# unibas-gravis/GiNGR

Measured on AMD Instinct MI355X. Metric: GiNGR update iters/sec, 50k<->50k CPD, higher is better.
Workload: dtype f64; 1 GPU; CPD update, synthetic Gaussian clouds 50000<->50000, GPMM rank 100, w=0.1, rigid global transform, sigma2_0=5032.781; points=50000, targets=50000, rank=100, parallelism=row-shard x1, exchange=single shard

## Files before the change

gingr_amd/_native.py:

```python
from __future__ import annotations

import ctypes
import os
from ctypes import POINTER, c_char_p, c_double, c_int, c_int32, c_int64, c_void_p

import numpy as np

_HERE = os.path.dirname(os.path.abspath(__file__))
LIB_PATH = os.environ.get("GINGR_HIP_LIB") or os.path.join(_HERE, "libgingr_hip.so")

GINGR_OK = 0
ERR_BAD_ARGUMENT, ERR_HIP, ERR_NONFINITE, ERR_NOT_SPD, ERR_NO_DEVICE, ERR_STATE, ERR_NOT_CONVERGED = 1, 2, 3, 4, 5, 6, 7
NUM_PHASES = 3
NUM_SEGMENTS = 2
SEGMENT_FULLFIT = 2
SEGMENT_REVSUM = 3
FLAVOUR_CPD, FLAVOUR_ICP, FLAVOUR_ICP_SURFACE, FLAVOUR_PAIRS = 0, 1, 2, 3
OP_UPDATE, OP_UPDATE_SAMPLE, OP_LOGPDF, OP_POSTERIOR_COVARIANCE, OP_POSTERIOR_MODEL = range(5)
FITTER_OPS = {
    flavour: tuple("gingr_fitter_" + op.format(name) for op in
                   ("update_{}_async", "update_{}_sample_async", "posterior_logpdf_{}", "posterior_covariance_{}", "posterior_model_{}"))
    for flavour, name in ((FLAVOUR_CPD, "cpd"), (FLAVOUR_ICP, "icp"), (FLAVOUR_ICP_SURFACE, "icp_surface"), (FLAVOUR_PAIRS, "pairs"))
}
RCCL_UNIQUE_ID_BYTES = 128

_STATUS_NAMES = {
    1: "GINGR_ERR_BAD_ARGUMENT", 2: "GINGR_ERR_HIP", 3: "GINGR_ERR_NONFINITE", 4: "GINGR_ERR_NOT_SPD",
    5: "GINGR_ERR_NO_DEVICE", 6: "GINGR_ERR_STATE", 7: "GINGR_ERR_NOT_CONVERGED",
}


class GingrNativeError(RuntimeError):
    def __init__(self, code: int, where: str, text: str = ""):
        self.code = code
        super().__init__(f"{where}: {_STATUS_NAMES.get(code, code)} {text}".strip())


class StateScalars(ctypes.Structure):
    _fields_ = [
        ("euler", c_double * 3), ("center", c_double * 3), ("translation", c_double * 3),
        ("scale", c_double), ("sigma2", c_double), ("iteration", c_int32), ("status", c_int32),
    ]


class CpdParams(ctypes.Structure):
    _fields_ = [("w", c_double), ("lambda_", c_double)]


class IcpParams(ctypes.Structure):
    _fields_ = [("initial_sigma", c_double), ("end_sigma", c_double), ("max_iterations", c_int32)]


class MhRequest(ctypes.Structure):
    _fields_ = [
        ("flavour", c_int32), ("kind", c_int32), ("cpd", POINTER(CpdParams)), ("icp", POINTER(IcpParams)),
        ("z", POINTER(c_double)), ("alpha", POINTER(c_double)), ("scalars", POINTER(StateScalars)),
        ("eval_sdev", c_double), ("eval_points", c_int64), ("need_forward", c_int32),
    ]


class MhResult(ctypes.Structure):
    _fields_ = [
        ("scalars", StateScalars), ("log_value", c_double), ("dist_sum", c_double), ("dist_max", c_double), ("count", c_int64),
        ("log_q_forward", c_double), ("log_q_backward", c_double), ("forward_status", c_int32), ("backward_status", c_int32),
    ]


ALLREDUCE_FN = ctypes.CFUNCTYPE(c_int, c_void_p, c_int32, c_void_p, c_int64)
_dp = POINTER(c_double)
_ip = POINTER(c_int32)

KERNEL_GAUSSIAN_MIXTURE, KERNEL_DOT, KERNEL_LOOKUP = 0, 1, 2
OPT_CULL, OPT_FINE_CULL, OPT_NN_GRID, OPT_TRI_GRID, OPT_SPLIT_EXCHANGE, OPT_GRAM_DOWNDATE, OPT_DECIMATE_BATCH = 0, 1, 2, 3, 4, 5, 6


class ScalarKernel(ctypes.Structure):
    _fields_ = [("kind", c_int32), ("n_kernels", c_int32), ("sigmas", _dp), ("scalings", _dp), ("mirror", c_double),
                ("scaling", c_double), ("lookup", _dp)]


GPMM_MAX_COLUMNS = 1536


class GpmmInfo(ctypes.Structure):
    _fields_ = [("columns", c_int32), ("rank", c_int32), ("tolerance_reached", c_int32), ("residual_fraction", c_double),
                ("kept_variance_fraction", c_double)]


CLASSIC_CPD_MAX_COLUMNS = 512


class ClassicCpdLowRankInfo(ctypes.Structure):
    _fields_ = [("columns", c_int32), ("tolerance_reached", c_int32), ("residual_fraction", c_double), ("factor_bytes", c_int64)]


class PcaInfo(ctypes.Structure):
    _fields_ = [("rank", c_int32), ("gpa_sweeps", c_int32), ("gpa_last_change", c_double), ("total_variance", c_double),
                ("kept_variance", c_double)]


class AugmentInfo(ctypes.Structure):
    _fields_ = [("columns", c_int32), ("rank", c_int32), ("total_variance", c_double), ("kept_variance", c_double)]


class LaplacianInfo(ctypes.Structure):
    _fields_ = [("n_components", c_int32), ("n_dropped", c_int32), ("block_columns", c_int32), ("outer_iterations", c_int32),
                ("total_degree", c_int32), ("converged", c_int32), ("max_residual", c_double), ("cut_gap", c_double)]


class NicpInfo(ctypes.Structure):
    _fields_ = [("iterations", c_int32), ("converged", c_int32), ("residual", c_double * 3), ("rhs_norm", c_double * 3)]


SIGNATURES = {
    "gingr_device_count": (c_int, []),
    "gingr_ctx_create": (c_int, [c_int, POINTER(c_void_p)]),
    "gingr_ctx_destroy": (None, [c_void_p]),
    "gingr_last_error": (c_char_p, [c_void_p]),
    "gingr_ctx_set_stream": (c_int, [c_void_p, c_void_p]),
    "gingr_ctx_get_stream": (c_void_p, [c_void_p]),
    "gingr_ctx_synchronize": (c_int, [c_void_p]),
    "gingr_build_info": (c_char_p, []),
    "gingr_ctx_set_option": (c_int, [c_void_p, c_int32, c_int32]),
    "gingr_ctx_get_option": (c_int, [c_void_p, c_int32, POINTER(c_int32)]),
    "gingr_cpd_stats": (c_int, [c_void_p, c_int64, _dp, c_int64, _dp, c_double, c_double, _dp, _dp, _dp, _dp, _dp]),
    "gingr_cpd_initial_sigma2": (c_int, [c_void_p, c_int64, _dp, c_int64, _dp, _dp]),
# ... 13 lines not shown
    "gingr_fitter_icp_surface_phase_async": (c_int, [c_void_p, POINTER(IcpParams), c_int32]),
    "gingr_fitter_get_surface_correspondence": (c_int, [c_void_p, _dp, _dp]),
    "gingr_fitter_surface_distance_stats": (c_int, [c_void_p, c_int32, c_int64, _dp, c_int32, c_double, _dp]),
    "gingr_fitter_mh_step": (c_int, [c_void_p, POINTER(MhRequest), _dp, _dp, POINTER(MhResult)]),
    "gingr_fitter_mh_restore": (c_int, [c_void_p]),
    "gingr_classic_cpd_create": (c_int, [c_void_p, c_int32, c_int64, _dp, c_int64, _dp, c_double, c_double, c_double, POINTER(c_void_p)]),
    "gingr_classic_cpd_destroy": (None, [c_void_p]),
    "gingr_classic_cpd_iterate": (c_int, [c_void_p, c_int32]),
    "gingr_classic_cpd_get": (c_int, [c_void_p, _dp, POINTER(c_double), _dp, _dp]),
    "gingr_classic_cpd_set": (c_int, [c_void_p, _dp, c_double]),
    "gingr_classic_cpd_create_lowrank": (c_int, [c_void_p, c_int64, _dp, c_int64, _dp, c_double, c_double, c_double, c_double, c_int32,
                                                 POINTER(ClassicCpdLowRankInfo), POINTER(c_void_p)]),
    "gingr_classic_cpd_get_factor": (c_int, [c_void_p, _ip, _dp]),
    "gingr_bcpd_create": (c_int, [c_void_p, c_int64, _dp, c_int64, _dp, c_double, c_double, c_double, c_double, c_double, POINTER(c_void_p)]),
    "gingr_bcpd_destroy": (None, [c_void_p]),
    "gingr_bcpd_iterate": (c_int, [c_void_p, c_int32]),
    "gingr_bcpd_get": (c_int, [c_void_p, _dp, _dp, _dp, _dp, _dp, _dp, _dp, _dp]),
    "gingr_bcpd_set": (c_int, [c_void_p, _dp, _dp, _dp, _dp, c_double]),
    "gingr_bcpd_create_lowrank": (c_int, [c_void_p, c_int64, _dp, c_int64, _dp, c_double, c_double, c_double, c_double, c_double, c_double,
                                          c_int32, POINTER(ClassicCpdLowRankInfo), POINTER(c_void_p)]),
    "gingr_bcpd_get_factor": (c_int, [c_void_p, _ip, _dp]),
    "gingr_classic_cpd_transform_points": (c_int, [c_void_p, c_int64, _dp, _dp]),
    "gingr_bcpd_transform_points": (c_int, [c_void_p, c_int64, _dp, _dp]),
    "gingr_bcpd_get_coefficients": (c_int, [c_void_p, _dp]),
    "gingr_mesh_distance_stats": (c_int, [c_void_p, c_int64, _dp, c_int64, _dp, c_int64, POINTER(c_int32), c_int32, c_double, _dp]),
    "gingr_fitter_update_icp_surface_sample_async": (c_int, [c_void_p, POINTER(IcpParams), _dp]),
    "gingr_fitter_posterior_logpdf_icp_surface": (c_int, [c_void_p, POINTER(IcpParams), _dp, POINTER(c_double)]),
    "gingr_rigid_icp_create": (c_int, [c_void_p, c_int32, c_int64, _dp, c_int64, _dp, POINTER(c_void_p)]),
    "gingr_rigid_icp_destroy": (None, [c_void_p]),
    "gingr_rigid_icp_iterate": (c_int, [c_void_p, c_int32, _dp]),
    "gingr_rigid_icp_get": (c_int, [c_void_p, _dp, _dp]),
    "gingr_rigid_icp_set": (c_int, [c_void_p, _dp]),
    "gingr_fitter_set_fit_points": (c_int, [c_void_p, _dp]),
    "gingr_nicp_solve": (c_int, [c_void_p, c_int32, c_int64, _dp, c_int64, _ip, _dp, _dp, c_int32, _ip, _dp, c_double, c_double, c_double,
                                 _dp, _dp]),
    "gingr_nicp_create": (c_int, [c_void_p, c_int32, c_int64, c_int64, _ip, c_int32, _ip, POINTER(c_void_p)]),
    "gingr_nicp_destroy": (None, [c_void_p]),
    "gingr_nicp_step": (c_int, [c_void_p, _dp, _dp, _dp, _dp, c_double, c_double, c_double, c_double, c_int32, _dp, _dp, POINTER(NicpInfo)]),
    "gingr_nicp_get_solution": (c_int, [c_void_p, _dp]),
    "gingr_mesh_closest_points": (c_int, [c_void_p, c_int64, _dp, c_int64, _dp, c_int64, _ip, _dp, _dp, _ip, _dp]),
    "gingr_mesh_decimate": (c_int, [c_void_p, c_int64, _dp, c_int64, _ip, c_int64, POINTER(c_int64), _ip, POINTER(c_int64), _ip, _dp]),
    "gingr_model_new_reference": (c_int, [c_void_p, c_void_p, c_int64, _dp, _ip, _dp, c_int64, c_int64, POINTER(c_void_p)]),
    "gingr_gpmm_build_diagonal": (c_int, [c_void_p, c_int64, _dp, POINTER(ScalarKernel), POINTER(ScalarKernel), POINTER(ScalarKernel),
                                          c_double, c_int32, c_int64, c_int64, POINTER(c_void_p)]),
    "gingr_gpmm_build_diagonal_ex": (c_int, [c_void_p, c_int64, _dp, POINTER(ScalarKernel), POINTER(ScalarKernel), POINTER(ScalarKernel),
                                             c_double, c_int32, c_int32, c_int64, c_int64, POINTER(GpmmInfo), POINTER(c_void_p)]),
    "gingr_model_truncate": (c_int, [c_void_p, c_void_p, c_int32, POINTER(c_void_p)]),
    "gingr_gpmm_build_gaussian": (c_int, [c_void_p, c_int64, _dp, c_int32, _dp, _dp, c_double, c_int32, c_int64, c_int64,
                                          POINTER(c_void_p)]),
    "gingr_pointset_distance_extrema": (c_int, [c_void_p, _dp, c_int64, _dp, _dp]),
    "gingr_model_download": (c_int, [c_void_p, c_void_p, _dp, _dp, _dp, _dp]),
    "gingr_model_num_points": (c_int64, [c_void_p]),
    "gingr_model_rank": (c_int32, [c_void_p]),
    "gingr_model_instance": (c_int, [c_void_p, c_void_p, _dp, _dp, _dp, _dp, c_double, _dp]),
    "gingr_model_coefficients": (c_int, [c_void_p, c_void_p, _dp, _dp, _dp, _dp, _dp]),
    "gingr_model_posterior_mean": (c_int, [c_void_p, c_void_p, _dp, _dp, _dp, _dp, _dp, c_int32, _ip, _dp, _dp, _dp, _dp]),
    "gingr_fitter_create": (c_int, [c_void_p, c_void_p, POINTER(c_void_p)]),
    "gingr_fitter_destroy": (None, [c_void_p]),
    "gingr_fitter_set_target": (c_int, [c_void_p, c_int64, _dp]),
    "gingr_fitter_set_landmarks": (c_int, [c_void_p, c_int32, _ip, _dp, _dp]),
    "gingr_fitter_set_options": (c_int, [c_void_p, c_int32, c_double]),
    "gingr_fitter_set_state": (c_int, [c_void_p, _dp, POINTER(StateScalars)]),
    "gingr_fitter_get_state": (c_int, [c_void_p, _dp, POINTER(StateScalars), _dp]),
    "gingr_fitter_get_cpd_stats": (c_int, [c_void_p, _dp, _dp, _dp, _dp]),
    "gingr_fitter_get_icp_idx": (c_int, [c_void_p, _ip, _dp]),
    "gingr_fitter_update_cpd_async": (c_int, [c_void_p, POINTER(CpdParams), c_int32]),
    "gingr_fitter_update_icp_async": (c_int, [c_void_p, POINTER(IcpParams), c_int32]),
    "gingr_fitter_update_cpd_sample_async": (c_int, [c_void_p, POINTER(CpdParams), _dp]),
    "gingr_fitter_update_icp_sample_async": (c_int, [c_void_p, POINTER(IcpParams), _dp]),
    "gingr_fitter_posterior_logpdf_cpd": (c_int, [c_void_p, POINTER(CpdParams), _dp, _dp]),
    "gingr_fitter_posterior_logpdf_icp": (c_int, [c_void_p, POINTER(IcpParams), _dp, _dp]),
    "gingr_model_marginal_covariance": (c_int, [c_void_p, c_void_p, _dp, _dp, _dp]),
    "gingr_model_cross_covariance": (c_int, [c_void_p, c_void_p, _dp, _dp, c_int64, _dp]),
    "gingr_fitter_posterior_covariance_cpd": (c_int, [c_void_p, POINTER(CpdParams), _dp]),
    "gingr_fitter_posterior_covariance_icp": (c_int, [c_void_p, POINTER(IcpParams), _dp]),
    "gingr_fitter_posterior_covariance_icp_surface": (c_int, [c_void_p, POINTER(IcpParams), _dp]),
    "gingr_model_posterior": (c_int, [c_void_p, c_void_p, _dp, _dp, _dp, _dp, _dp, c_int32, _ip, _dp, _dp, POINTER(c_void_p)]),
    "gingr_fitter_posterior_model_cpd": (c_int, [c_void_p, POINTER(CpdParams), POINTER(c_void_p)]),
    "gingr_fitter_posterior_model_icp": (c_int, [c_void_p, POINTER(IcpParams), POINTER(c_void_p)]),
    "gingr_fitter_posterior_model_icp_surface": (c_int, [c_void_p, POINTER(IcpParams), POINTER(c_void_p)]),
    "gingr_fitter_set_pairs": (c_int, [c_void_p, c_int64, _ip, _dp, _dp]),
    "gingr_fitter_set_pairs_cov": (c_int, [c_void_p, c_int64, _ip, _dp, _dp]),
    "gingr_fitter_get_pair_observations": (c_int, [c_void_p, _dp, _dp]),
    "gingr_fitter_set_sigma2": (c_int, [c_void_p, c_double]),
    "gingr_fitter_last_update_error": (c_int, [c_void_p, POINTER(c_int32)]),
    "gingr_fitter_update_pairs_async": (c_int, [c_void_p, c_int32]),
    "gingr_fitter_pairs_phase_async": (c_int, [c_void_p, c_int32]),
    "gingr_fitter_update_pairs_sample_async": (c_int, [c_void_p, _dp]),
    "gingr_fitter_posterior_logpdf_pairs": (c_int, [c_void_p, _dp, _dp]),
    "gingr_fitter_posterior_covariance_pairs": (c_int, [c_void_p, _dp]),
    "gingr_fitter_posterior_model_pairs": (c_int, [c_void_p, POINTER(c_void_p)]),
    "gingr_model_from_shapes": (c_int, [c_void_p, c_int64, c_int32, _dp, _dp, c_int32, c_int32, c_double, c_double, c_int32,
                                        POINTER(c_void_p), POINTER(PcaInfo)]),
    "gingr_model_augment": (c_int, [c_void_p, c_void_p, c_void_p, c_double, c_int32, POINTER(c_void_p), POINTER(AugmentInfo)]),
    "gingr_model_from_laplacian": (c_int, [c_void_p, c_int64, _dp, c_int64, _ip, c_double, c_int32, c_double, c_int32,
                                           POINTER(LaplacianInfo), POINTER(c_void_p)]),
    "gingr_fitter_retry_counter": (c_int, [c_void_p, c_int32, POINTER(c_int32)]),
    "gingr_fitter_exchange": (c_int, [c_void_p, POINTER(c_void_p), POINTER(c_int64), POINTER(c_int64)]),
    "gingr_fitter_cpd_phase_async": (c_int, [c_void_p, POINTER(CpdParams), c_int32]),
    "gingr_fitter_update_cpd_sharded_async": (c_int, [c_void_p, POINTER(CpdParams), c_int32, ALLREDUCE_FN, c_void_p]),
    "gingr_fitter_update_icp_sharded_async": (c_int, [c_void_p, POINTER(IcpParams), c_int32, ALLREDUCE_FN, c_void_p]),
    "gingr_fitter_icp_phase_async": (c_int, [c_void_p, POINTER(IcpParams), c_int32]),
    "gingr_fitter_update_sharded_async": (c_int, [c_void_p, c_int32, POINTER(CpdParams), POINTER(IcpParams), c_int32, _dp, ALLREDUCE_FN, c_void_p]),
    "gingr_fitter_posterior_logpdf_sharded": (c_int, [c_void_p, c_int32, POINTER(CpdParams), POINTER(IcpParams), _dp, ALLREDUCE_FN, c_void_p, _dp]),
    "gingr_fitter_fullfit_exchange": (c_int, [c_void_p, POINTER(c_void_p), POINTER(c_int64)]),
    "gingr_fitter_reversal_exchange": (c_int, [c_void_p, POINTER(c_void_p), POINTER(c_int64)]),
# ... 83 lines not shown
```

gingr_amd/csrc/common.h:

```cpp
#pragma once
#include <cstdlib>

#include <hip/hip_runtime.h>

#include <cstdarg>
#include <cstdint>
#include <cstdio>
#include <cstring>
#include <string>
#include <vector>

#include "../../include/gingr_hip.h"
#include "host_device.h"

#define GINGR_TIMERS 18

struct gingr_ctx {
    int device = 0;
    hipStream_t own_stream = nullptr;
    hipStream_t stream = nullptr;
    char err[512] = {0};
    bool timing = false;
    struct Span {
        hipEvent_t a, b;
        int which;
    };
    std::vector<Span> spans;
    std::vector<hipEvent_t> pool;
    double t_ms[GINGR_TIMERS] = {0};
    int64_t t_n[GINGR_TIMERS] = {0};
    int cull = 1;
    int tri_grid = 1;
    int nn_grid = 1;
    int32_t *regime_host = nullptr, *regime_dev = nullptr;
    int fine_override = -1;
    unsigned long long *nn_tests = nullptr;
    void *rccl_comm = nullptr;
    int32_t rccl_world = 0, rccl_rank = 0;
    int split_exchange = 0;
    int gram_downdate = -1;
    int decimate_batch = 16;
    hipStream_t side_stream = nullptr, exchange_stream = nullptr;
    hipEvent_t split_ev[2] = {nullptr, nullptr};
    void *scratch = nullptr;
    size_t scratch_bytes = 0;
};

int gingr_set_error(gingr_ctx *ctx, int code, const char *fmt, ...);
void gingr_ctx_rccl_release(gingr_ctx *ctx);

#define HIP_TRY(ctx, expr)                                                                                   \
    do {                                                                                                     \
        hipError_t e__ = (expr);                                                                             \
        if (e__ != hipSuccess)                                                                               \
            return gingr_set_error((ctx), GINGR_ERR_HIP, "%s failed: %s (%s:%d)", #expr, hipGetErrorString(e__), \
                                   __FILE__, __LINE__);                                                      \
    } while (0)

#define GINGR_TRY(expr)          \
    do {                         \
        int s__ = (expr);        \
        if (s__ != GINGR_OK) return s__; \
    } while (0)

#define HANDLE_TRY(ctx, fail, expr)                                                              \
    do {                                                                                         \
        if ((expr) != hipSuccess) {                                                              \
            (void)hipGetLastError();                                                             \
            return fail(gingr_set_error((ctx), GINGR_ERR_HIP, "%s: %s", __func__, #expr));       \
        }                                                                                        \
    } while (0)

inline int check_launch(gingr_ctx *ctx) {
    HIP_TRY(ctx, hipGetLastError());
    return GINGR_OK;
}

struct DevBuf {
    void *p = nullptr;
    size_t bytes = 0;
    DevBuf() = default;
    DevBuf(const DevBuf &) = delete;
    DevBuf &operator=(const DevBuf &) = delete;
    ~DevBuf() {
        if (p) (void)hipFree(p);
    }
    void release() {
        if (p) (void)hipFree(p);
        p = nullptr;
        bytes = 0;
    }
    hipError_t alloc(size_t n) {
        release();
// ... 108 lines not shown
```

gingr_amd/csrc/context.hip:

```cpp
#include "common.h"

#include <map>
#include <mutex>
void set_dynamic_lds(const void *func, int bytes) {
    static std::mutex mu;
    static std::map<std::pair<int, const void *>, int> limit;
    int dev = 0;
    (void)hipGetDevice(&dev);
    std::lock_guard<std::mutex> lock(mu);
    int &have = limit[std::make_pair(dev, func)];
    if (have >= bytes) return;
    if (hipFuncSetAttribute(func, hipFuncAttributeMaxDynamicSharedMemorySize, bytes) == hipSuccess)
        have = bytes;
    else
        (void)hipGetLastError();
}


int gingr_set_error(gingr_ctx *ctx, int code, const char *fmt, ...) {
    if (ctx) {
        va_list ap;
        va_start(ap, fmt);
        vsnprintf(ctx->err, sizeof(ctx->err), fmt, ap);
        va_end(ap);
// ... 78 lines not shown
    (void)hipGetLastError();
    *out = ctx;
    return GINGR_OK;
}

void gingr_ctx_destroy(gingr_ctx *ctx) {
    if (!ctx) return;
    (void)hipSetDevice(ctx->device);
    (void)hipStreamSynchronize(ctx->stream);
    timing_resolve(ctx);
    gingr_ctx_rccl_release(ctx);
    for (auto e : ctx->pool) (void)hipEventDestroy(e);
    if (ctx->scratch) (void)hipFree(ctx->scratch);
    if (ctx->nn_tests) (void)hipFree(ctx->nn_tests);
    if (ctx->regime_host) (void)hipHostFree(ctx->regime_host);
    if (ctx->side_stream) {
        (void)hipStreamSynchronize(ctx->side_stream);
        (void)hipStreamDestroy(ctx->side_stream);
    }
    for (hipEvent_t e : ctx->split_ev)
        if (e) (void)hipEventDestroy(e);
    if (ctx->own_stream) (void)hipStreamDestroy(ctx->own_stream);
    delete ctx;
}

const char *gingr_last_error(const gingr_ctx *ctx) { return ctx ? ctx->err : "null context"; }

int gingr_ctx_set_stream(gingr_ctx *ctx, void *hip_stream) {
    if (!ctx) return GINGR_ERR_BAD_ARGUMENT;
    HIP_TRY(ctx, hipStreamSynchronize(ctx->stream));
    ctx->stream = hip_stream ? reinterpret_cast<hipStream_t>(hip_stream) : ctx->own_stream;
    return GINGR_OK;
}

void *gingr_ctx_get_stream(gingr_ctx *ctx) { return ctx ? reinterpret_cast<void *>(ctx->stream) : nullptr; }

int gingr_ctx_synchronize(gingr_ctx *ctx) {
    if (!ctx) return GINGR_ERR_BAD_ARGUMENT;
    HIP_TRY(ctx, hipSetDevice(ctx->device));
    HIP_TRY(ctx, hipStreamSynchronize(ctx->stream));
    return GINGR_OK;
}

int gingr_ctx_set_option(gingr_ctx *ctx, int32_t option, int32_t value) {
    if (!ctx) return GINGR_ERR_BAD_ARGUMENT;
    switch (option) {
        case GINGR_OPT_CULL: ctx->cull = value != 0; return GINGR_OK;
        case GINGR_OPT_FINE_CULL: ctx->fine_override = value < 0 ? -1 : (value != 0); return GINGR_OK;
        case GINGR_OPT_NN_GRID: ctx->nn_grid = value < 0 ? 0 : (value > 2 ? 2 : value); return GINGR_OK;
        case GINGR_OPT_TRI_GRID: ctx->tri_grid = value < 0 ? 0 : (value > 2 ? 2 : value); return GINGR_OK;
        case GINGR_OPT_SPLIT_EXCHANGE: ctx->split_exchange = value != 0; return GINGR_OK;
        case GINGR_OPT_GRAM_DOWNDATE: ctx->gram_downdate = value < 0 ? -1 : (value != 0); return GINGR_OK;
        case GINGR_OPT_DECIMATE_BATCH: ctx->decimate_batch = value < 1 ? 1 : (value > 60 ? 60 : value); return GINGR_OK;
        default: return gingr_set_error(ctx, GINGR_ERR_BAD_ARGUMENT, "ctx_set_option: unknown option %d", option);
    }
}

int gingr_ctx_get_option(gingr_ctx *ctx, int32_t option, int32_t *value) {
    if (!ctx || !value) return GINGR_ERR_BAD_ARGUMENT;
    switch (option) {
        case GINGR_OPT_CULL: *value = ctx->cull; return GINGR_OK;
        case GINGR_OPT_FINE_CULL: *value = ctx->fine_override; return GINGR_OK;
        case GINGR_OPT_NN_GRID: *value = ctx->nn_grid; return GINGR_OK;
        case GINGR_OPT_TRI_GRID: *value = ctx->tri_grid; return GINGR_OK;
        case GINGR_OPT_SPLIT_EXCHANGE: *value = ctx->split_exchange; return GINGR_OK;
        case GINGR_OPT_GRAM_DOWNDATE: *value = ctx->gram_downdate; return GINGR_OK;
        case GINGR_OPT_DECIMATE_BATCH: *value = ctx->decimate_batch; return GINGR_OK;
        default: return gingr_set_error(ctx, GINGR_ERR_BAD_ARGUMENT, "ctx_get_option: unknown option %d", option);
    }
}

int gingr_ctx_timing_enable(gingr_ctx *ctx, int32_t enable) {
    if (!ctx) return GINGR_ERR_BAD_ARGUMENT;
    ctx->timing = enable != 0;
    return GINGR_OK;
}

int gingr_ctx_timing_read(gingr_ctx *ctx, int32_t which, double *total_ms, int64_t *launches) {
    if (!ctx || which < 0 || which >= GINGR_TIMERS) return GINGR_ERR_BAD_ARGUMENT;
    timing_resolve(ctx);
    if (total_ms) *total_ms = ctx->t_ms[which];
    if (launches) *launches = ctx->t_n[which];
    return GINGR_OK;
}

int gingr_ctx_nn_counting(gingr_ctx *ctx, int32_t enable) {
    if (!ctx) return GINGR_ERR_BAD_ARGUMENT;
    HIP_TRY(ctx, hipSetDevice(ctx->device));
    HIP_TRY(ctx, hipStreamSynchronize(ctx->stream));
    if (enable && !ctx->nn_tests) {
        void *p = nullptr;
        HIP_TRY(ctx, hipMalloc(&p, sizeof(unsigned long long)));
        ctx->nn_tests = static_cast<unsigned long long *>(p);
    }
    if (ctx->nn_tests) {
        HIP_TRY(ctx, hipMemsetAsync(ctx->nn_tests, 0, sizeof(unsigned long long), ctx->stream));
        HIP_TRY(ctx, hipStreamSynchronize(ctx->stream));
    }
    if (!enable && ctx->nn_tests) {
        (void)hipFree(ctx->nn_tests);
        ctx->nn_tests = nullptr;
    }
    return GINGR_OK;
}

int gingr_ctx_nn_tests(gingr_ctx *ctx, int64_t *tests) {
    if (!ctx || !tests) return GINGR_ERR_BAD_ARGUMENT;
    *tests = 0;
    if (!ctx->nn_tests) return gingr_set_error(ctx, GINGR_ERR_STATE, "nn_tests: counting is off (gingr_ctx_nn_counting)");
    HIP_TRY(ctx, hipSetDevice(ctx->device));
    HIP_TRY(ctx, hipStreamSynchronize(ctx->stream));
    unsigned long long v = 0;
    HIP_TRY(ctx, hipMemcpy(&v, ctx->nn_tests, sizeof(v), hipMemcpyDeviceToHost));
    *tests = (int64_t)v;
    return GINGR_OK;
}

int gingr_ctx_timing_reset(gingr_ctx *ctx) {
    if (!ctx) return GINGR_ERR_BAD_ARGUMENT;
    timing_resolve(ctx);
// ... 210 lines not shown
```

gingr_amd/csrc/fitter.h:

```cpp
#pragma once

#include "gp.h"
#include "surface.h"

#include <cstdlib>
#include <vector>

struct StatScratch {
    DevBuf cp, d2, nn, nnd2, ws, part, out;
    DevBuf pos;
    int64_t pos_K = -1, pos_T = -1;
    const int32_t *pos_tri = nullptr;
};

struct gingr_fitter {
    gingr_ctx *ctx = nullptr;
    const gingr_model *m = nullptr;
    int64_t N = 0;
    double *target = nullptr;
    double *inv_den = nullptr, *Pt1 = nullptr;
    double *fit = nullptr;
    double *P1 = nullptr, *PX = nullptr;
    int32_t *nn_idx = nullptr;
    double *nn_d2 = nullptr;
// ... 18 lines not shown
    int32_t *tperm = nullptr;
    std::vector<int32_t> h_tperm;
    double *tboxes = nullptr, *fboxes = nullptr;
    int32_t *tile_bad = nullptr;
    double *xch = nullptr;
    int64_t off[GINGR_NUM_SEGMENTS] = {0, 0}, cnt[GINGR_NUM_SEGMENTS] = {0, 0};
    double *ws = nullptr;
    int64_t ws_doubles = 0;
    int colsum_chunks = 0;
    double *work = nullptr;
    void *aos = nullptr;
    int32_t n_lm = 0;
    int32_t *lm_pid = nullptr;
    double *lm_xyz = nullptr, *lm_cov = nullptr;
    int32_t *lm_mask = nullptr;
    int32_t global_transform = GINGR_RIGID_TRANSFORMS;
    double step_length = 1.0;
    double stop_threshold = -1.0;
    int32_t stop_hit = 0;
    int32_t last_err = 0;
    bool has_state = false;
    int32_t surface_method = 0;
    bool reversed = false;
    int32_t *radj_ptr = nullptr, *radj_tri = nullptr, *rmbnd = nullptr;
    double *rmvn = nullptr, *rfboxes = nullptr;
    void *rws = nullptr;
    int64_t rq0 = 0, rqn = 0;
    double *rtvn_loc = nullptr;
    double *revsum = nullptr, *partial_revsum = nullptr;
    int32_t *gperm = nullptr;
    double *gsorted = nullptr;
    int32_t *rnn_pos = nullptr;
    bool rnn_warm = false;
    int32_t *rtri_pos = nullptr;
    bool rtri_warm = false;
    int32_t *mtri_orig = nullptr, *mboundary = nullptr;
    double *rcp = nullptr, *rd2 = nullptr, *rnnd2 = nullptr, *rw01 = nullptr, *robs = nullptr, *rwin = nullptr;
    int32_t *rnn = nullptr, *rpre = nullptr, *rhit = nullptr, *rkeys = nullptr, *rvals = nullptr, *rskeys = nullptr, *rsvals = nullptr;
    void *rsort = nullptr;
    size_t rsort_bytes = 0;
    int64_t Tm = 0, Tt = 0;
    int32_t *mtri = nullptr, *ttri = nullptr, *ttri_orig = nullptr;
    int32_t *madj_ptr = nullptr, *madj_tri = nullptr, *tadj_ptr = nullptr, *tadj_tri = nullptr;
    double *mcn = nullptr, *tcn = nullptr, *mvn = nullptr, *tvn = nullptr;
    double *mtboxes = nullptr, *ttboxes = nullptr;
    double *mtribox = nullptr, *ttribox = nullptr;
    int32_t *tboundary = nullptr;
    double *surf_cp = nullptr, *surf_d2 = nullptr, *surf_w01 = nullptr, *surf_win = nullptr, *surf_nnd2 = nullptr;
    int32_t *surf_nn = nullptr, *surf_pre = nullptr, *surf_hit = nullptr;
    struct Key {
        std::vector<double> v;
        int flavour = -1;
        double p0 = 0, p1 = 0;
        bool same(const Key &o) const { return flavour == o.flavour && p0 == o.p0 && p1 == o.p1 && v == o.v; }
    };
    Key state_key, post_key;
    bool state_key_valid = false;
    int post_stage = 0;
    bool skip_phase1 = false;
    double *small = nullptr;
    StatScratch *stat_scratch = nullptr;
    double *alt_seg = nullptr;
    bool seg_swapped = false;
    double *seg1_live() const { return seg_swapped ? alt_seg : xch + off[1]; }
    double *seg1_parked() const { return seg_swapped ? xch + off[1] : alt_seg; }
    Key alt_key;
    int alt_stage = 0;
    bool allow_alt = false, corr_stale = false;
    double *fxbuf[2] = {nullptr, nullptr};
    unsigned *lp_sync = nullptr;
    double *lp_scratch = nullptr;
    unsigned lp_epoch = 0;
    bool fx_valid[2] = {false, false};
    double *nfac[2] = {nullptr, nullptr};
    bool nf_valid[2] = {false, false};
    int live = 0;
    int32_t *surf_tri_pos = nullptr;
    bool surf_tri_warm = false;
    bool nn_warm = false, surf_nn_warm = false;
    NNGrid tgrid;
    TriGrid ttgrid;
    MovGrid mgrid;
    void forget_posteriors() {
        post_stage = 0;
        alt_stage = 0;
        fx_valid[0] = fx_valid[1] = false;
        nf_valid[0] = nf_valid[1] = false;
    }
    double *partial_out = nullptr;
    double *fullfit = nullptr, *partial_fullfit = nullptr;
    int32_t *zero_counts = nullptr;
    double *gstage = nullptr;
    int gstage_world = 0;
    int gather_agreed = -1, gather_agreed_world = 0;
    bool sharded() const { return m->M != m->M_total; }
    int32_t *retry = nullptr;
    double *fit_alt = nullptr, *mh_save = nullptr;
    double *mh_rb = nullptr;
    Key mh_key;
    bool mh_saved = false;
    uint64_t mh_serial = 0;
    bool cpd_seen = false, fit_boxes_valid = false;
    int split_half = 0;
    DevBuf cov_work, cov_out;
    int64_t n_pairs = 0, pairs_cap = -1;
    int32_t *ppid = nullptr, *pkeys = nullptr, *pvals = nullptr, *pskeys = nullptr, *psvals = nullptr;
    double *pxyz = nullptr, *pvar = nullptr, *pobs = nullptr, *pwin = nullptr;
    void *psort = nullptr;
    size_t psort_bytes = 0;
    int32_t n_pc = 0, n_cat = 0;
    std::vector<int32_t> h_pc_row, h_lm_row, h_lm_mask;
    std::vector<double> h_pc_xyz, h_pc_cov, h_lm_xyz, h_lm_cov;
    DevBuf cat_pid, cat_xyz, cat_cov;
};

constexpr int64_t kGramDowndateMinRows = 16384;
constexpr int64_t kTriGridMinTriangles = 16384;
constexpr size_t kScalarsDoubles = (sizeof(gingr_state_scalars) + 7) / 8, kDevStateDoubles = (sizeof(DevState) + 7) / 8;

template <typename T>
int dev_alloc(gingr_ctx *ctx, T **p, size_t count) {
    HIP_TRY(ctx, hipMalloc(reinterpret_cast<void **>(p), (count ? count : 1) * sizeof(T)));
    static const bool poison = getenv("GINGR_DEBUG_POISON") != nullptr;
    if (poison) {
        HIP_TRY(ctx, hipMemset(*p, 0xFF, (count ? count : 1) * sizeof(T)));
        HIP_TRY(ctx, hipDeviceSynchronize());
    }
    return GINGR_OK;
}

inline void dev_free(void *p) { if (p) (void)hipFree(p); }

inline Cloud cloud_of(const double *soa, int64_t n) { return Cloud{soa, soa + n, soa + 2 * n, n}; }

inline hipError_t ensure(DevBuf &b, size_t bytes) { return b.p && b.bytes >= bytes ? hipSuccess : b.alloc(bytes); }

int check_ready(gingr_fitter *f);
int check_parameters(gingr_fitter *f, const Correspondence &c);
SweepArgs base_args(const gingr_fitter *f);
void refresh_fit(gingr_fitter *f);
void fit_boxes_now(gingr_fitter *f);
std::vector<double> state_key_values(int32_t r, const double *alpha, const double euler[3], const double center[3], const double t[3],
                                     double scale, double sigma2);
void scalars_of_state(const DevState &hst, gingr_state_scalars *s);
int fitter_upload_zrand(gingr_fitter *f, const double *z);
void launch_mh_readback(gingr_ctx *ctx, int64_t n, const double *block, int nblock, const double *fit, int64_t M, const int32_t *perm,
                        double *out, double *flag, int32_t *done, double epoch);
bool wait_pinned_flag(gingr_fitter *f, double epoch);
int pull_small(gingr_fitter *f, const double *src, int n, double *dst);
struct PinnedWords {
    double *pin = nullptr;
    size_t pin_doubles = 0;
    double *pin_dev = nullptr;
    int32_t *done = nullptr;
    uint64_t epoch = 0;
};
bool wait_pinned_flag(const PinnedWords &w, double epoch);
int pull_small(gingr_ctx *ctx, PinnedWords &w, const double *src, int n, double *dst);
int model_observation_system(gingr_ctx *ctx, const gingr_model *model, const double euler[3], const double center[3],
                             const double translation[3], const double *obs_xyz, const double *weight, int32_t n_lm, const int32_t *lm_pid,
                             const double *lm_xyz, const double *lm_cov, gingr_fitter **f_out, DevBuf &sys);
struct Rot3 {
    double R[9];
};
void launch_basis_rotate(gingr_ctx *ctx, const gingr_model *src, const double *T, const Rot3 &rot, gingr_model *dst);
int gather_fit(gingr_fitter *f, const Correspondence &c, gingr_allreduce_fn reduce, void *user, fitter_gather_fn gather, const char *who);
int fitter_posterior_inputs(gingr_fitter *f, const Correspondence &c);
void free_meshes(gingr_fitter *f);
int pairs_ensure_planes(gingr_fitter *f);
int pairs_rebuild_cov_list(gingr_fitter *f);
void free_pairs(gingr_fitter *f);
```

gingr_amd/csrc/fitter.hip:

```cpp
#include "fitter.h"

#include <algorithm>
#include <atomic>
#include <chrono>
#include <thread>

namespace {

__global__ __launch_bounds__(256) void mh_readback_kernel(const double *__restrict__ block, int nblock, const double *__restrict__ fit, int64_t M,
                                                         const int32_t *__restrict__ perm, double *__restrict__ out, double *flag,
                                                         int32_t *__restrict__ done, double epoch) {
    const int64_t i = (int64_t)blockIdx.x * 256 + threadIdx.x;
    if (i < nblock) out[i] = block[i];
    if (fit && i < M) {
        const int64_t o = perm ? perm[i] : i;
        double *dst = out + nblock + 3 * o;
        dst[0] = fit[i];
        dst[1] = fit[M + i];
        dst[2] = fit[2 * M + i];
    }
    if (!flag) return;
    __threadfence_system();
    __syncthreads();
    if (threadIdx.x == 0) {
        if (atomicAdd(done, 1) == (int)gridDim.x - 1) {
            *done = 0;
            __threadfence_system();
            *reinterpret_cast<volatile double *>(flag) = epoch;
        }
    }
}

}

void launch_mh_readback(gingr_ctx *ctx, int64_t n, const double *block, int nblock, const double *fit, int64_t M, const int32_t *perm,
                        double *out, double *flag, int32_t *done, double epoch) {
    hipLaunchKernelGGL(mh_readback_kernel, dim3((unsigned)ceil_div(n, 256)), dim3(256), 0, ctx->stream, block, nblock, fit, M, perm, out, flag,
                       done, epoch);
}

SweepArgs base_args(const gingr_fitter *f) {
    SweepArgs a;
    memset(&a, 0, sizeof(a));
    a.Q0 = f->m->Q0;
    a.ref = f->m->ref;
    a.mean = f->m->mean;
    a.M = f->m->M;
    a.rp = f->m->rp;
    a.state = f->st;
    a.pose = f->pose;
    a.c0[0] = f->m->c0[0];
    a.c0[1] = f->m->c0[1];
    a.c0[2] = f->m->c0[2];
    a.partial = f->ws;
    return a;
}

void fit_boxes_now(gingr_fitter *f) {
    if (!f->fboxes) return;
    (void)hipMemsetAsync(f->absmax + 1, 0, sizeof(double), f->ctx->stream);
    launch_tile_bbox(f->ctx, cloud_of(f->fit, f->m->M), f->fboxes, f->absmax + 2, f->absmax + 1);
    f->fit_boxes_valid = true;
}

void refresh_fit(gingr_fitter *f) {
    SweepArgs a = base_args(f);
    a.coef0 = f->alpha;
    a.shape_out = f->fit;
    if (f->fboxes && f->m->rp <= 512 && f->cpd_seen) {
        a.qboxes = f->fboxes + 6 * ceil_div(f->m->M, 256);
        a.box_centre = f->absmax + 2;
        a.absmax_slot = f->absmax + 1;
        launch_sweep(f->ctx, SWEEP_FIT, a);
        f->fit_boxes_valid = true;
    } else {
        launch_sweep(f->ctx, SWEEP_FIT, a);
        f->fit_boxes_valid = false;
        if (f->cpd_seen) fit_boxes_now(f);
    }
}

int check_ready(gingr_fitter *f) {
    if (!f) return GINGR_ERR_BAD_ARGUMENT;
    if (!f->target) return gingr_set_error(f->ctx, GINGR_ERR_STATE, "update: no target set (gingr_fitter_set_target)");
    if (!f->has_state) return gingr_set_error(f->ctx, GINGR_ERR_STATE, "update: no state set (gingr_fitter_set_state)");
    if (hipSetDevice(f->ctx->device) != hipSuccess) return gingr_set_error(f->ctx, GINGR_ERR_HIP, "hipSetDevice failed");
    return GINGR_OK;
}

int check_parameters(gingr_fitter *f, const Correspondence &c) {
    GINGR_TRY(check_ready(f));
    switch (correspondence_error(c)) {
        case CorrespondenceError::None: return GINGR_OK;
        case CorrespondenceError::CpdParams: return gingr_set_error(f->ctx, GINGR_ERR_BAD_ARGUMENT, "cpd params: need 0 <= w < 1 and lambda > 0");
        case CorrespondenceError::IcpParams: return gingr_set_error(f->ctx, GINGR_ERR_BAD_ARGUMENT, "icp params: max_iterations < 1");
        case CorrespondenceError::BadFlavour: break;
    }
    return gingr_set_error(f->ctx, GINGR_ERR_BAD_ARGUMENT, "correspondence flavour %d out of range", (int)c.kind);
}

int check_correspondence(gingr_fitter *f, const Correspondence &c) {
    GINGR_TRY(check_parameters(f, c));
    if (needs_meshes(c) && (!f->Tm || !f->Tt)) return gingr_set_error(f->ctx, GINGR_ERR_STATE, "icp surface: no meshes set (gingr_fitter_set_meshes)");
    if (c.kind == Flavour::Pairs) GINGR_TRY(pairs_ensure_planes(f));
    return GINGR_OK;
}

std::vector<double> state_key_values(int32_t r, const double *alpha, const double euler[3], const double center[3], const double t[3],
                                     double scale, double sigma2) {
    std::vector<double> v(alpha, alpha + r);
    for (int q = 0; q < 3; ++q) v.push_back(euler[q]);
    for (int q = 0; q < 3; ++q) v.push_back(center[q]);
    for (int q = 0; q < 3; ++q) v.push_back(t[q]);
    v.push_back(scale);
    v.push_back(sigma2);
    return v;
}

void scalars_of_state(const DevState &hst, gingr_state_scalars *s) {
    for (int q = 0; q < 3; ++q) {
        s->euler[q] = hst.euler[q];
        s->center[q] = hst.center[q];
// ... 126 lines not shown
                    f->zrand, f->pose, f->scalars, f->fxbuf[0], f->fxbuf[1], f->alt_seg, f->nfac[0], f->nfac[1],
                    f->lp_sync, f->lp_scratch, f->retry, f->part, f->absmax, f->tperm, f->tboxes, f->fboxes,
                    f->tile_bad, f->xch, f->fullfit, f->gstage, f->zero_counts, f->ws, f->work, f->aos, f->lm_pid,
                    f->lm_xyz, f->lm_cov, f->lm_mask};
    for (void *q : ptrs) dev_free(q);
    if (f->pin) (void)hipHostFree(f->pin);
    if (f->zpin) (void)hipHostFree(f->zpin);
    if (f->zpin_done) (void)hipEventDestroy(f->zpin_done);
    nn_grid_free(&f->tgrid);
    tri_grid_free(&f->ttgrid);
    free_meshes(f);
    free_pairs(f);
    delete f;
}

int gingr_fitter_set_target(gingr_fitter *f, int64_t N, const double *target_xyz) {
    if (!f) return GINGR_ERR_BAD_ARGUMENT;
    f->nn_warm = f->surf_nn_warm = f->surf_tri_warm = false;
    f->forget_posteriors();
    gingr_ctx *ctx = f->ctx;
    if (N < 1 || N > INT32_MAX || !target_xyz) return gingr_set_error(ctx, GINGR_ERR_BAD_ARGUMENT, "set_target: bad N");
    HIP_TRY(ctx, hipSetDevice(ctx->device));
    HIP_TRY(ctx, hipStreamSynchronize(ctx->stream));
    const int64_t M = f->m->M;
    const int32_t rp = f->m->rp;
    void *old[] = {f->target, f->inv_den, f->Pt1, f->xch, f->ws, f->aos, f->tperm, f->tboxes, f->fboxes, f->tile_bad};
    for (void *q : old) dev_free(q);
    free_meshes(f);
    f->target = f->inv_den = f->Pt1 = f->xch = f->ws = f->tboxes = f->fboxes = nullptr;
    f->aos = nullptr;
    f->tperm = f->tile_bad = nullptr;
    f->N = N;
    GINGR_TRY(dev_alloc(ctx, &f->target, (size_t)3 * N));
    GINGR_TRY(dev_alloc(ctx, &f->inv_den, (size_t)N));
    GINGR_TRY(dev_alloc(ctx, &f->Pt1, (size_t)N));
    f->cnt[0] = N;
    f->cnt[1] = (int64_t)rp * rp + rp + 8 + rp;
    int64_t o = 0;
    for (int s = 0; s < GINGR_NUM_SEGMENTS; ++s) {
        f->off[s] = o;
        o += round_up(f->cnt[s], 32);
    }
    GINGR_TRY(dev_alloc(ctx, &f->xch, (size_t)o));
    f->seg_swapped = false;
    HIP_TRY(ctx, hipMemsetAsync(f->xch, 0, (size_t)o * sizeof(double), ctx->stream));
    int64_t w = cpd_colsum_ws_doubles(M, N);
    auto mx = [&](int64_t v) {
        if (v > w) w = v;
    };
    mx(cpd_rowstats_ws_doubles(M, N));
    mx(ceil_div(nn_ws_bytes(M, N), 8));
    mx(ceil_div(nn_ws_bytes(N, M), 8));
    mx(gram_ws_doubles(M, rp) + sweep_ws_doubles(M, rp));
    f->ws_doubles = w;
    GINGR_TRY(dev_alloc(ctx, &f->ws, (size_t)w));
    const int64_t big = M > N ? M : N;
    double *aos = nullptr;
    GINGR_TRY(dev_alloc(ctx, &aos, (size_t)3 * big));
    f->aos = aos;
    HIP_TRY(ctx, hipMemcpyAsync(aos, target_xyz, (size_t)3 * N * sizeof(double), hipMemcpyHostToDevice, ctx->stream));
    kd_leaf_order(target_xyz, N, f->h_tperm);
    GINGR_TRY(nn_grid_build(ctx, target_xyz, N, f->h_tperm.data(), M, &f->tgrid));
    GINGR_TRY(dev_alloc(ctx, &f->tperm, (size_t)N));
    HIP_TRY(ctx, hipMemcpyAsync(f->tperm, f->h_tperm.data(), (size_t)N * sizeof(int32_t), hipMemcpyHostToDevice, ctx->stream));
    GINGR_TRY(dev_alloc(ctx, &f->tboxes, (size_t)ceil_div(N, 256) * 30));
    GINGR_TRY(dev_alloc(ctx, &f->fboxes, (size_t)ceil_div(M, 256) * 30));
    f->fit_boxes_valid = false;
    GINGR_TRY(dev_alloc(ctx, &f->tile_bad, (size_t)ceil_div(N, 256)));
    launch_aos_to_soa(ctx, aos, N, f->target, f->tperm);
    launch_tile_bbox(ctx, cloud_of(f->target, N), f->tboxes);
    launch_cloud_centroid(ctx, cloud_of(f->target, N), f->absmax + 2);
    launch_cloud_absmax(ctx, cloud_of(f->target, N), f->absmax + 2, f->absmax);
    if (f->has_state) fit_boxes_now(f);
    GINGR_TRY(check_launch(ctx));
    HIP_TRY(ctx, hipStreamSynchronize(ctx->stream));
    return GINGR_OK;
}

int gingr_fitter_set_landmarks(gingr_fitter *f, int32_t n_lm, const int32_t *lm_pid, const double *lm_xyz,
                               const double *lm_cov) {
    if (!f) return GINGR_ERR_BAD_ARGUMENT;
    f->forget_posteriors();
    gingr_ctx *ctx = f->ctx;
    if (n_lm < 0 || (n_lm > 0 && (!lm_pid || !lm_xyz || !lm_cov)))
        return gingr_set_error(ctx, GINGR_ERR_BAD_ARGUMENT, "set_landmarks: bad argument");
    HIP_TRY(ctx, hipSetDevice(ctx->device));
    HIP_TRY(ctx, hipStreamSynchronize(ctx->stream));
    dev_free(f->lm_pid);
    dev_free(f->lm_xyz);
    dev_free(f->lm_cov);
    f->lm_pid = nullptr;
    f->lm_xyz = f->lm_cov = nullptr;
    f->n_lm = n_lm;
    const int64_t M = f->m->M;
    std::vector<int32_t> mask((size_t)M, 0), local((size_t)(n_lm > 0 ? n_lm : 1), -1);
    for (int32_t l = 0; l < n_lm; ++l) {
        if (lm_pid[l] < 0 || lm_pid[l] >= f->m->M_total)
            return gingr_set_error(ctx, GINGR_ERR_BAD_ARGUMENT, "set_landmarks: point id %d out of range", lm_pid[l]);
        const int64_t lp = (int64_t)lm_pid[l] - f->m->row_begin;
        if (lp >= 0 && lp < M) {
            const int32_t pos = f->m->hiperm[(size_t)lp];
            local[(size_t)l] = pos;
            mask[(size_t)pos] = 1;
        }
    }
    HIP_TRY(ctx, hipMemcpy(f->lm_mask, mask.data(), (size_t)M * sizeof(int32_t), hipMemcpyHostToDevice));
// ... 171 lines not shown
        scalars6[5] = loc[5];
    }
    return GINGR_OK;
}

int gingr_fitter_get_icp_idx(gingr_fitter *f, int32_t *idx, double *d2) {
    if (!f) return GINGR_ERR_BAD_ARGUMENT;
    gingr_ctx *ctx = f->ctx;
    if (f->corr_stale)
        return gingr_set_error(ctx, GINGR_ERR_STATE, "get_icp_idx: a probabilistic query brought another state's posterior back; the correspondences on the device are not this state's -- run an update or a phase first");
    HIP_TRY(ctx, hipSetDevice(ctx->device));
    const int64_t M = f->m->M;
    std::vector<int32_t> hidx((size_t)M);
    std::vector<double> hd2((size_t)M);
    HIP_TRY(ctx, hipMemcpyAsync(hidx.data(), f->nn_idx, (size_t)M * sizeof(int32_t), hipMemcpyDeviceToHost, ctx->stream));
    HIP_TRY(ctx, hipMemcpyAsync(hd2.data(), f->nn_d2, (size_t)M * sizeof(double), hipMemcpyDeviceToHost, ctx->stream));
    HIP_TRY(ctx, hipStreamSynchronize(ctx->stream));
    for (int64_t sidx = 0; sidx < M; ++sidx) {
        const int32_t row = f->m->hperm[(size_t)sidx];
        const int32_t pos = hidx[(size_t)sidx];
        if (idx) idx[row] = (pos >= 0 && (size_t)pos < f->h_tperm.size()) ? f->h_tperm[(size_t)pos] : -1;
        if (d2) d2[row] = hd2[(size_t)sidx];
    }
    return GINGR_OK;
}

int gingr_fitter_retry_counter(gingr_fitter *f, int32_t set_to, int32_t *value_out) {
    if (!f) return GINGR_ERR_BAD_ARGUMENT;
    gingr_ctx *ctx = f->ctx;
    HIP_TRY(ctx, hipSetDevice(ctx->device));
    if (set_to >= 0) HIP_TRY(ctx, hipMemcpyAsync(f->retry, &set_to, sizeof(set_to), hipMemcpyHostToDevice, ctx->stream));
    int32_t v = set_to;
    if (value_out && set_to < 0) HIP_TRY(ctx, hipMemcpyAsync(&v, f->retry, sizeof(v), hipMemcpyDeviceToHost, ctx->stream));
    HIP_TRY(ctx, hipStreamSynchronize(ctx->stream));
    if (value_out) *value_out = v;
    return GINGR_OK;
}

int gingr_fitter_exchange(gingr_fitter *f, void **dev_ptr, int64_t offsets[GINGR_NUM_SEGMENTS],
                          int64_t counts[GINGR_NUM_SEGMENTS]) {
    if (!f || !dev_ptr) return GINGR_ERR_BAD_ARGUMENT;
    if (!f->xch) return gingr_set_error(f->ctx, GINGR_ERR_STATE, "exchange: no target set");
    *dev_ptr = f->xch;
    for (int s = 0; s < GINGR_NUM_SEGMENTS; ++s) {
        if (offsets) offsets[s] = f->off[s];
        if (counts) counts[s] = f->cnt[s];
    }
    return GINGR_OK;
}

}

void fitter_set_partial_output(gingr_fitter *f, double *base) { f->partial_out = base; }
void fitter_set_partial_fullfit(gingr_fitter *f, double *base) { f->partial_fullfit = base; }
double *fitter_fullfit(gingr_fitter *f) { return f->fullfit; }
void fitter_set_partial_revsum(gingr_fitter *f, double *base) { f->partial_revsum = base; }
double *fitter_revsum(gingr_fitter *f) { return f->revsum; }
int fitter_upload_zrand(gingr_fitter *f, const double *z) {
    gingr_ctx *ctx = f->ctx;
    const size_t bytes = (size_t)f->m->rp * sizeof(double);
    if (!f->zpin) {
        HIP_TRY(ctx, hipHostMalloc(reinterpret_cast<void **>(&f->zpin), bytes, hipHostMallocDefault));
        if (hipEventCreateWithFlags(&f->zpin_done, hipEventDisableTiming) != hipSuccess) {
            (void)hipHostFree(f->zpin);
            f->zpin = nullptr, f->zpin_done = nullptr;
            return gingr_set_error(ctx, GINGR_ERR_HIP, "upload of the posterior draws: hipEventCreate failed");
        }
    } else {
        HIP_TRY(ctx, hipEventSynchronize(f->zpin_done));
    }
    memset(f->zpin, 0, bytes);
    memcpy(f->zpin, z, (size_t)f->m->r * sizeof(double));
    HIP_TRY(ctx, hipMemcpyAsync(f->zrand, f->zpin, bytes, hipMemcpyHostToDevice, ctx->stream));
    HIP_TRY(ctx, hipEventRecord(f->zpin_done, ctx->stream));
    return GINGR_OK;
}
int fitter_set_zrand(gingr_fitter *f, const double *z) {
    f->zrand_active = false;
    if (!z) return GINGR_OK;
    GINGR_TRY(fitter_upload_zrand(f, z));
    f->zrand_active = true;
    return GINGR_OK;
}
gingr_ctx *fitter_ctx(gingr_fitter *f) { return f->ctx; }
bool fitter_gather_possible(gingr_fitter *f, int32_t world, int32_t rank) {
    if (!f || !f->fullfit || world < 1 || rank < 0 || rank >= world) return false;
    const gingr_model *m = f->m;
    const int64_t Mt = m->M_total, base = Mt / world, extra = Mt % world;
    const int64_t b = rank * base + (rank < extra ? rank : extra), e = b + base + (rank < extra ? 1 : 0);
    return b == m->row_begin && e - b == m->M;
}
int fitter_gather_agreed(gingr_fitter *f, int32_t world) { return f->gather_agreed_world == world ? f->gather_agreed : -1; }
void fitter_set_gather_agreed(gingr_fitter *f, int32_t world, int agreed) {
    f->gather_agreed = agreed;
    f->gather_agreed_world = world;
}
bool fitter_reversed(gingr_fitter *f) { return f->reversed; }
const gingr_model *fitter_model(gingr_fitter *f) { return f->m; }
```

gingr_amd/csrc/fitter_phases.hip:

```cpp
#include "fitter.h"

#include <algorithm>
#include <utility>

namespace {

__global__ __launch_bounds__(256) void swap_segments_kernel(double *__restrict__ a, double *__restrict__ b, int64_t n, int exchange) {
    const int64_t i = (int64_t)blockIdx.x * 256 + threadIdx.x;
    if (i >= n) return;
    const double va = a[i], vb = b[i];
    a[i] = vb;
    if (exchange) b[i] = va;
}

__global__ __launch_bounds__(256) void fit_contribution_kernel(const double *__restrict__ fit, const int32_t *__restrict__ iperm, int64_t M,
                                                               int64_t row_begin, int64_t M_total, double *__restrict__ full) {
    const int64_t g = (int64_t)blockIdx.x * 256 + threadIdx.x;
    if (g >= M_total) return;
    const int64_t l = g - row_begin;
    const bool mine = l >= 0 && l < M;
    const int64_t pos = mine ? iperm[l] : 0;
#pragma unroll
    for (int d = 0; d < 3; ++d) full[d * M_total + g] = mine ? fit[d * M + pos] : 0.0;
}
// ... 15 lines not shown
    const int64_t q = g < cut ? g / (base + 1) : extra + (g - cut) / (base > 0 ? base : 1);
    const int64_t b = q * base + (q < extra ? q : extra);
    const double *p = stage + q * 3 * chunk + (g - b);
#pragma unroll
    for (int d = 0; d < 3; ++d) full[d * M_total + g] = p[d * chunk];
}

__global__ __launch_bounds__(256) void reversal_local_kernel(int64_t M, int64_t row_begin, const int32_t *__restrict__ perm, int64_t M_total,
                                                             const double *__restrict__ sums, const double *__restrict__ sigma2,
                                                             double *__restrict__ obs, double *__restrict__ win) {
    const int64_t p = (int64_t)blockIdx.x * 256 + threadIdx.x;
    if (p >= M) return;
    const int64_t g = row_begin + perm[p];
    const double k = sums[3 * M_total + g];
    const double kk = k > 0.0 ? k : 1.0;
#pragma unroll
    for (int d = 0; d < 3; ++d) obs[d * M + p] = sums[d * M_total + g] / kk;
    win[p] = k / sigma2[0];
}

__global__ __launch_bounds__(256) void soa_permute_kernel(const double *__restrict__ src, const int32_t *__restrict__ perm, int64_t n,
                                                          double *__restrict__ dst) {
    const int64_t p = (int64_t)blockIdx.x * 256 + threadIdx.x;
    if (p >= n) return;
    const int64_t g = perm[p];
#pragma unroll
    for (int d = 0; d < 3; ++d) dst[d * n + p] = src[d * n + g];
}
__global__ __launch_bounds__(256) void index_map_kernel(const int32_t *__restrict__ pos, int64_t n, const int32_t *__restrict__ map,
                                                        int32_t *__restrict__ idx) {
    const int64_t j = (int64_t)blockIdx.x * 256 + threadIdx.x;
    if (j >= n) return;
    const int32_t v = pos[j];
    idx[j] = v >= 0 ? map[v] : v;
}

int64_t split_cut(int64_t N) { return (N / 512) * 256; }

void nearest_target_vertex(gingr_ctx *ctx, gingr_fitter *f, Cloud query, Cloud tgt, int32_t *idx, double *d2, bool warm) {
    const int32_t *w = warm ? idx : nullptr;
    if (ctx->nn_grid && f->tgrid.ready && ctx->cull && query.n <= f->tgrid.max_queries) {
        if (!launch_nn_grid(ctx, query, tgt, f->tperm, f->tgrid, w, idx, d2))
            launch_nn(ctx, query, tgt, f->tperm, f->tboxes, f->ws, idx, d2, idx, f->tgrid.flag, f->tgrid.cur_nflag());
    } else {
        launch_nn(ctx, query, tgt, f->tperm, f->tboxes, f->ws, idx, d2, w);
    }
}

struct Segments {
    double *seg0, *G, *rhs, *sc8;
    double *seg0w, *Gw, *rhsw, *sc8w;
};

bool memo_enter(gingr_fitter *f, const Correspondence &c, int phase) {
    const gingr_model *m = f->m;
    if (phase == 0) {
        f->skip_phase1 = false;
        gingr_fitter::Key k;
        k.flavour = memo_flavour_key(c, f->surface_method, f->reversed);
        k.p0 = c.cpd.w;
        k.p1 = c.cpd.lambda;
        const bool single = m->M == m->M_total;
        if (single && f->state_key_valid) {
            k.v = f->state_key.v;
            if (f->post_stage == 2 && f->post_key.same(k)) {
                f->skip_phase1 = true;
                return true;
            }
            if (f->allow_alt && !f->partial_out && f->alt_stage == 2 && f->alt_key.same(k)) {
                const bool both = f->post_stage == 2;
                f->seg_swapped = !f->seg_swapped;
                if (both) {
                    std::swap(f->post_key, f->alt_key);
                } else {
                    f->post_key = f->alt_key;
                    f->alt_stage = 0;
                    f->fx_valid[f->live] = f->nf_valid[f->live] = false;
                }
                f->live ^= 1;
                f->post_stage = 2;
                f->corr_stale = true;
                f->skip_phase1 = true;
                return true;
            }
            if (f->allow_alt && !f->partial_out && f->post_stage == 2) {
                f->seg_swapped = !f->seg_swapped;
                f->alt_key = f->post_key;
                f->alt_stage = 2;
                f->live ^= 1;
            }
            f->fx_valid[f->live] = f->nf_valid[f->live] = false;
            f->post_key = k;
            f->post_stage = 1;
        } else {
            f->post_stage = 0;
            f->fx_valid[f->live] = f->nf_valid[f->live] = false;
        }
        f->corr_stale = false;
    } else if (phase == 1) {
        if (f->skip_phase1) {
            f->skip_phase1 = false;
            return true;
        }
        if (f->post_stage == 1) f->post_stage = 2;
    } else {
        f->state_key_valid = false;
        f->mh_saved = false;
    }
    return false;
}

void phase0_cpd_colsums(gingr_fitter *f, const Segments &s, Cloud fit, Cloud tgt) {
    gingr_ctx *ctx = f->ctx;
    const gingr_model *m = f->m;
// ... 181 lines not shown
        CpdObsArgs ob;
        memset(&ob, 0, sizeof(ob));
        ob.ref = m->ref;
        ob.mean = m->mean;
        ob.sigma2 = &f->st->sigma2;
        ob.R = f->st->R;
        ob.center = f->st->center;
        ob.t = f->st->t;
        ob.lambda = c.cpd.lambda;
        ob.lm_mask = f->lm_mask;
        ob.weight = f->weight;
        ob.evec = f->evec;
        launch_cpd_rowstats(ctx, fit, tgt, &f->st->sigma2, f->absmax, f->inv_den, f->tboxes, f->tile_bad, f->ws, f->P1,
                            f->PX, f->part, f->scalars, nullptr, 0, &ob, false);
        fa.scalar_mode = 1;
        fa.part = f->part;
        fa.scalars_local = f->scalars;
        fa.contribute_xpx = m->row_begin == 0 ? 1 : 0;
    }
}

struct GramOutcome {
    bool rhs_done;
    ZeroGate rhs_gate;
};

GramOutcome phase1_gram(gingr_fitter *f, const Correspondence &c, double *gram_ws, double *sweep_ws, Phase1FinalizeArgs &fa) {
    gingr_ctx *ctx = f->ctx;
    const gingr_model *m = f->m;
    const int64_t M = m->M;
    const int32_t rp = m->rp;
    GramOutcome out{false, ZeroGate{}};
    if (uniform_weights(c, f->reversed, f->n_lm)) {
        fa.nslabs = 0;
        fa.scaled_src = m->mom + MomentLayout{rp}.stot();
        fa.sigma2 = &f->st->sigma2;
        fa.scaled_contribute = m->row_begin == 0 ? 1 : 0;
    } else if (zero_one_weights(c, f->reversed) &&
               (ctx->gram_downdate == 1 || (ctx->gram_downdate < 0 && M >= kGramDowndateMinRows))) {
        const bool gated = ctx->gram_downdate != 1;
        ZeroGate few{f->zero_counts, (int32_t)ceil_div(M, 256), 0, M}, many = few;
        many.run_if_many = 1;
        fa.gram_partial = gram_ws;
        fa.nslabs = launch_gram_downdate(ctx, m->Q0, M, rp, f->weight, gram_ws, gated ? &few : nullptr);
        fa.scaled_src = m->mom + MomentLayout{rp}.stot();
        fa.sigma2 = &f->st->sigma2;
        fa.scaled_contribute = m->row_begin == 0 ? 1 : 0;
        if (gated) {
            bool alt_rhs = false;
            fa.alt_nslabs = launch_gram(ctx, m->Q0, M, rp, f->weight, gram_ws, nullptr, f->evec, sweep_ws, &alt_rhs, &many);
            fa.gate = many;
            out.rhs_gate = few;
        }
    } else {
        fa.gram_partial = gram_ws;
        fa.nslabs = launch_gram(ctx, m->Q0, M, rp, f->weight, gram_ws, nullptr, f->evec, sweep_ws, &out.rhs_done);
    }
    return out;
}

void phase2_solve_and_commit(gingr_fitter *f, const Correspondence &c, const Segments &s) {
    gingr_ctx *ctx = f->ctx;
    const gingr_model *m = f->m;
    const int32_t r = m->r, rp = m->rp;
    const bool eig = uniform_weights(c, f->reversed, f->n_lm) && !f->zrand_active && m->eig_ready;
    if (eig)
        launch_posterior_solve_eig(ctx, r, rp, m->eigV, m->eigL, &f->st->sigma2, s.rhs, f->acoef, f->st);
    else if (f->zrand_active && f->allow_alt && f->post_stage == 2 && f->nf_valid[f->live] && m->M == m->M_total && !f->partial_out)
        launch_posterior_sample_cached(ctx, r, rp, f->nfac[f->live], f->fxbuf[f->live] + (int64_t)rp * rp, f->zrand, f->acoef, f->st);
    else
        launch_posterior_solve(ctx, r, rp, s.G, s.rhs, f->zrand_active ? f->zrand : nullptr, f->work, f->acoef, f->st);
    launch_post_matvecs(ctx, m, f->alpha, f->acoef, f->zbuf);
    PostSolveArgs a;
    memset(&a, 0, sizeof(a));
    a.r = r;
    a.rp = rp;
    a.pvec = m->pvec;
    a.zbuf = f->zbuf;
    a.alpha = f->alpha;
    a.scalars = s.sc8;
    a.is_icp = post_solve_sigma2_rule(c);
    if (is_icp_schedule(c)) {
        a.icp_step = (c.icp.initial_sigma - c.icp.end_sigma) / (double)c.icp.max_iterations;
        a.icp_end = c.icp.end_sigma;
    }
    a.step = f->step_length;
    a.global_transform = f->global_transform;
    a.state = f->st;
    a.retry = f->retry;
    a.zero_slot = f->absmax + 1;
    a.probabilistic = f->zrand_active ? 1 : 0;
    a.stop_threshold = f->stop_threshold;
    launch_post_solve(ctx, a);
    refresh_fit(f);
}

int run_phase(gingr_fitter *f, const Correspondence &c, int phase) {
    gingr_ctx *ctx = f->ctx;
    const gingr_model *m = f->m;
    const int64_t M = m->M;
    const int32_t rp = m->rp;
    if (f->seg_swapped && !f->allow_alt) {
        const int64_t seg = (int64_t)rp * rp + rp + 8;
        hipLaunchKernelGGL(swap_segments_kernel, dim3((unsigned)ceil_div(seg, 256)), dim3(256), 0, ctx->stream, f->xch + f->off[1], f->alt_seg,
                           seg, 0);
        f->seg_swapped = false;
        f->alt_stage = 0;
        f->fx_valid[f->live ^ 1] = f->nf_valid[f->live ^ 1] = false;
    }
    Segments s;
    s.seg0 = f->xch + f->off[0];
    s.G = f->seg1_live();
    s.rhs = s.G + (int64_t)rp * rp;
    s.sc8 = s.rhs + rp;
    double *wbase = f->partial_out ? f->partial_out : f->xch;
    s.seg0w = wbase + f->off[0];
    s.Gw = f->partial_out ? wbase + f->off[1] : s.G;
    s.rhsw = s.Gw + (int64_t)rp * rp;
    s.sc8w = s.rhsw + rp;
    const Cloud fit = cloud_of(f->fit, M);
    const Cloud tgt = cloud_of(f->target, f->N);
    if (phase == GINGR_PHASE_GATHER) {
        if (!f->sharded()) return GINGR_OK;
        if (!f->fullfit) return gingr_set_error(ctx, GINGR_ERR_STATE, "gather phase: no meshes set (gingr_fitter_set_meshes)");
        hipLaunchKernelGGL(fit_contribution_kernel, dim3((unsigned)ceil_div(m->M_total, 256)), dim3(256), 0, ctx->stream, f->fit, m->iperm, M,
                           m->row_begin, m->M_total, f->partial_fullfit ? f->partial_fullfit : f->fullfit);
        return check_launch(ctx);
    }
    const Cloud meshc = f->sharded() && f->fullfit ? cloud_of(f->fullfit, m->M_total) : fit;
    if (memo_enter(f, c, phase)) return GINGR_OK;
    switch (phase) {
        case 0:
            if (c.kind == Flavour::Pairs)
                break;
            if (reversed_icp(c, f->reversed))
                GINGR_TRY(phase0_reversed(f, c, fit, tgt, meshc));
            else if (c.kind == Flavour::IcpSurface)
                phase0_surface(f, fit, tgt, meshc);
            else if (c.kind == Flavour::IcpCloud)
                phase0_nearest_vertex(f, fit, tgt);
            else
                phase0_cpd_colsums(f, s, fit, tgt);
            break;
        case 1: {
            Phase1FinalizeArgs fa;
            memset(&fa, 0, sizeof(fa));
            fa.rp = rp;
// ... 266 lines not shown
```

gingr_amd/csrc/gp.h:

```cpp
#pragma once

#include "common.h"
#include "correspondence.h"
#include "svd3.h"

#include <functional>

#define GINGR_COEFF_NOISE 1e-5

struct DevState {
    double R[9];
    double euler[3];
    double center[3];
    double t[3];
    double scale;
    double sigma2;
    int32_t iteration;
    int32_t status;
    int32_t err;
    int32_t pad;
    int32_t stopped;
    int32_t pad2;
};

// ... 23 lines not shown
    double scale;
};

struct MomentLayout {
    int32_t rp;
    __host__ __device__ int64_t stot() const { return 0; }
    __host__ __device__ int64_t S(int d, int e) const { return (int64_t)rp * rp * (1 + d * 3 + e); }
    __host__ __device__ int64_t V(int d, int e) const { return (int64_t)rp * rp * 10 + (int64_t)rp * (d * 3 + e); }
    __host__ __device__ int64_t W(int d) const { return (int64_t)rp * rp * 10 + (int64_t)rp * (9 + d); }
    __host__ __device__ int64_t total() const { return (int64_t)rp * rp * 10 + (int64_t)rp * 12; }
};

struct PostVec {
    int32_t rp;
    static constexpr int kV = 0;
    static constexpr int kW = 9;
    static constexpr int kBV = 12;
    static constexpr int kBW = 21;
    static constexpr int kRows = 24;
    __host__ __device__ int64_t consts() const { return (int64_t)kRows * rp; }
    __host__ __device__ int64_t total() const { return consts() + 16; }
    static constexpr int kZa = 0;
    static constexpr int kBSa = 9;
    static constexpr int kBTa = 18;
    static constexpr int kA1 = 27;
    static constexpr int kZRows = 28;
};

constexpr int kBasisRowSlack = 144;

struct gingr_model {
    gingr_ctx *ctx = nullptr;
    int64_t M_total = 0, row_begin = 0, row_end = 0, M = 0;
    int32_t r = 0, rp = 0;
    double *Q0 = nullptr;
    double *ref = nullptr;
    double *mean = nullptr;
    double *mom = nullptr;
    int32_t *perm = nullptr;
    std::vector<int32_t> hperm, hiperm;
    int32_t *iperm = nullptr;
    std::vector<double> h_full_pts;
    double *Binv = nullptr;
    double *eigV = nullptr;
    double *eigL = nullptr;
    bool eig_ready = false;
    double *cmat = nullptr;
    double *pvec = nullptr;
    double c0[3] = {0, 0, 0};
    double Pp[9] = {0};
    double Ps[3] = {0};
    std::vector<double> variance;
    bool finalized = false;
};

void launch_interp_pack(gingr_ctx *ctx, const double *Qs, int32_t rp, const int32_t *inv_src, const int32_t *ids, const double *w,
                        const int32_t *perm_new, int64_t row_begin, int64_t M, double *Q0);

int model_create_impl(gingr_ctx *ctx, int64_t M_total, int32_t rank, const double *ref, const double *mean,
                      const double *variance, int64_t row_begin, int64_t row_end,
                      const std::function<int(gingr_model *)> &fill_basis, gingr_model **out, bool finalize = true);

void fitter_set_partial_output(gingr_fitter *f, double *base);
void fitter_set_partial_fullfit(gingr_fitter *f, double *base);
int check_correspondence(gingr_fitter *f, const Correspondence &c);
typedef int (*fitter_gather_fn)(void *user, gingr_fitter *f);
int fitter_sharded_update(gingr_fitter *f, const Correspondence &c, int32_t n_iterations, const double *z, gingr_allreduce_fn reduce,
                          void *user, fitter_gather_fn gather = nullptr, bool split_native = false);
int fitter_sharded_logpdf(gingr_fitter *f, const Correspondence &c, const double *mesh_xyz_full, gingr_allreduce_fn reduce, void *user,
                          double *logpdf, fitter_gather_fn gather = nullptr);
int fitter_run_phase(gingr_fitter *f, const Correspondence &c, int phase);
int fitter_update(gingr_fitter *f, const Correspondence &c, int32_t n_iterations);
int fitter_sample_update(gingr_fitter *f, const Correspondence &c, const double *z);
int fitter_posterior_logpdf(gingr_fitter *f, const Correspondence &c, const double *mesh_xyz, double *logpdf);
int fitter_logpdf_prepare(gingr_fitter *f, const double *mesh_xyz_full);
int fitter_logpdf_finish(gingr_fitter *f, double *logpdf);
int fitter_set_zrand(gingr_fitter *f, const double *z);
double *fitter_fullfit(gingr_fitter *f);
void fitter_set_partial_revsum(gingr_fitter *f, double *base);
double *fitter_revsum(gingr_fitter *f);
gingr_ctx *fitter_ctx(gingr_fitter *f);
bool fitter_gather_possible(gingr_fitter *f, int32_t world, int32_t rank);
int fitter_gather_agreed(gingr_fitter *f, int32_t world);
void fitter_set_gather_agreed(gingr_fitter *f, int32_t world, int agreed);
const gingr_model *fitter_model(gingr_fitter *f);

struct ZeroGate {
    const int32_t *counts;
    int32_t nblocks;
    int32_t run_if_many;
    int64_t M;
};

__device__ __forceinline__ bool gate_open(const ZeroGate &g) {
    if (!g.counts) return true;
    __shared__ int gate_sum;
    if (threadIdx.x == 0) gate_sum = 0;
    __syncthreads();
    int s = 0;
    for (int b = threadIdx.x; b < g.nblocks; b += blockDim.x) s += g.counts[b];
#pragma unroll
    for (int off = 32; off > 0; off >>= 1) s += __shfl_xor(s, off);
    if ((threadIdx.x & 63) == 0 && s != 0) atomicAdd(&gate_sum, s);
    __syncthreads();
    const bool many = (int64_t)gate_sum * 8 > g.M;
    return many == (g.run_if_many != 0);
}

enum SweepMode {
    SWEEP_RHS = 0,
    SWEEP_PROJ1 = 1,
    SWEEP_SHAPES = 2,
    SWEEP_PROJ2 = 3,
    SWEEP_FIT = 4,
    SWEEP_POSED = 5,
    SWEEP_RHS_ICP = 6
};

struct SweepArgs {
    const double *Q0;
    const double *ref;
    const double *mean;
    int64_t M;
    int32_t rp;
    const double *coef0;
    const double *coef1;
    const double *evec;
    const double *shape_in;
    double *shape_out;
    const DevState *state;
    const DevPose *pose;
    double c0[3];
    double *partial;
    double *out;
    double *zero_slot;
    double *qboxes;
    const double *box_centre;
    double *absmax_slot;
    int32_t no_reduce;
    const int32_t *icp_idx;
    const double *tx, *ty, *tz;
    int64_t n_targets;
    const int32_t *lm_mask;
    double *weight_out, *evec_out;
    const DevState *frame;
    ZeroGate gate;
};

int sweep_num_blocks(int64_t M);
int64_t sweep_ws_doubles(int64_t M, int32_t rp);
void launch_sweep(gingr_ctx *ctx, SweepMode mode, const SweepArgs &a);

int64_t gram_ws_doubles(int64_t M, int32_t rp);
int launch_gram(gingr_ctx *ctx, const double *Q0, int64_t M, int32_t rp, const double *weight, double *ws, double *G,
                const double *evec = nullptr, double *rhs_partial = nullptr, bool *rhs_done = nullptr, const ZeroGate *gate = nullptr);

int64_t gram_wide_ws_doubles(int64_t M, int32_t rp);
int launch_gram_wide(gingr_ctx *ctx, const double *Q0, int64_t M, int32_t rp, const double *weight, double *ws, const double *evec,
                     double *rhs_partial, const ZeroGate *gate = nullptr);

int64_t gram_rows_ws_doubles(int64_t rows, int32_t rp);
int launch_gram_rows(gingr_ctx *ctx, const double *Z, int64_t rows, int32_t rp, double *ws);

struct Phase1FinalizeArgs {
    int32_t rp;
    const double *gram_partial;
    int32_t nslabs;
    const double *scaled_src;
    const double *sigma2;
    int32_t scaled_contribute;
    double *G;
    const double *sweep_partial;
    int32_t sweep_blocks;
    double *rhs;
    int32_t scalar_mode;
    const double *part;
    double *scalars_local;
    double *sc8;
    int32_t contribute_xpx;
    ZeroGate gate;
    int32_t alt_nslabs;
};
void launch_phase1_finalize(gingr_ctx *ctx, const Phase1FinalizeArgs &a);
int launch_gram_downdate(gingr_ctx *ctx, const double *Q0, int64_t M, int32_t rp, const double *weight, double *ws,
                         const ZeroGate *gate = nullptr);

void launch_obs_cpd(gingr_ctx *ctx, const gingr_model *m, const DevState *st, Cloud fit, const double *P1,
                    const double *PX, double lambda, const int32_t *lm_mask, double *weight, double *evec);
void launch_obs_icp(gingr_ctx *ctx, const gingr_model *m, const DevState *st, Cloud target, const int32_t *idx,
                    const int32_t *lm_mask, double *weight, double *evec);
void launch_obs_points(gingr_ctx *ctx, const gingr_model *m, const DevState *st, const double *obs_soa,
                       const double *weight_in, double *weight, double *evec, const int32_t *lm_mask = nullptr,
                       int32_t *zero_counts = nullptr);
void launch_landmarks(gingr_ctx *ctx, const gingr_model *m, const DevState *st, int32_t n_lm, const int32_t *lm_pid_local,
                      const double *lm_xyz, const double *lm_cov, double *G, double *rhs);

void launch_posterior_solve(gingr_ctx *ctx, int32_t r, int32_t rp, const double *G, const double *rhs, const double *zrand,
                            double *work, double *a, DevState *st);
int launch_posterior_logpdf(gingr_ctx *ctx, int32_t r, int32_t rp, const double *G, const double *rhs, const double *Stot,
                            const double *qte, double *fx, bool cached, double *work, double *out2, unsigned *sync = nullptr,
                            unsigned epoch = 0, bool keep_factor = true, double *nfac = nullptr);
void launch_posterior_sample_cached(gingr_ctx *ctx, int32_t r, int32_t rp, const double *nfac, const double *a_mean, const double *zrand,
                                    double *a, DevState *st);
void launch_posterior_solve_eig(gingr_ctx *ctx, int32_t r, int32_t rp, const double *eigV, const double *eigL, const double *sigma2,
                                const double *rhs, double *a, DevState *st);
constexpr int kJacMaxN = 512;
int sym_eig(gingr_ctx *ctx, int count, const double *const *G, const int32_t *ldg, const int32_t *n, double *const *evals,
            double *const *Vs, bool blocks = false);
int launch_jacobi_eig(gingr_ctx *ctx, const double *G, int32_t ldg, int32_t n, double *evals, double *Vs, bool blocks = false);
constexpr int kSymEigColsMaxN = 192;
int64_t sym_eig_cols_work_doubles(int32_t n);
int64_t sym_eig_blocks_work_doubles(int32_t n);
int sym_eig_blocks(gingr_ctx *ctx, int count, const double *const *G, const int32_t *ldg, const int32_t *n, double *const *work,
                   double *const *evals, double *const *Vs, int32_t *const *info);
void launch_sym_eig_cols(gingr_ctx *ctx, int count, const double *const *G, const int32_t *ldg, const int32_t *n, double *const *work,
                         double *const *evals, double *const *Vs, int32_t *const *info);
int64_t posterior_work_doubles(int32_t rp);
int64_t binv_work_doubles(int32_t rp);
void launch_binv(gingr_ctx *ctx, int32_t r, int32_t rp, const double *S, double *work, double *Binv, int32_t *err_flag);
void launch_coeff_solve(gingr_ctx *ctx, int32_t r, int32_t rp, const double *Binv, const double *p, double *out);
void launch_state_init(gingr_ctx *ctx, DevState *st, const gingr_state_scalars *host_scalars_dev, double *zero_slot = nullptr);

int64_t moment_grams_ws_doubles(int64_t M, int32_t rp);
void launch_moment_grams(gingr_ctx *ctx, const double *Q0, int64_t M, int32_t rp, double *ws, double *mom);
void launch_centered_mean(gingr_ctx *ctx, const gingr_model *m, double *ptil);

struct PostSolveArgs {
    int32_t r, rp;
    const double *pvec;
    const double *zbuf;
    double *alpha;
    const double *scalars;
    int32_t is_icp;
    double icp_step, icp_end;
    double step;
    int32_t global_transform;
    DevState *state;
    double *zero_slot;
    int32_t *retry;
    int32_t probabilistic;
    double stop_threshold;
};
#define GINGR_RETRY_INIT 10
void launch_post_solve(gingr_ctx *ctx, const PostSolveArgs &a);
void launch_post_matvecs(gingr_ctx *ctx, const gingr_model *m, const double *alpha, const double *a, double *zbuf);
void launch_small_gemm(gingr_ctx *ctx, int32_t r, int32_t rp, const double *A, const double *B, double scale, double *out);
void launch_postvec(gingr_ctx *ctx, int32_t r, int32_t rp, const double *Binv, const double *moment_vectors, double *pvec);

void launch_marginal_covariance(gingr_ctx *ctx, const gingr_model *m, const double *W, int64_t ldw, bool upper, const double R[9],
                                const DevState *state, double *cov6);
void launch_cross_covariance(gingr_ctx *ctx, const gingr_model *m, const double *W, int64_t ldw, const double R[9], int64_t device_row,
// ... 7 lines not shown
```

gingr_amd/csrc/gp.hip:

```cpp
#include "dense_spd.h"
#include "gp.h"
#include "solve_blocks.h"

#include <algorithm>

namespace {


template <bool FAST, typename PtrD>
__device__ __forceinline__ void posterior_solve_body(PtrD sm, int r, int rp, const double *__restrict__ G, const double *__restrict__ rhs,
                                                     const double *__restrict__ zrand, double *__restrict__ a, DevState *__restrict__ st,
                                                     int *bad_spd, int *bad) {
    const int n = rp, ld = solve_ld(n);
    constexpr int XR = FAST ? 2 * kNB : kNB;
    auto A = sm;
    auto y = sm + (size_t)n * ld;
    auto rd = sm + (size_t)(n + XR) * ld;
    auto y2 = rd + n;
    const int tid = threadIdx.x;
    if (tid == 0) {
        *bad_spd = 0;
        *bad = 0;
    }
    for (int k = tid; k < kNB * ld; k += kSolveThreads) y[k] = k < r ? rhs[k] : 0.0;
    for (int k = tid; k < n; k += kSolveThreads) y2[k] = (zrand && k < r) ? zrand[k] : 0.0;
    if (FAST)
        for (int k = tid; k < kNB * ld; k += kSolveThreads) {
            const int c = k / ld, j = k - c * ld;
            y[kNB * ld + k] = (j < n && (j & 15) == c) ? 1.0 : 0.0;
        }
    GINGR_STAGE_CLOCK(7)
    lds_load_spd<kSolveThreads>(A, ld, r, n, G, 1.0, nullptr, 0.0, 1.0);
    GINGR_STAGE_CLOCK(0)
    lds_cholesky<kSolveThreads>(A, ld, n, rd, bad_spd, kNB, FAST ? kNB : 0);
    GINGR_STAGE_CLOCK(4)
    if constexpr (FAST) {
        if (zrand) {
            lds_backward_w<kSolveThreads>(A, ld, n, y + kNB * ld, y2, rd);
            for (int k = tid; k < n; k += kSolveThreads) y2[k] = rd[k];
            __syncthreads();
        }
        lds_backward_w<kSolveThreads>(A, ld, n, y + kNB * ld, y, rd);
        for (int k = tid; k < n; k += kSolveThreads) y[k] = rd[k];
        __syncthreads();
    } else {
        lds_backward<kSolveThreads>(A, ld, n, rd, y);
        if (zrand) lds_backward<kSolveThreads>(A, ld, n, rd, y2);
    }
    GINGR_STAGE_CLOCK(5)
    GINGR_STAGE_CLOCK(6)
    for (int k = tid; k < rp; k += kSolveThreads) {
        const double v = k < r ? y[k] + y2[k] : 0.0;
        a[k] = v;
        if (!finite_d(v)) *bad = 1;
    }
    __syncthreads();
    if (tid == 0) {
        if (*bad_spd)
            st->err = GINGR_ERR_NOT_SPD;
        else if (*bad)
            st->err = GINGR_ERR_NONFINITE;
    }
}

template <int MODE>
__global__ __launch_bounds__(kSolveThreads) void posterior_solve_lds_kernel(int r, int rp, const double *__restrict__ G,
                                                                  const double *__restrict__ rhs,
                                                                  const double *__restrict__ zrand, double *__restrict__ a,
                                                                  DevState *__restrict__ st) {
    extern __shared__ double lds_sm[];
    __shared__ int bad_spd, bad;
#ifdef GINGR_SOLVE_TWICE
    for (int pass = 0; pass < 2; ++pass) {
        __syncthreads();
#endif
    posterior_solve_body<MODE == 0>(lds_sm, r, rp, G, rhs, zrand, a, st, &bad_spd, &bad);
#ifdef GINGR_SOLVE_TWICE
    }
#endif
}

constexpr int kWideSolveThreads = 512;

template <int SW>
struct WideSolveLds {
    double rdl[SW];
    double red[2][kWideSolveThreads / 64][SW];
    double xs[2][512];
    double yv[2][SW];
    int bad_spd;
};

template <int SW, bool HAS_S>
__device__ __forceinline__ void wide_solve_body(double *P, WideSolveLds<SW> &Ls, int r, int n, const double *__restrict__ G, double ca,
                                                const double *__restrict__ S, double cs, double ci, const double *__restrict__ b1,
                                                const double *__restrict__ b2, double cb, const double *__restrict__ zrand, double *gw) {
    constexpr int ldp = SW + 1, NW = kWideSolveThreads / 64;
    double *rdl = Ls.rdl;
    auto &red = Ls.red;
    auto &xs = Ls.xs;
    auto &yv = Ls.yv;
    int &bad_spd = Ls.bad_spd;
    const int tid = threadIdx.x, lane = tid & 63, wave = tid >> 6, l15 = lane & 15, l4 = lane >> 4;
    double *Lg = gw;
    double *rdg = gw + (size_t)(n + kNB) * n;
    const int nvec = zrand ? 2 : 1;
    if (tid == 0) bad_spd = 0;
    GINGR_STAGE_CLOCK(7)
    typedef double d2 __attribute__((ext_vector_type(2)));
    constexpr int NTJ = SW / 16;
    constexpr int TSTEP = NW / NTJ;
    constexpr int TACC = SW == 64 ? 9 : 9;
    constexpr int HALF = SW / 2;
    constexpr int RSTEP = kWideSolveThreads / HALF;
    constexpr int PRE = 17;
    const int wv = __builtin_amdgcn_readfirstlane(wave);
    const int my_tj = wv % NTJ, ti0 = wv / NTJ;
    for (int e = tid; e < kNB * n; e += kWideSolveThreads) Lg[(size_t)n * n + e] = e < r ? (b2 ? __builtin_fma(cb, b2[e], b1[e]) : b1[e]) : 0.0;
    __syncthreads();
    const int srow = tid / HALF, scp = tid % HALF;
    for (int kb = 0; kb < n; kb += SW) {
        const int sw = min(SW, n - kb), rows = n - kb + kNB;
        const int nti = rows >> 4, ntj = sw >> 4;
        v4f64 acc[TACC];
// ... 737 lines not shown
        return (brow == 0 && c < r) ? __builtin_fma(GINGR_COEFF_NOISE, rhs[c], qte[c]) : 0.0;
    }
};
__global__ __launch_bounds__(512) void logpdf_finish_kernel(int r, int n, int64_t Mp, const double *__restrict__ G, const double *__restrict__ rhs,
                                                            const double *__restrict__ Wn, const double *__restrict__ Wk, const double *__restrict__ Lk,
                                                            const int32_t *__restrict__ flag_n, const int32_t *__restrict__ flag_k,
                                                            double *__restrict__ fx, double *__restrict__ out2) {
    __shared__ double w[512], hv[2][512], red[512];
    const int tid = threadIdx.x;
    for (int k = tid; k < n; k += 512) w[k] = k < r ? Wk[k] : 0.0;
    __syncthreads();
    for (int kk = tid & 255; kk < r; kk += 256) {
        const int half = tid >> 8;
        const int j0 = half ? (r + 1) / 2 : 0, j1 = half ? r : (r + 1) / 2;
        double s0 = 0.0, s1 = 0.0, s2 = 0.0, s3 = 0.0;
        int j = j0;
        for (; j + 3 < j1; j += 4) {
            s0 = __builtin_fma(G[(int64_t)j * n + kk], w[j], s0);
            s1 = __builtin_fma(G[(int64_t)(j + 1) * n + kk], w[j + 1], s1);
            s2 = __builtin_fma(G[(int64_t)(j + 2) * n + kk], w[j + 2], s2);
            s3 = __builtin_fma(G[(int64_t)(j + 3) * n + kk], w[j + 3], s3);
        }
        for (; j < j1; ++j) s0 = __builtin_fma(G[(int64_t)j * n + kk], w[j], s0);
        hv[half][kk] = (s0 + s1) + (s2 + s3);
    }
    for (int64_t e = tid; e < (int64_t)n * n; e += 512) {
        const int64_t i = e / n, j = e - i * n;
        fx[e] = j <= i ? Lk[i * Mp + j] : 0.0;
    }
    for (int k = tid; k < n; k += 512) {
        fx[(int64_t)n * n + k] = k < r ? Wn[k] : 0.0;
        fx[(int64_t)n * n + n + k] = 1.0 / Lk[(int64_t)k * Mp + k];
    }
    __syncthreads();
    double part = 0.0;
    for (int k = tid; k < r; k += 512) {
        const double nw = (hv[0][k] + hv[1][k]) + w[k];
        part = __builtin_fma(w[k] - Wn[k], nw - rhs[k], part);
    }
    red[tid] = part;
    __syncthreads();
    for (int st2 = 256; st2 > 0; st2 >>= 1) {
        if (tid < st2) red[tid] += red[tid + st2];
        __syncthreads();
    }
    if (tid == 0) {
        const bool bad = *flag_n != 0 || *flag_k != 0;
        out2[0] = bad ? __builtin_nan("") : -0.5 * red[0] - 0.5 * (double)r * 1.8378770664093454836;
        out2[1] = bad ? 1.0 : 0.0;
    }
}
}

void launch_posterior_solve(gingr_ctx *ctx, int32_t r, int32_t rp, const double *G, const double *rhs, const double *zrand,
                            double *work, double *a, DevState *st) {
    TimerScope ts(ctx, 5);
    if (rp > 240 && !zrand) {
        const DenseSpdWork ws(rp, DenseSpdWork::kRhsRows);
        double *Aw = work + ws.aw(), *Linv = work + ws.linv(), *W = work + ws.w();
        int32_t *flag = reinterpret_cast<int32_t *>(work + ws.flag());
        launch_spd_system(ctx->stream, (int)r, ws, SpdIdentityPlus{G, (int)rp}, SpdRhsRow{rhs}, Aw, flag);
        dense_spd_solve3(ctx, Aw, ws.Mp, Linv, W, flag);
        hipLaunchKernelGGL(solve_finish_kernel, dim3(1), dim3(256), 0, ctx->stream, (int)r, (int)rp, W, flag, a, st);
        return;
    }
    if (r <= 128) {
        const bool fast = rp <= 112;
        const size_t lds = lds_solve_doubles(rp, fast ? 2 * kNB : kNB) * sizeof(double);
        auto go = [&](auto kern) {
            if (lds > 48 * 1024)
                set_dynamic_lds(kern, (size_t)(lds));
            hipLaunchKernelGGL(kern, dim3(1), dim3(kSolveThreads), lds, ctx->stream, (int)r, (int)rp, G, rhs, zrand, a, st);
        };
        if (fast)
            go(posterior_solve_lds_kernel<0>);
        else
            go(posterior_solve_lds_kernel<1>);
        return;
    }
    auto gow = [&](auto kern, int sw) {
        const size_t lds = (size_t)(rp + kNB) * (sw + 1) * sizeof(double);
        set_dynamic_lds(kern, (size_t)(lds));
        hipLaunchKernelGGL(kern, dim3(1), dim3(kWideSolveThreads), lds, ctx->stream, (int)r, (int)rp, G, rhs, zrand, a, st, work);
    };
    if (rp <= 256)
        gow(posterior_solve_wide_kernel<64>, 64);
    else
        gow(posterior_solve_wide_kernel<32>, 32);
}

namespace {
__global__ __launch_bounds__(1024) void posterior_solve_eig_kernel(int r, int rp, const double *__restrict__ V,
                                                                   const double *__restrict__ lam, const double *__restrict__ sigma2,
                                                                   const double *__restrict__ rhs, double *__restrict__ a, DevState *st) {
    __shared__ double x[512], t[512];
    __shared__ int bad;
    const int tid = threadIdx.x, lane16 = tid & 15, grp = tid >> 4;
    if (tid == 0) bad = 0;
    for (int k = tid; k < r; k += 1024) x[k] = rhs[k];
    __syncthreads();
    const double inv_s2 = 1.0 / sigma2[0];
    for (int k = grp; k < r; k += 64) {
        double s = 0.0;
        for (int i = lane16; i < r; i += 16) s = __builtin_fma(V[(int64_t)i * r + k], x[i], s);
        s = group16_sum(s);
        if (lane16 == 0) t[k] = s / (1.0 + lam[k] * inv_s2);
    }
    __syncthreads();
    for (int i = grp; i < rp; i += 64) {
        double s = 0.0;
        if (i < r)
            for (int k = lane16; k < r; k += 16) s = __builtin_fma(V[(int64_t)i * r + k], t[k], s);
        s = group16_sum(s);
        if (lane16 == 0) {
            a[i] = i < r ? s : 0.0;
            if (!finite_d(s)) bad = 1;
        }
    }
    __syncthreads();
    if (tid == 0 && bad) st->err = GINGR_ERR_NONFINITE;
}
}

void launch_posterior_solve_eig(gingr_ctx *ctx, int32_t r, int32_t rp, const double *eigV, const double *eigL, const double *sigma2,
                                const double *rhs, double *a, DevState *st) {
// ... 109 lines not shown
```

gingr_amd/csrc/gp_gram.hip:

```cpp
#include "gp.h"
#include "gp_device.h"

#include <algorithm>

namespace {

__global__ __launch_bounds__(256) void gram_kernel(const double *__restrict__ Q0, int64_t rows, int rp,
                                                   const double *__restrict__ weight, int64_t rows_per_slab, int nbp,
                                                   int row_stride, int offA, int offB, int full,
                                                   double *__restrict__ partial) {
    __shared__ double red[16 * 4 * 64];
    int pa = 0, pb = 0;
    if (full) {
        pa = blockIdx.y / nbp;
        pb = blockIdx.y - pa * nbp;
    } else {
        int t = blockIdx.y;
        for (pa = 0; pa < nbp; ++pa) {
            const int cnt = nbp - pa;
            if (t < cnt) {
                pb = pa + t;
                break;
            }
            t -= cnt;
// ... 43 lines not shown
        for (int t = 0; t < 4; ++t) {
            ca[t] = na[t];
            cb[t] = nb[t];
        }
    }
    for (int w = 1; w < 4; ++w) {
        __syncthreads();
        if (wave == w) {
#pragma unroll
            for (int i = 0; i < 4; ++i)
#pragma unroll
                for (int j = 0; j < 4; ++j)
#pragma unroll
                    for (int reg = 0; reg < 4; ++reg) red[((i * 4 + j) * 4 + reg) * 64 + lane] = acc[i][j][reg];
        }
        __syncthreads();
        if (wave == 0) {
#pragma unroll
            for (int i = 0; i < 4; ++i)
#pragma unroll
                for (int j = 0; j < 4; ++j)
#pragma unroll
                    for (int reg = 0; reg < 4; ++reg) acc[i][j][reg] += red[((i * 4 + j) * 4 + reg) * 64 + lane];
        }
    }
    if (wave != 0) return;
    double *out = partial + (int64_t)blockIdx.x * rp * rp;
#pragma unroll
    for (int i = 0; i < 4; ++i)
#pragma unroll
        for (int j = 0; j < 4; ++j) {
#pragma unroll
            for (int reg = 0; reg < 4; ++reg) {
                const int gi = pa * 64 + 4 * (kq + 4 * reg) + i;
                const int gj = pb * 64 + 4 * cl + j;
                if (gi < rp && gj < rp) out[(int64_t)gi * rp + gj] = acc[i][j][reg];
            }
        }
}

template <int NT>
__host__ __device__ constexpr int tri_row(int q) {
    int t = 0;
    while (q >= NT - t) q -= NT - t, ++t;
    return t;
}
template <int NT>
__host__ __device__ constexpr int tri_col(int q) {
    int t = 0;
    while (q >= NT - t) q -= NT - t, ++t;
    return t + q;
}

template <int NT, int HALF, bool FULL>
__device__ __forceinline__ void gram_tri_half(const double *__restrict__ Q0, int rp, const double *__restrict__ weight, int64_t r0,
                                              int64_t r1, int kgroup, int kq, int cl, int lane, double *red, double *xchg,
                                              double *__restrict__ out, const double *__restrict__ evec, int64_t npts,
                                              double *__restrict__ rhs_out, double *rsh) {
    constexpr int kTiles = NT * (NT + 1) / 2;
    constexpr int kMine = HALF == 0 ? (kTiles + 1) / 2 : kTiles / 2;
    constexpr int kM = kMine > 0 ? kMine : 1;
    v4f64 acc[kM];
#pragma unroll
    for (int q = 0; q < kMine; ++q) acc[q] = v4f64{0, 0, 0, 0};
    constexpr int kOwn = HALF == 0 ? (NT + 1) / 2 : NT / 2;
    constexpr int kO = kOwn > 0 ? kOwn : 1;
    const bool with_rhs = evec != nullptr;
    const bool with_w = weight != nullptr;
    const int kgu = __builtin_amdgcn_readfirstlane(kgroup);
    const int64_t ubase = r0 + 4 * kgu;
    const int64_t first = ubase + kq;
    const double *pclamp = Q0 + r0 * rp + cl;
    const double *pnext = Q0 + first * rp + cl;
    const int64_t pstep = 16 * (int64_t)rp;
    int64_t left_u = r1 - ubase;
    const int64_t pt_first = first / 3;
    const int rem_first = (int)(first - 3 * pt_first);
    constexpr unsigned kThird = 0x55555556u;
    unsigned third = (unsigned)rem_first * kThird;
    const double *wclamp = with_w ? weight + r0 / 3 : pclamp;
    const double *eclamp = with_rhs ? evec + r0 / 3 : pclamp;
    const double *wp = with_w ? weight + pt_first : pclamp;
    const double *ep = with_rhs ? evec + rem_first * npts + pt_first : pclamp;
    const int64_t estep = with_rhs ? 5 + npts : 0, ewrap = with_rhs ? 6 - 2 * npts : 0;
    double fn[2][kO], wn[2], en[2];
    int vrows[2];
    auto load_next = [&](auto slot) __attribute__((always_inline)) {
        constexpr int L = decltype(slot)::value;
        if (left_u >= 4) {
            vrows[L] = 4;
#pragma unroll
            for (int k = 0; k < kOwn; ++k) fn[L][k] = pnext[16 * (2 * k + HALF)];
            wn[L] = *wp;
            en[L] = *ep;
        } else {
            vrows[L] = (int)max((int64_t)0, left_u);
            const bool valid = left_u > kq;
            const double *p = valid ? pnext : pclamp;
#pragma unroll
            for (int k = 0; k < kOwn; ++k) fn[L][k] = p[16 * (2 * k + HALF)];
            wn[L] = *(valid ? wp : wclamp);
            en[L] = *(valid ? ep : eclamp);
        }
        left_u -= 16;
        pnext += pstep;
        const unsigned t2 = third + kThird;
        const bool wrap = t2 < third;
        third = t2;
        wp += wrap ? 6 : 5;
        ep += wrap ? ewrap : estep;
    };
    double racc[kO];
#pragma unroll
    for (int k = 0; k < kOwn; ++k) racc[k] = 0.0;
    const int64_t nsteps = (r1 - r0 + 15) / 16;
    constexpr int kBufStride = 4 * 2 * NT * 64;
    double *xbuf = xchg + (size_t)kgu * 2 * NT * 64 + lane;
    double cur[2][NT], a[2][NT];
    auto hand_over_write = [&](auto slot) __attribute__((always_inline)) {
        constexpr int L = decltype(slot)::value;
        double w = wn[L], e = en[L];
        if constexpr (!FULL) {
            w = with_w ? w : 1.0;
            e = with_rhs ? e : 0.0;
        }
        if (vrows[L] < 4) {
            asm volatile("; rows past the slab");
            const bool valid = vrows[L] > kq;
            w = valid ? w : 0.0;
            e = valid ? e : 0.0;
        }
#pragma unroll
        for (int k = 0; k < kOwn; ++k) {
            xbuf[L * kBufStride + (2 * k + HALF) * 64] = fn[L][k];
            xbuf[L * kBufStride + (NT + 2 * k + HALF) * 64] = fn[L][k] * w;
            racc[k] = __builtin_fma(fn[L][k], e, racc[k]);
        }
    };
    auto hand_over_read = [&](auto set) __attribute__((always_inline)) {
        constexpr int S = decltype(set)::value;
#pragma unroll
        for (int t = 0; t < NT; ++t) {
            cur[S][t] = xbuf[S * kBufStride + t * 64];
            a[S][t] = xbuf[S * kBufStride + (NT + t) * 64];
        }
    };
    auto mfmas = [&](auto set, auto begin, auto endq) __attribute__((always_inline)) {
        constexpr int S = decltype(set)::value;
        static_for<decltype(begin)::value, decltype(endq)::value>([&](auto m) {
            constexpr int mi = decltype(m)::value, q = 2 * mi + HALF, tr = tri_row<NT>(q), tc = tri_col<NT>(q);
            acc[mi] = __builtin_amdgcn_mfma_f64_16x16x4f64(a[S][tr], cur[S][tc], acc[mi], 0, 0, 0);
        });
    };
    using std::integral_constant;
    constexpr integral_constant<int, 0> c0{};
    constexpr integral_constant<int, 1> c1{};
    constexpr int kQ1 = kMine / 4, kQ2 = kMine / 2, kQ3 = (3 * kMine) / 4;
    load_next(c0);
    load_next(c1);
    hand_over_write(c0);
    __syncthreads();
    load_next(c0);
    hand_over_read(c0);
// ... 22 lines not shown
        step(c1);
    }
    if (st < nsteps) step(c0);
    __syncthreads();
    if (evec) {
#pragma unroll
        for (int k = 0; k < kOwn; ++k) {
            racc[k] += __shfl_xor(racc[k], 16);
            racc[k] += __shfl_xor(racc[k], 32);
        }
        if (kq == 0)
#pragma unroll
            for (int k = 0; k < kOwn; ++k) rsh[kgroup * (NT * 16) + (2 * k + HALF) * 16 + cl] = racc[k];
        __syncthreads();
        if (HALF == 0 && kgroup == 0 && kq == 0)
#pragma unroll
            for (int t = 0; t < NT; ++t) {
                const int c = t * 16 + cl;
                rhs_out[c] = ((rsh[c] + rsh[NT * 16 + c]) + rsh[2 * NT * 16 + c]) + rsh[3 * NT * 16 + c];
            }
    }
    static_assert(((kTiles + 1) / 2) * 2 * 256 <= 2 * kBufStride, "the exchange area must hold one slot of the K-group reduction");
    double *slot0 = red + HALF * ((kTiles + 1) / 2) * 256, *slot1 = xchg + HALF * ((kTiles + 1) / 2) * 256;
    auto put = [&](double *slot) {
#pragma unroll
        for (int q = 0; q < kMine; ++q)
#pragma unroll
            for (int reg = 0; reg < 4; ++reg) slot[(q * 4 + reg) * 64 + lane] = acc[q][reg];
    };
    auto add = [&](const double *slot) {
#pragma unroll
        for (int q = 0; q < kMine; ++q)
#pragma unroll
            for (int reg = 0; reg < 4; ++reg) acc[q][reg] += slot[(q * 4 + reg) * 64 + lane];
    };
    if (kgroup >= 2) put(kgroup == 2 ? slot0 : slot1);
    __syncthreads();
    if (kgroup < 2) add(kgroup == 0 ? slot0 : slot1);
    __syncthreads();
    if (kgroup == 1) put(slot0);
    __syncthreads();
    if (kgroup == 0) add(slot0);
    if (kgroup != 0) return;
    int q = 0;
#pragma unroll
    for (int t = 0; t < NT; ++t)
#pragma unroll
        for (int u = t; u < NT; ++u, ++q)
            if ((q & 1) == HALF)
#pragma unroll
                for (int reg = 0; reg < 4; ++reg) out[(int64_t)(16 * t + kq + 4 * reg) * rp + 16 * u + cl] = acc[q >> 1][reg];
}

template <int NT, bool FULL>
__global__ __launch_bounds__(512) void gram_tri_kernel(const double *__restrict__ Q0, int64_t rows, int rp,
                                                       const double *__restrict__ weight, int64_t rows_per_slab,
                                                       double *__restrict__ partial, const double *__restrict__ evec, int64_t npts,
                                                       double *__restrict__ rhs_partial, ZeroGate gate) {
    constexpr int kTiles = NT * (NT + 1) / 2;
    if (!gate_open(gate)) return;
    __shared__ double red[(kTiles + 1) * 256];
    __shared__ double xchg[2 * 4 * 2 * NT * 64];
    __shared__ double rsh[4 * NT * 16];
    const int wave = threadIdx.x >> 6, lane = threadIdx.x & 63, kq = lane >> 4, cl = lane & 15;
    const int64_t r0 = (int64_t)blockIdx.x * rows_per_slab;
    const int64_t r1 = min(rows, r0 + rows_per_slab);
    double *out = partial + (int64_t)blockIdx.x * rp * rp;
    double *rhs_out = rhs_partial ? rhs_partial + (int64_t)blockIdx.x * rp : nullptr;
    if ((wave >> 2) == 0)
        gram_tri_half<NT, 0, FULL>(Q0, rp, weight, r0, r1, wave & 3, kq, cl, lane, red, xchg, out, evec, npts, rhs_out, rsh);
    else
        gram_tri_half<NT, 1, FULL>(Q0, rp, weight, r0, r1, wave & 3, kq, cl, lane, red, xchg, out, evec, npts, rhs_out, rsh);
}

__global__ __launch_bounds__(256) void gram_reduce_kernel(const double *__restrict__ partial, int nslabs, int rp, int symmetric,
                                                          double *__restrict__ G) {
    __shared__ double sh[8][33];
    const int el = threadIdx.x & 31, g = threadIdx.x >> 5;
    const int idx = blockIdx.x * 32 + el;
    const int rr = rp * rp;
    const int i = idx / rp, j = idx - i * rp;
    const bool need = idx < rr && !(symmetric && i > j);
    double s = 0.0;
    if (need) {
        const double *p = partial + idx;
#pragma unroll 8
        for (int b = g; b < nslabs; b += 8) s += p[(int64_t)b * rr];
    }
    sh[g][el] = s;
    __syncthreads();
    if (g == 0 && need) {
        const double t = ((sh[0][el] + sh[1][el]) + (sh[2][el] + sh[3][el])) + ((sh[4][el] + sh[5][el]) + (sh[6][el] + sh[7][el]));
        G[i * rp + j] = t;
        if (symmetric) G[j * rp + i] = t;
    }
}

__global__ __launch_bounds__(256) void phase1_finalize_kernel(Phase1FinalizeArgs A) {
    __shared__ double sh[8][33];
    __shared__ double sv[256];
    const int rp = A.rp, rr = rp * rp;
    const int nG = (A.nslabs > 0 || A.scaled_src) ? (rr + 31) / 32 : 0;
    const int b = blockIdx.x;
    if (A.gate.counts && gate_open(A.gate)) {
        A.nslabs = A.alt_nslabs;
        A.scaled_src = nullptr;
        A.sweep_blocks = A.alt_nslabs;
    }
    if (b < nG) {
        const int el = threadIdx.x & 31, g = threadIdx.x >> 5;
        const int idx = b * 32 + el;
        if (A.nslabs <= 0) {
            if (g == 0 && idx < rr) A.G[idx] = A.scaled_contribute ? A.scaled_src[idx] * (1.0 / A.sigma2[0]) : 0.0;
            return;
        }
        const int i = idx / rp, j = idx - i * rp;
        const bool need = idx < rr && !(i > j);
        double s = 0.0;
        if (need) {
            const double *p = A.gram_partial + idx;
#pragma unroll 8
            for (int q = g; q < A.nslabs; q += 8) s += p[(int64_t)q * rr];
        }
        sh[g][el] = s;
        __syncthreads();
        if (g == 0 && need) {
            double t = ((sh[0][el] + sh[1][el]) + (sh[2][el] + sh[3][el])) + ((sh[4][el] + sh[5][el]) + (sh[6][el] + sh[7][el]));
            if (A.scaled_src)
                t = ((A.scaled_contribute ? A.scaled_src[idx] : 0.0) - t) * (1.0 / A.sigma2[0]);
            A.G[i * rp + j] = t;
            A.G[j * rp + i] = t;
        }
        return;
    }
    if (b < nG + rp) {
        const int k = b - nG;
        double s = 0.0;
        for (int q = threadIdx.x; q < A.sweep_blocks; q += 256) s += A.sweep_partial[(int64_t)q * rp + k];
        sv[threadIdx.x] = s;
        __syncthreads();
#pragma unroll
        for (int st = 128; st > 0; st >>= 1) {
            if ((int)threadIdx.x < st) sv[threadIdx.x] += sv[threadIdx.x + st];
            __syncthreads();
        }
        if (threadIdx.x == 0) A.rhs[k] = sv[0];
        return;
    }
    if (A.scalar_mode == 1) {
        const int map[4] = {1, 0, 2, 3};
        for (int q = 0; q < 4; ++q) {
            sv[threadIdx.x] = A.part[q * GINGR_SCALAR_BLOCKS + threadIdx.x];
            __syncthreads();
#pragma unroll
            for (int st = 128; st > 0; st >>= 1) {
                if ((int)threadIdx.x < st) sv[threadIdx.x] += sv[threadIdx.x + st];
                __syncthreads();
            }
            if (threadIdx.x == 0) {
                const double tot = sv[0];
                if (A.scalars_local) A.scalars_local[map[q]] = tot;
                A.sc8[map[q]] = (map[q] == 1 && !A.contribute_xpx) ? 0.0 : tot;
            }
            __syncthreads();
        }
        if (threadIdx.x >= 4 && threadIdx.x < 8) A.sc8[threadIdx.x] = 0.0;
    } else if (threadIdx.x < 8) {
        A.sc8[threadIdx.x] = 0.0;
    }
}

__global__ __launch_bounds__(256) void gram_downdate_kernel(const double *__restrict__ Q0, int64_t M, int rp, const double *__restrict__ weight,
                                                            int64_t verts_per_slab, double *__restrict__ partial, ZeroGate gate) {
    if (!gate_open(gate)) return;
    constexpr int kBatch = 4;
    int pa = 0, pb = 0;
    {
        const int np = (rp + 111) / 112;
        int t = blockIdx.y;
        for (pa = 0; pa < np; ++pa) {
            if (t < np - pa) {
                pb = pa + t;
                break;
            }
            t -= np - pa;
        }
    }
    const int ca0 = 112 * pa, cb0 = 112 * pb;
    __shared__ double q[kBatch][3][112], qb[kBatch][3][112];
    __shared__ unsigned long long zmask[16];
    const int tid = threadIdx.x, ti = tid >> 4, tj = tid & 15;
// ... 102 lines not shown
    gram_tri_plan(M, &nslabs_tri, &rps);
    const int64_t n = (int64_t)std::max(nslabs, nslabs_tri) * rp * rp;
    return rp >= 128 ? std::max(n, gram_wide_ws_doubles(M, rp)) : n;
}

int launch_gram(gingr_ctx *ctx, const double *Q0, int64_t M, int32_t rp, const double *weight, double *ws, double *G, const double *evec,
                double *rhs_partial, bool *rhs_done, const ZeroGate *gate) {
    if (rhs_done) *rhs_done = false;
    int nbp, npatch, nslabs;
    int64_t rps;
    gram_plan(M, rp, &nbp, &npatch, &nslabs, &rps);
    {
        const int nt = rp / 16;
        if (nt <= 7) {
            TimerScope ts(ctx, 2);
            gram_tri_plan(M, &nslabs, &rps);
            const bool fuse = evec && rhs_partial && rhs_done;
            if (fuse) *rhs_done = true;
            auto go = [&](auto kern) {
                hipLaunchKernelGGL(kern, dim3(nslabs), dim3(512), 0, ctx->stream, Q0, 3 * M, (int)rp, weight, rps, ws,
                                   fuse ? evec : (const double *)nullptr, M, fuse ? rhs_partial : (double *)nullptr, gate ? *gate : ZeroGate{});
            };
            const bool full = fuse && weight;
#define GINGR_GRAM_TRI(n) \
    case n: \
        if (full) go(gram_tri_kernel<n, true>); \
        else go(gram_tri_kernel<n, false>); \
        break;
            switch (nt) {
                GINGR_GRAM_TRI(1)
                GINGR_GRAM_TRI(2)
                GINGR_GRAM_TRI(3)
                GINGR_GRAM_TRI(4)
                GINGR_GRAM_TRI(5)
                GINGR_GRAM_TRI(6)
                default:
                    if (full) go(gram_tri_kernel<7, true>);
                    else go(gram_tri_kernel<7, false>);
                    break;
            }
#undef GINGR_GRAM_TRI
        } else {
            const bool fuse = evec && rhs_partial && rhs_done;
            if (fuse) *rhs_done = true;
            nslabs = launch_gram_wide(ctx, Q0, M, rp, weight, ws, fuse ? evec : nullptr, fuse ? rhs_partial : nullptr, gate);
        }
    }
    if (G)
        hipLaunchKernelGGL(gram_reduce_kernel, dim3((unsigned)ceil_div((int64_t)rp * rp, 32)), dim3(256), 0, ctx->stream, ws,
                           nslabs, (int)rp, 1, G);
    return nslabs;
}

int launch_gram_downdate(gingr_ctx *ctx, const double *Q0, int64_t M, int32_t rp, const double *weight, double *ws, const ZeroGate *gate) {
    int nslabs_tri;
    int64_t rows_per_slab;
    gram_tri_plan(M, &nslabs_tri, &rows_per_slab);
    const int64_t want = std::max<int64_t>(1, std::min<int64_t>(std::min(nslabs_tri, 128), ceil_div(M, 64)));
    const int64_t vps = ceil_div(M, want);
    const int nslabs = (int)ceil_div(M, vps);
    const int np = (rp + 111) / 112;
    hipLaunchKernelGGL(gram_downdate_kernel, dim3((unsigned)nslabs, (unsigned)(np * (np + 1) / 2)), dim3(256), 0, ctx->stream, Q0, M, (int)rp, weight,
                       vps, ws, gate ? *gate : ZeroGate{});
    return nslabs;
}

void launch_phase1_finalize(gingr_ctx *ctx, const Phase1FinalizeArgs &a) {
    const int nG = (a.nslabs > 0 || a.scaled_src) ? (a.rp * a.rp + 31) / 32 : 0;
    hipLaunchKernelGGL(phase1_finalize_kernel, dim3((unsigned)(nG + a.rp + 1)), dim3(256), 0, ctx->stream, a);
}

namespace {
__global__ __launch_bounds__(256) void moment_scatter_kernel(const double *__restrict__ T, int rp, MomentLayout ml, double *__restrict__ mom) {
    const int64_t idx = (int64_t)blockIdx.x * 256 + threadIdx.x;
    const int64_t w = 3 * (int64_t)rp;
    if (idx >= w * w) return;
    const int I = (int)(idx / w), J = (int)(idx - (int64_t)I * w);
    const int d = I / rp, a = I - d * rp, e = J / rp, b = J - e * rp;
    mom[ml.S(d, e) + (int64_t)a * rp + b] = T[idx];
}
__global__ __launch_bounds__(256) void transpose_kernel(const double *__restrict__ in, int rp, double *__restrict__ out) {
    const int idx = blockIdx.x * 256 + threadIdx.x;
    if (idx >= rp * rp) return;
    const int i = idx / rp, j = idx - i * rp;
    out[idx] = in[j * rp + i];
}
bool moments_as_rows(int32_t rp) { return 3 * rp >= 128 && 3 * rp <= 512; }
}

int64_t moment_grams_ws_doubles(int64_t M, int32_t rp) {
    if (moments_as_rows(rp)) return gram_rows_ws_doubles(M, 3 * rp) + 9 * (int64_t)rp * rp;
    return gram_ws_doubles(M, rp);
}

void launch_moment_grams(gingr_ctx *ctx, const double *Q0, int64_t M, int32_t rp, double *ws, double *mom) {
    const MomentLayout ml{rp};
    if (moments_as_rows(rp)) {
        const int32_t w = 3 * rp;
        double *T = ws + gram_rows_ws_doubles(M, w);
        const int nslabs = launch_gram_rows(ctx, Q0, M, w, ws);
        hipLaunchKernelGGL(gram_reduce_kernel, dim3((unsigned)ceil_div((int64_t)w * w, 32)), dim3(256), 0, ctx->stream, ws, nslabs, (int)w, 1, T);
        hipLaunchKernelGGL(moment_scatter_kernel, dim3((unsigned)ceil_div((int64_t)w * w, 256)), dim3(256), 0, ctx->stream, T, (int)rp, ml, mom);
        return;
    }
    int nbp, npatch, nslabs;
    int64_t rps;
// ... 15 lines not shown
```

gingr_amd/csrc/gp_sweep.hip:

```cpp
#include "gp.h"
#include "gp_device.h"

#include <algorithm>

namespace {

__global__ __launch_bounds__(256) void interp_pack_kernel(const double *__restrict__ Qs, int32_t rp, const int32_t *__restrict__ inv_src,
                                                          const int32_t *__restrict__ ids, const double *__restrict__ w,
                                                          const int32_t *__restrict__ perm_new, int64_t row_begin, int64_t M,
                                                          double *__restrict__ Q0) {
    const int64_t idx = (int64_t)blockIdx.x * 256 + threadIdx.x;
    if (idx >= 3 * M * rp) return;
    const int64_t row = idx / rp;
    const int32_t q = (int32_t)(idx - row * rp);
    const int64_t s = row / 3;
    const int d = (int)(row - 3 * s);
    const int64_t o = row_begin + perm_new[s];
    double acc = 0.0;
#pragma unroll
    for (int k = 0; k < 3; ++k) {
        const double wk = w[3 * o + k];
        if (wk != 0.0) acc += wk * Qs[((int64_t)3 * inv_src[ids[3 * o + k]] + d) * rp + q];
    }
    Q0[idx] = acc;
// ... 165 lines not shown
        if (TRANS) {
            if (!valid) e[0] = e[1] = e[2] = 0.0;
#pragma unroll
            for (int m = 0; m < KMAX; ++m) {
                if (m < km) {
                    const int k = m * 16;
                    acc[m] = __builtin_fma(q0[k], e[0], __builtin_fma(q1[k], e[1], __builtin_fma(q2[k], e[2], acc[m])));
                }
            }
        }
    }
    if (TRANS) {
        __syncthreads();
#pragma unroll
        for (int m = 0; m < KMAX; ++m)
            if (m < km) red[grp * rp + m * 16 + lane16] = acc[m];
        __syncthreads();
        for (int k = tid; k < rp; k += kSweepThreads) {
            double s = 0.0;
            for (int g = 0; g < kGroups; ++g) s += red[g * rp + k];
            a.partial[(int64_t)blockIdx.x * rp + k] = s;
        }
    }
    if (MODE == SWEEP_SHAPES) {
        __syncthreads();
        if (lane16 == 0)
            for (int s = 0; s < 16; ++s) red[grp * 16 + s] = us[s];
        __syncthreads();
        if (tid < 24) {
            double s = 0.0;
            if (tid < 16)
                for (int g = 0; g < kGroups; ++g) s += red[g * 16 + tid];
            a.partial[(int64_t)blockIdx.x * 24 + tid] = s;
        }
    }
}

__global__ __launch_bounds__(256) void block_partials_reduce_kernel(const double *__restrict__ partial, int nblocks, int width,
                                                                    double *__restrict__ out) {
    __shared__ double sh[256];
    const int k = blockIdx.x;
    double s = 0.0;
    for (int b = threadIdx.x; b < nblocks; b += 256) s += partial[(int64_t)b * width + k];
    sh[threadIdx.x] = s;
    __syncthreads();
#pragma unroll
    for (int st = 128; st > 0; st >>= 1) {
        if ((int)threadIdx.x < st) sh[threadIdx.x] += sh[threadIdx.x + st];
        __syncthreads();
    }
    if (threadIdx.x == 0) out[k] = sh[0];
}

template <int KM, int S>
__global__ __launch_bounds__(kSweepThreads) void sweep_fit_boxes_kernel(SweepArgs a) {
    constexpr int CH = KM < 8 ? KM : 8;
    static_assert(4 % S == 0, "points per group and round");
    extern __shared__ double lds[];
    const int tid = threadIdx.x, lane16 = tid & 15, grp = tid >> 4;
    const int rp = a.rp, km = rp >> 4;
    const int64_t M = a.M;
    double *coef = lds, *red = lds + rp;
    for (int k = tid; k < rp; k += kSweepThreads) coef[k] = a.coef0[k];
    double R[9], tr[3], cen[3];
    for (int q = 0; q < 9; ++q) R[q] = a.state->R[q];
    for (int q = 0; q < 3; ++q) {
        tr[q] = a.state->t[q];
        cen[q] = a.state->center[q];
    }
    const double scale = a.state->scale;
    double cf[KM];
    __syncthreads();
#pragma unroll
    for (int m = 0; m < KM; ++m) cf[m] = m < km ? coef[m * 16 + lane16] : 0.0;
    double amax = 0.0;
    for (int64_t qd = blockIdx.x; qd * 64 < M; qd += gridDim.x) {
        double lo[3] = {__builtin_huge_val(), __builtin_huge_val(), __builtin_huge_val()};
        double hi[3] = {-__builtin_huge_val(), -__builtin_huge_val(), -__builtin_huge_val()};
#pragma unroll
        for (int s0 = 0; s0 < 4; s0 += S) {
            double facc[S][3], rm[S][3];
#pragma unroll
            for (int s = 0; s < S; ++s)
#pragma unroll
                for (int d = 0; d < 3; ++d) facc[s][d] = 0.0;
#pragma unroll
            for (int mc = 0; mc < KM; mc += CH) {
                double u[S][3][CH];
#pragma unroll
                for (int s = 0; s < S; ++s) {
                    const int64_t p = qd * 64 + (s0 + s) * kGroups + grp;
                    const int64_t pc = p < M ? p : 0;
                    const double *q0 = a.Q0 + (3 * pc) * rp + lane16;
#pragma unroll
                    for (int d = 0; d < 3; ++d) {
#pragma unroll
                        for (int m = 0; m < CH; ++m) u[s][d][m] = (mc + m < KM && mc + m < km) ? q0[d * rp + (mc + m) * 16] : 0.0;
                        if (mc == 0) rm[s][d] = a.ref[d * M + pc] + a.mean[d * M + pc];
                    }
                }
#pragma unroll
                for (int s = 0; s < S; ++s)
#pragma unroll
                    for (int d = 0; d < 3; ++d)
#pragma unroll
                        for (int m = 0; m < CH; ++m)
                            if (mc + m < KM) facc[s][d] = __builtin_fma(u[s][d][m], cf[mc + m], facc[s][d]);
            }
#pragma unroll
            for (int s = 0; s < S; ++s) {
                const int64_t p = qd * 64 + (s0 + s) * kGroups + grp;
                double f[3];
#pragma unroll
                for (int d = 0; d < 3; ++d) f[d] = group16_sum(facc[s][d]);
                const double ix = rm[s][0] + f[0] - cen[0], iy = rm[s][1] + f[1] - cen[1], iz = rm[s][2] + f[2] - cen[2];
                const double nx = scale * (R[0] * ix + R[1] * iy + R[2] * iz + cen[0] + tr[0]);
                const double ny = scale * (R[3] * ix + R[4] * iy + R[5] * iz + cen[1] + tr[1]);
                const double nz = scale * (R[6] * ix + R[7] * iy + R[8] * iz + cen[2] + tr[2]);
                if (p < M) {
                    if (lane16 == 0) {
                        a.shape_out[p] = nx;
                        a.shape_out[M + p] = ny;
                        a.shape_out[2 * M + p] = nz;
                    }
                    lo[0] = fmin(lo[0], nx), lo[1] = fmin(lo[1], ny), lo[2] = fmin(lo[2], nz);
                    hi[0] = fmax(hi[0], nx), hi[1] = fmax(hi[1], ny), hi[2] = fmax(hi[2], nz);
                }
            }
        }
        if (lane16 == 0) {
#pragma unroll
            for (int d = 0; d < 3; ++d) {
                red[grp * 8 + d] = lo[d];
                red[grp * 8 + 3 + d] = hi[d];
            }
        }
        __syncthreads();
        if (tid < 6) {
            double v = red[tid];
            for (int g = 1; g < kGroups; ++g) v = tid < 3 ? fmin(v, red[g * 8 + tid]) : fmax(v, red[g * 8 + tid]);
            a.qboxes[qd * 6 + tid] = v;
            red[kGroups * 8 + tid] = fabs(v - a.box_centre[tid % 3]);
        }
        __syncthreads();
        if (tid == 0)
            for (int q = 0; q < 6; ++q) amax = fmax(amax, red[kGroups * 8 + q]);
        __syncthreads();
    }
    if (tid == 0 && a.absmax_slot) {
        const unsigned long long mb = __builtin_bit_cast(unsigned long long, amax);
        if (mb > __hip_atomic_load(reinterpret_cast<unsigned long long *>(a.absmax_slot), __ATOMIC_RELAXED, __HIP_MEMORY_SCOPE_AGENT))
            atomicMax(reinterpret_cast<unsigned long long *>(a.absmax_slot), mb);
    }
}

}

int sweep_num_blocks(int64_t M) {
    const int64_t nb = ceil_div(M, kGroups);
    return (int)(nb < kSweepMaxBlocks ? (nb > 0 ? nb : 1) : kSweepMaxBlocks);
}

int64_t sweep_ws_doubles(int64_t M, int32_t rp) {
    const int w = rp > 24 ? rp : 24;
    return (int64_t)sweep_num_blocks(M) * w;
}

template <int MODE>
static void launch_sweep_mode(gingr_ctx *ctx, const SweepArgs &a, int width) {
    if (MODE == SWEEP_FIT && a.qboxes && a.rp <= 512) {
        const int nq = (int)std::min<int64_t>(4096, ceil_div(a.M, 64));
        const size_t l2 = (size_t)(a.rp + kGroups * 8 + 8) * sizeof(double);
        TimerScope ts(ctx, 4);
        if (a.rp <= 64)
            hipLaunchKernelGGL((sweep_fit_boxes_kernel<4, 4>), dim3(nq), dim3(kSweepThreads), l2, ctx->stream, a);
        else if (a.rp <= 112)
            hipLaunchKernelGGL((sweep_fit_boxes_kernel<7, 4>), dim3(nq), dim3(kSweepThreads), l2, ctx->stream, a);
        else if (a.rp <= 128)
            hipLaunchKernelGGL((sweep_fit_boxes_kernel<8, 4>), dim3(nq), dim3(kSweepThreads), l2, ctx->stream, a);
        else if (a.rp <= 192)
            hipLaunchKernelGGL((sweep_fit_boxes_kernel<12, 1>), dim3(nq), dim3(kSweepThreads), l2, ctx->stream, a);
        else if (a.rp <= 256)
            hipLaunchKernelGGL((sweep_fit_boxes_kernel<16, 1>), dim3(nq), dim3(kSweepThreads), l2, ctx->stream, a);
        else if (a.rp <= 384)
            hipLaunchKernelGGL((sweep_fit_boxes_kernel<24, 1>), dim3(nq), dim3(kSweepThreads), l2, ctx->stream, a);
        else
            hipLaunchKernelGGL((sweep_fit_boxes_kernel<32, 1>), dim3(nq), dim3(kSweepThreads), l2, ctx->stream, a);
        return;
    }
    const int nb = sweep_num_blocks(a.M);
    const size_t lds = (size_t)(2 * a.rp + kGroups * (a.rp > 16 ? a.rp : 16)) * sizeof(double);
    TimerScope ts(ctx, 4);
    if (a.rp <= 128) {
        hipLaunchKernelGGL((sweep_kernel<MODE, 8>), dim3(nb), dim3(kSweepThreads), lds, ctx->stream, a);
    } else {
        if (lds > 48 * 1024)
            set_dynamic_lds(&sweep_kernel<MODE, 32>, (size_t)(lds));
        hipLaunchKernelGGL((sweep_kernel<MODE, 32>), dim3(nb), dim3(kSweepThreads), lds, ctx->stream, a);
    }
    ts.stop();
    if (width > 0 && !a.no_reduce)
        hipLaunchKernelGGL(block_partials_reduce_kernel, dim3((unsigned)width), dim3(256), 0, ctx->stream, a.partial, nb,
                           width, a.out);
}

void launch_sweep(gingr_ctx *ctx, SweepMode mode, const SweepArgs &a) {
    switch (mode) {
        case SWEEP_RHS: launch_sweep_mode<SWEEP_RHS>(ctx, a, a.rp); break;
        case SWEEP_PROJ1: launch_sweep_mode<SWEEP_PROJ1>(ctx, a, a.rp); break;
        case SWEEP_SHAPES: launch_sweep_mode<SWEEP_SHAPES>(ctx, a, 24); break;
        case SWEEP_PROJ2: launch_sweep_mode<SWEEP_PROJ2>(ctx, a, a.rp); break;
        case SWEEP_FIT: launch_sweep_mode<SWEEP_FIT>(ctx, a, 0); break;
        case SWEEP_POSED: launch_sweep_mode<SWEEP_POSED>(ctx, a, 0); break;
        case SWEEP_RHS_ICP: launch_sweep_mode<SWEEP_RHS_ICP>(ctx, a, a.rp); break;
    }
}

void launch_interp_pack(gingr_ctx *ctx, const double *Qs, int32_t rp, const int32_t *inv_src, const int32_t *ids, const double *w,
                        const int32_t *perm_new, int64_t row_begin, int64_t M, double *Q0) {
    const int64_t total = 3 * M * rp;
    hipLaunchKernelGGL(interp_pack_kernel, dim3((unsigned)ceil_div(total, 256)), dim3(256), 0, ctx->stream, Qs, rp, inv_src, ids, w,
                       perm_new, row_begin, M, Q0);
}
void launch_pack_basis(gingr_ctx *ctx, const double *stage_colmajor, const double *variance_dev, int64_t M, int32_t r,
                       int32_t rp, const int32_t *perm, double *Q0) {
    const int64_t total = 3 * M * rp;
    hipLaunchKernelGGL(pack_basis_kernel, dim3((unsigned)ceil_div(total, 256)), dim3(256), 0, ctx->stream, stage_colmajor,
// ... 3 lines not shown
```

gingr_amd/csrc/group.hip:

```cpp
#include "gp.h"

#include <algorithm>
#include <atomic>
#include <condition_variable>
#include <functional>
#include <mutex>
#include <thread>

namespace {

constexpr int kMaxGroup = 16;

struct PeerPtrs {
    const double *p[kMaxGroup];
};

__global__ __launch_bounds__(256) void peer_sum_kernel(double *__restrict__ out, PeerPtrs src, int n, int64_t count) {
    const int64_t i = ((int64_t)blockIdx.x * 256 + threadIdx.x) * 2;
    if (i + 1 < count) {
        double2 s = *reinterpret_cast<const double2 *>(src.p[0] + i);
        for (int q = 1; q < n; ++q) {
            const double2 v = *reinterpret_cast<const double2 *>(src.p[q] + i);
            s.x += v.x;
            s.y += v.y;
// ... 216 lines not shown
        int64_t count = 0;
        std::vector<double *> mom((size_t)n, nullptr), tmp((size_t)n, nullptr);
        auto release = [&]() {
            for (int r = 0; r < n; ++r)
                if (tmp[(size_t)r]) {
                    (void)hipSetDevice(g->dev[(size_t)r]);
                    (void)hipFree(tmp[(size_t)r]);
                }
        };
        for (int r = 0; r < n; ++r) {
            void *p = nullptr;
            int64_t c = 0;
            GINGR_TRY(gingr_model_gram_exchange(g->model[(size_t)r], &p, &c));
            if (r == 0) count = c;
            if (c != count) return group_fail(g, GINGR_ERR_STATE, "group: shards disagree on the model rank");
            mom[(size_t)r] = static_cast<double *>(p);
        }
        for (int r = 0; r < n; ++r) {
            void *buf = nullptr;
            bool fine = false;
            if (hipSetDevice(g->dev[(size_t)r]) != hipSuccess) {
                release();
                return group_fail(g, GINGR_ERR_HIP, "group: hipSetDevice failed");
            }
            const int rc = alloc_peer_readable(g, (size_t)count * sizeof(double), &buf, &fine);
            if (rc) {
                release();
                return rc;
            }
            tmp[(size_t)r] = static_cast<double *>(buf);
        }
        int rc = g->run([&](int r) {
            gingr_ctx *ctx = g->ctx[(size_t)r];
            if (hipMemcpyAsync(tmp[(size_t)r], mom[(size_t)r], (size_t)count * sizeof(double), hipMemcpyDeviceToDevice, ctx->stream) != hipSuccess)
                return gingr_set_error(ctx, GINGR_ERR_HIP, "group: moment copy failed");
            return gingr_ctx_synchronize(ctx);
        });
        if (!rc)
            rc = g->run([&](int r) {
                gingr_ctx *ctx = g->ctx[(size_t)r];
                PeerPtrs src;
                for (int q = 0; q < n; ++q) src.p[q] = tmp[(size_t)q];
                hipLaunchKernelGGL(peer_sum_kernel, dim3((unsigned)ceil_div(ceil_div(count, 2), 256)), dim3(256), 0, ctx->stream,
                                   mom[(size_t)r], src, n, count);
                if (hipGetLastError() != hipSuccess) return gingr_set_error(ctx, GINGR_ERR_HIP, "group: moment all-reduce launch failed");
                return gingr_ctx_synchronize(ctx);
            });
        release();
        if (rc) return rc;
        GINGR_TRY(g->run([&](int r) { return gingr_model_finalize(g->ctx[(size_t)r], g->model[(size_t)r]); }));
    }
    g->rank = gingr_model_rank(g->model[0]);
    g->fit.assign((size_t)n, nullptr);
    return g->run([&](int r) { return gingr_fitter_create(g->ctx[(size_t)r], g->model[(size_t)r], &g->fit[(size_t)r]); });
}

int exchange_buffers(gingr_group *g, int r, std::vector<hipEvent_t> &ev, const std::vector<double *> &src_base, int64_t src_off, double *dst,
                     int64_t count, bool ok, bool gather_rows = false) {
    gingr_ctx *ctx = g->ctx[(size_t)r];
    int rc = GINGR_OK;
    if (ok && hipEventRecord(ev[(size_t)r], ctx->stream) != hipSuccess) rc = gingr_set_error(ctx, GINGR_ERR_HIP, "group: hipEventRecord failed");
    g->bar.wait();
    if (!ok || rc) return rc;
    PeerPtrs src;
    for (int q = 0; q < g->n; ++q) {
        if (q != r && hipStreamWaitEvent(ctx->stream, ev[(size_t)q], 0) != hipSuccess)
            return gingr_set_error(ctx, GINGR_ERR_HIP, "group: hipStreamWaitEvent failed");
        src.p[q] = src_base[(size_t)q] + src_off;
    }
    if (gather_rows) {
        RowBounds rb;
        for (int q = 0; q < g->n; ++q) rb.b[q] = g->begin[(size_t)q];
        rb.b[g->n] = g->M_total;
        hipLaunchKernelGGL(peer_gather_rows_kernel, dim3((unsigned)ceil_div(g->M_total, 256)), dim3(256), 0, ctx->stream, dst, src, rb, g->n, g->M_total);
    } else {
        hipLaunchKernelGGL(peer_sum_kernel, dim3((unsigned)ceil_div(ceil_div(count, 2), 256)), dim3(256), 0, ctx->stream, dst, src, g->n, count);
    }
    if (hipGetLastError() != hipSuccess) return gingr_set_error(ctx, GINGR_ERR_HIP, "group: all-reduce kernel launch failed");
    return GINGR_OK;
}
int exchange_segment(gingr_group *g, int r, int s, int parity, bool ok) {
    return exchange_buffers(g, r, g->ready[parity][s], g->send[parity], g->off[s], g->xch[(size_t)r] + g->off[s], g->cnt[s], ok);
}
int timed_exchange_segment(gingr_group *g, int r, int s, int parity, bool ok) {
    TimerScope ts(g->ctx[(size_t)r], 6 + s);
    return exchange_segment(g, r, s, parity, ok);
}
int exchange_fullfit(gingr_group *g, int r, int parity, bool ok) {
    return exchange_buffers(g, r, g->readyfit[parity], g->sendfit[parity], 0, fitter_fullfit(g->fit[(size_t)r]), 3 * g->M_total, ok, true);
}
int exchange_revsum(gingr_group *g, int r, int parity, bool ok) {
    return exchange_buffers(g, r, g->readyrev[parity], g->sendrev[parity], 0, fitter_revsum(g->fit[(size_t)r]), 4 * g->M_total, ok);
}

bool group_flavour(const Correspondence &c) { return correspondence_error(c) != CorrespondenceError::BadFlavour && c.kind != Flavour::Pairs; }

int group_update(gingr_group *g, const Correspondence &c, int32_t n_iterations, const double *z) {
    if (!g || n_iterations < 0 || !group_flavour(c)) return GINGR_ERR_BAD_ARGUMENT;
    if (g->fit.empty() || !g->fit[0] || g->xch.empty()) return group_fail(g, GINGR_ERR_STATE, "group update: no model / target set");
    const bool gather = needs_gathered_fit(c, g->reversed);
    if (gather && !g->meshes) return group_fail(g, GINGR_ERR_STATE, "group update: no meshes set (gingr_group_set_meshes)");
    if (z && n_iterations != 1) return group_fail(g, GINGR_ERR_BAD_ARGUMENT, "group update: a sampled proposal is one iteration");
    if (g->n == 1)
        return g->run([&](int) { return z ? fitter_sample_update(g->fit[0], c, z) : fitter_update(g->fit[0], c, n_iterations); });
    const int64_t it0 = g->iteration;
    g->iteration += n_iterations;
    return g->run([&](int r) {
// ... 405 lines not shown
```

gingr_amd/csrc/model.hip:

```cpp
#include "fitter.h"

#include <algorithm>
#include <cmath>
#include <functional>

namespace {

__global__ __launch_bounds__(256) void unpack_basis_kernel(const double *__restrict__ Q0, const double *__restrict__ variance,
                                                           int64_t M, int32_t r, int32_t rp,
                                                           const int32_t *__restrict__ perm, double *__restrict__ stage) {
    const int64_t idx = (int64_t)blockIdx.x * 256 + threadIdx.x;
    if (idx >= 3 * M * r) return;
    const int64_t row = idx / r;
    const int32_t k = (int32_t)(idx - row * r);
    const int64_t s = row / 3, d = row - 3 * s;
    const double sd = sqrt(variance[k]);
    stage[(int64_t)k * 3 * M + 3 * (int64_t)(perm ? perm[s] : s) + d] = sd > 0.0 ? Q0[row * rp + k] / sd : 0.0;
}

__global__ __launch_bounds__(256) void truncate_basis_kernel(const double *__restrict__ Qs, int32_t rps, int64_t rows, int32_t k, int32_t rpn,
                                                             double *__restrict__ Q) {
    const int64_t idx = (int64_t)blockIdx.x * 256 + threadIdx.x;
    if (idx >= rows * rpn) return;
    const int64_t row = idx / rpn;
    const int32_t q = (int32_t)(idx - row * rpn);
    Q[idx] = q < k ? Qs[row * rps + q] : 0.0;
}

int model_finalize_impl(gingr_ctx *ctx, gingr_model *m) {
    DevBuf work, flag;
    HIP_TRY(ctx, work.alloc((size_t)binv_work_doubles(m->rp) * sizeof(double)));
    HIP_TRY(ctx, flag.alloc(sizeof(int32_t)));
    launch_binv(ctx, m->r, m->rp, m->mom, work.as<double>(), m->Binv, flag.as<int32_t>());
    GINGR_TRY(check_launch(ctx));
    int32_t err = 0;
    HIP_TRY(ctx, hipMemcpyAsync(&err, flag.p, sizeof(err), hipMemcpyDeviceToHost, ctx->stream));
    HIP_TRY(ctx, hipStreamSynchronize(ctx->stream));
    if (err) return gingr_set_error(ctx, GINGR_ERR_NOT_SPD, "model finalize: Q^T Q / 1e-5 + I is not positive definite");
    const MomentLayout ml{m->rp};
    const int64_t rr = (int64_t)m->rp * m->rp;
    launch_small_gemm(ctx, m->r, m->rp, m->Binv, m->mom + ml.stot(), 1.0 / GINGR_COEFF_NOISE, m->cmat);
    for (int d = 0; d < 3; ++d)
        for (int e = 0; e < 3; ++e) {
            launch_small_gemm(ctx, m->r, m->rp, m->Binv, m->mom + ml.S(d, e), 1.0, m->cmat + (1 + d * 3 + e) * rr);
            launch_small_gemm(ctx, m->r, m->rp, m->mom + ml.S(d, e), m->cmat, 1.0, work.as<double>());
            launch_small_gemm(ctx, m->r, m->rp, m->Binv, work.as<double>(), 1.0, m->cmat + (10 + d * 3 + e) * rr);
        }
    const PostVec pvl{m->rp};
    launch_postvec(ctx, m->r, m->rp, m->Binv, m->mom + ml.V(0, 0), m->pvec);
    {
        double cst[16];
        for (int q = 0; q < 9; ++q) cst[q] = m->Pp[q];
        for (int q = 0; q < 3; ++q) {
            cst[9 + q] = m->Ps[q];
            cst[12 + q] = m->c0[q];
        }
        cst[15] = (double)m->M_total;
        HIP_TRY(ctx, hipMemcpyAsync(m->pvec + pvl.consts(), cst, sizeof(cst), hipMemcpyHostToDevice, ctx->stream));
        HIP_TRY(ctx, hipStreamSynchronize(ctx->stream));
    }
    GINGR_TRY(check_launch(ctx));
    m->eig_ready = false;
    if (m->r <= kSymEigColsMaxN) {
        if (launch_jacobi_eig(ctx, m->mom + ml.stot(), m->rp, m->r, m->eigL, m->eigV) == GINGR_OK)
            m->eig_ready = true;
        else
            (void)hipGetLastError();
    }
    HIP_TRY(ctx, hipStreamSynchronize(ctx->stream));
    m->finalized = true;
    return GINGR_OK;
}

}


int model_create_impl(gingr_ctx *ctx, int64_t M_total, int32_t rank, const double *ref, const double *mean,
                      const double *variance, int64_t row_begin, int64_t row_end,
                      const std::function<int(gingr_model *)> &fill_basis, gingr_model **out, bool finalize) {
    if (!ctx || !out) return GINGR_ERR_BAD_ARGUMENT;
    *out = nullptr;
    if (M_total < 1 || rank < 1 || rank > 512 || !ref || !mean || !variance)
// ... 90 lines not shown
            }
        if (hipGetLastError() != hipSuccess || hipStreamSynchronize(ctx->stream) != hipSuccess)
            return fail(gingr_set_error(ctx, GINGR_ERR_HIP, "model_upload: kernel launch failed"));
    }
    for (int q = 0; q < 9; ++q) m->Pp[q] = 0.0;
    for (int q = 0; q < 3; ++q) m->Ps[q] = 0.0;
    if (M != M_total) {
        m->h_full_pts.resize((size_t)3 * M_total);
        for (int64_t i = 0; i < 3 * M_total; ++i) m->h_full_pts[(size_t)i] = ref[i] + mean[i];
    }
    for (int64_t i = 0; i < M_total; ++i) {
        double pt[3];
        for (int d = 0; d < 3; ++d) pt[d] = ref[3 * i + d] + mean[3 * i + d] - m->c0[d];
        for (int d = 0; d < 3; ++d) {
            m->Ps[d] += pt[d];
            for (int e = 0; e < 3; ++e) m->Pp[d * 3 + e] += pt[d] * pt[e];
        }
    }
    if (row_begin == 0 && row_end == M_total && finalize) {
        rc = model_finalize_impl(ctx, m);
        if (rc) return fail(rc);
    }
    *out = m;
    return GINGR_OK;
}

extern "C" {

int gingr_model_upload(gingr_ctx *ctx, int64_t M_total, int32_t rank, const double *ref, const double *mean,
                       const double *basis_colmajor, const double *variance, int64_t row_begin, int64_t row_end,
                       gingr_model **out) {
    if (!ctx || !out) return GINGR_ERR_BAD_ARGUMENT;
    *out = nullptr;
    if (!basis_colmajor) return gingr_set_error(ctx, GINGR_ERR_BAD_ARGUMENT, "model_upload: basis is null");
    DevBuf stage, var;
    auto fill = [&](gingr_model *m) -> int {
        const int64_t M = m->M;
        if (stage.alloc((size_t)3 * M * rank * sizeof(double)) != hipSuccess || var.alloc(rank * sizeof(double)) != hipSuccess)
            return gingr_set_error(ctx, GINGR_ERR_HIP, "model_upload: out of device memory");
        if (hipMemcpy2DAsync(stage.p, (size_t)3 * M * sizeof(double), basis_colmajor + 3 * row_begin,
                             (size_t)3 * M_total * sizeof(double), (size_t)3 * M * sizeof(double), (size_t)rank,
                             hipMemcpyHostToDevice, ctx->stream) != hipSuccess)
            return gingr_set_error(ctx, GINGR_ERR_HIP, "model_upload: basis copy failed");
        (void)hipMemcpyAsync(var.p, variance, rank * sizeof(double), hipMemcpyHostToDevice, ctx->stream);
        launch_pack_basis(ctx, stage.as<double>(), var.as<double>(), M, rank, m->rp, m->perm, m->Q0);
        return GINGR_OK;
    };
    return model_create_impl(ctx, M_total, rank, ref, mean, variance, row_begin, row_end, fill, out);
}

void gingr_model_destroy(gingr_model *m) {
    if (!m) return;
    if (m->ctx) (void)hipSetDevice(m->ctx->device);
    void *ptrs[] = {m->Q0, m->ref, m->mean, m->mom, m->Binv, m->eigV, m->eigL, m->cmat, m->pvec, m->perm, m->iperm};
    for (void *p : ptrs) dev_free(p);
    delete m;
}

int64_t gingr_model_num_points(const gingr_model *m) { return m ? m->M : 0; }
int32_t gingr_model_rank(const gingr_model *m) { return m ? m->r : 0; }

int gingr_model_gram_exchange(gingr_model *m, void **dev_ptr, int64_t *count) {
    if (!m || !dev_ptr || !count) return GINGR_ERR_BAD_ARGUMENT;
    *dev_ptr = m->mom;
    *count = MomentLayout{m->rp}.total();
    return GINGR_OK;
}

int gingr_model_finalize(gingr_ctx *ctx, gingr_model *m) {
    if (!ctx || !m) return GINGR_ERR_BAD_ARGUMENT;
    HIP_TRY(ctx, hipSetDevice(ctx->device));
    return model_finalize_impl(ctx, m);
}

static void fill_scalars(gingr_state_scalars *s, const double euler[3], const double center[3], const double translation[3],
                         double scale) {
    memset(s, 0, sizeof(*s));
    for (int q = 0; q < 3; ++q) {
        s->euler[q] = euler[q];
        s->center[q] = center[q];
        s->translation[q] = translation[q];
    }
    s->scale = scale;
    s->sigma2 = 1.0;
}

}

int model_observation_system(gingr_ctx *ctx, const gingr_model *model, const double euler[3], const double center[3],
                             const double translation[3], const double *obs_xyz, const double *weight, int32_t n_lm, const int32_t *lm_pid,
                             const double *lm_xyz, const double *lm_cov, gingr_fitter **f_out, DevBuf &sys) {
    gingr_fitter *f = nullptr;
    GINGR_TRY(gingr_fitter_create(ctx, model, &f));
    const int64_t M = model->M;
    const int32_t r = model->r, rp = model->rp;
    int rc = GINGR_OK;
    std::vector<double> zero((size_t)r, 0.0);
    gingr_state_scalars s;
    fill_scalars(&s, euler, center, translation, 1.0);
    rc = gingr_fitter_set_state(f, zero.data(), &s);
    if (!rc) rc = gingr_fitter_set_landmarks(f, n_lm, lm_pid, lm_xyz, lm_cov);
    DevBuf aos, obs, win, gws;
    if (!rc && (aos.alloc((size_t)3 * M * sizeof(double)) != hipSuccess || obs.alloc((size_t)3 * M * sizeof(double)) != hipSuccess ||
                win.alloc((size_t)M * sizeof(double)) != hipSuccess ||
                sys.alloc(((size_t)rp * rp + rp) * sizeof(double)) != hipSuccess ||
                gws.alloc((size_t)gram_ws_doubles(M, rp) * sizeof(double)) != hipSuccess))
        rc = gingr_set_error(ctx, GINGR_ERR_HIP, "out of memory");
    if (!rc) {
        std::vector<double> wo((size_t)M), wh((size_t)M);
// ... 225 lines not shown
```

gingr_amd/csrc/solve_blocks.h:

```cpp
#pragma once

#include "common.h"
#include "gp_device.h"

constexpr int kNB = 16;

#ifndef GINGR_STAGE_CLOCK
#define GINGR_STAGE_CLOCK(slot)
#endif


template <int J>
__device__ __forceinline__ double row_bcast(double v) {
    double out;
    asm volatile("s_nop 1\n\tv_mov_b64_dpp %0, %1 row_newbcast:%2 row_mask:0xf bank_mask:0xf" : "=v"(out) : "v"(v), "n"(J));
    return out;
}

template <int J, bool FRESH>
__device__ __forceinline__ void fmac_row_bcast(double &acc, double a, double b) {
    if (FRESH)
        asm volatile("s_nop 1\n\tv_fmac_f64_dpp %0, %1, %2 row_newbcast:%3 row_mask:0xf bank_mask:0xf"
                     : "+v"(acc)
                     : "v"(a), "v"(b), "n"(J));
    else
        asm volatile("v_fmac_f64_dpp %0, %1, %2 row_newbcast:%3 row_mask:0xf bank_mask:0xf" : "+v"(acc) : "v"(a), "v"(b), "n"(J));
}

template <int K>
__device__ __forceinline__ void panel_step4(double (&x)[4], double rdl, double nl) {
    double t0, t1, t2, t3;
    asm volatile(
        "v_mul_f64 %4, %0, %8\n\t"
        "v_mul_f64 %5, %1, %8\n\t"
        "v_mul_f64 %6, %2, %8\n\t"
        "v_mul_f64 %7, %3, %8\n\t"
        "v_fmac_f64_dpp %0, %4, %9 row_newbcast:%10 row_mask:0xf bank_mask:0xf\n\t"
        "v_fmac_f64_dpp %1, %5, %9 row_newbcast:%10 row_mask:0xf bank_mask:0xf\n\t"
        "v_fmac_f64_dpp %2, %6, %9 row_newbcast:%10 row_mask:0xf bank_mask:0xf\n\t"
        "v_fmac_f64_dpp %3, %7, %9 row_newbcast:%10 row_mask:0xf bank_mask:0xf"
        : "+v"(x[0]), "+v"(x[1]), "+v"(x[2]), "+v"(x[3]), "=&v"(t0), "=&v"(t1), "=&v"(t2), "=&v"(t3)
        : "v"(rdl), "v"(nl), "n"(K));
}

__device__ __forceinline__ double row16_sum_dpp(double v) {
    auto step = [&](auto ctrl) {
        constexpr int c = decltype(ctrl)::value;
        const unsigned long long b = __builtin_bit_cast(unsigned long long, v);
        const int lo = __builtin_amdgcn_update_dpp(0, (int)(unsigned)b, c, 0xf, 0xf, false);
        const int hi = __builtin_amdgcn_update_dpp(0, (int)(unsigned)(b >> 32), c, 0xf, 0xf, false);
        v += __builtin_bit_cast(double, ((unsigned long long)(unsigned)hi << 32) | (unsigned)lo);
    };
    step(std::integral_constant<int, 0xB1>{});
    step(std::integral_constant<int, 0x4E>{});
    step(std::integral_constant<int, 0x141>{});
    step(std::integral_constant<int, 0x140>{});
    return v;
}


__host__ __device__ inline int solve_ld(int n) { return n | 1; }
__host__ __device__ inline size_t lds_solve_doubles(int rp, int xr) { return (size_t)(rp + xr) * solve_ld(rp) + 2 * (size_t)rp; }

template <int NT, bool HAS_S = false>
__device__ __forceinline__ void lds_load_spd(double *A, int ld, int r, int n, const double *__restrict__ G, double ca,
                                             const double *__restrict__ S, double cs, double ci) {
    const int tid = threadIdx.x, tx = tid & 15, ty = tid >> 4;
    constexpr int RB = NT / 16;
    if (RB == 16 && n <= 128) {
        double v[36], vs[HAS_S ? 36 : 1];
        int idx = 0;
#pragma unroll
        for (int bi = 0; bi < 8; ++bi)
#pragma unroll
            for (int bj = 0; bj <= bi; ++bj, ++idx) {
                const int i = bi * 16 + ty, j = bj * 16 + tx;
                const int g = min(min(i, r - 1), n - 1) * n + min(j, r - 1);
                v[idx] = G[g];
                if (HAS_S) vs[idx] = S[g];
            }
        idx = 0;
#pragma unroll
        for (int bi = 0; bi < 8; ++bi)
#pragma unroll
            for (int bj = 0; bj <= bi; ++bj, ++idx) {
                double t = ca * v[idx];
                if (HAS_S) t = __builtin_fma(cs, vs[idx], t);
                v[idx] = t;
            }
        idx = 0;
#pragma unroll
        for (int bi = 0; bi < 8; ++bi)
#pragma unroll
            for (int bj = 0; bj <= bi; ++bj, ++idx) {
                const int i = bi * 16 + ty, j = bj * 16 + tx;
                if (bi * 16 < n && j <= i) {
                    double t = v[idx];
                    if (i == j) t += ci;
                    A[i * ld + j] = (i < r && j < r) ? t : (i == j ? 1.0 : 0.0);
                }
            }
        __syncthreads();
        return;
    }
    int ib = 0, jb = 0;
    while (ib < n) {
        double v[8];
        int off[8];
#pragma unroll
        for (int u = 0; u < 8; ++u) {
            const int i = ib + ty, j = jb + tx;
            const int g = min(i, r - 1) * n + min(j, r - 1);
            double t = ca * G[g];
            if (HAS_S) t = __builtin_fma(cs, S[g], t);
            if (i == j) t += ci;
            v[u] = (i < r && j < r) ? t : (i == j ? 1.0 : 0.0);
            off[u] = (ib < n && i < n && j <= i) ? i * ld + j : -1;
            jb += 16;
            if (jb > ib + RB - 16 || jb >= n) {
                jb = 0;
                ib += RB;
            }
        }
#pragma unroll
        for (int u = 0; u < 8; ++u)
            if (off[u] >= 0) A[off[u]] = v[u];
    }
    __syncthreads();
}

template <int NT, bool IDENT = false>
__device__ __forceinline__ void lds_cholesky(double *A, int ld, int n, double *rd, int *bad_spd, int xr, int wr = 0) {
    const int tid = threadIdx.x, lane = tid & 63, wave = tid >> 6;
    constexpr int NW = NT / 64;
    constexpr int PU = NT >= 1024 ? 2 : 4;
    constexpr int PR = (NT / 16) * PU;
    const int rows_all = n + xr;
    auto diag_block = [&](int kb) {
        const int l15 = lane & 15;
        double row[kNB];
#pragma unroll
        for (int k = 0; k < kNB; ++k) row[k] = A[(kb + l15) * ld + kb + k];
        static_for<0, kNB>([&](auto cc) {
            constexpr int c = decltype(cc)::value;
            const double d = row_bcast<c>(row[c]);
// ... 201 lines not shown
```

gingr_amd/models.py:

```python
from __future__ import annotations

import ctypes
import dataclasses
from ctypes import c_int64, c_void_p
from typing import Optional, Sequence, Tuple

import numpy as np

from . import _native as nat
from ._native import f64, dptr, iptr
from .context import Context, _check


@dataclasses.dataclass
class PointDistributionModel:
    reference: np.ndarray
    mean: np.ndarray
    basis: np.ndarray
    variance: np.ndarray
    cells: Optional[np.ndarray] = None

    @property
    def rank(self) -> int:
        return int(self.variance.shape[0])
# ... 523 lines not shown
                                                            int(row_end), ctypes.byref(h)), "gingr_model_upload")
            self.handle = h
        self.row_begin, self.row_end = int(row_begin), int(row_end)
        self.M_local = self.row_end - self.row_begin
        self.rank = int(self._lib.gingr_model_rank(self.handle))

    @classmethod
    def _adopt(cls, ctx: Context, handle, model, M: int) -> "DeviceModel":
        self = cls.__new__(cls)
        self.ctx, self._lib, self.host, self.handle, self._owner = ctx, ctx._lib, model, handle, True
        self.row_begin, self.row_end, self.M_local = 0, M, M
        self.rank = int(self._lib.gingr_model_rank(handle))
        return self

    def truncate(self, k: int) -> "DeviceModel":
        if isinstance(self.host, PointDistributionModel):
            host = self.host.truncate(k)
            h = c_void_p()
            _check(self.ctx.handle, self._lib.gingr_model_truncate(self.ctx.handle, self.handle, int(k), ctypes.byref(h)), "gingr_model_truncate")
            return DeviceModel._adopt(self.ctx, h, host, host.numberOfPoints)
        return TruncatedDevicePointDistributionModel(self, k, cells=getattr(self.host, "cells", None)).device()

    def _augment_native(self, other: "DeviceModel", relativeTolerance: float, maxRank: int):
        if not isinstance(other, DeviceModel):
            raise TypeError("augment: the other model must be a DeviceModel")
        h, info = c_void_p(), nat.AugmentInfo()
        _check(self.ctx.handle, self._lib.gingr_model_augment(self.ctx.handle, self.handle, other.handle, float(relativeTolerance), int(maxRank),
                                                              ctypes.byref(h), ctypes.byref(info)), "gingr_model_augment")
        return h, AugmentInfo(int(info.columns), int(info.rank), float(info.total_variance), float(info.kept_variance))

    def augment(self, other: "DeviceModel", relativeTolerance: float = 1e-10, maxRank: int = 0) -> "DeviceModel":
        h, info = self._augment_native(other, relativeTolerance, maxRank)
        cells = _cells_of(self)
        return AugmentedDevicePointDistributionModel(self.ctx, None, None, cells=cells if cells is not None else _cells_of(other), _handle=h,
                                                     _info=info).device()

    def download(self, basis: bool = True) -> "PointDistributionModel":
        M, r = self.M_local, self.rank
        ref, mean, var = np.empty((M, 3)), np.empty((M, 3)), np.empty(r)
        U = np.empty((3 * M, r), order="F") if basis else None
        _check(self.ctx.handle, self._lib.gingr_model_download(self.ctx.handle, self.handle, dptr(ref), dptr(mean),
                                                               U.ctypes.data_as(nat._dp) if basis else None, dptr(var)),
               "gingr_model_download")
        return PointDistributionModel(reference=ref, mean=mean, basis=U, variance=var)

    def gram_exchange(self) -> Tuple[int, int]:
        p, n = c_void_p(), c_int64()
        _check(self.ctx.handle, self._lib.gingr_model_gram_exchange(self.handle, ctypes.byref(p), ctypes.byref(n)), "gram_exchange")
        return p.value, n.value

    def finalize(self):
        _check(self.ctx.handle, self._lib.gingr_model_finalize(self.ctx.handle, self.handle), "gingr_model_finalize")

    def close(self):
        if getattr(self, "handle", None):
            if self._owner and getattr(self.ctx, "handle", None):
                self._lib.gingr_model_destroy(self.handle)
            self.handle = None

    def __del__(self):
        try:
            self.close()
        except Exception:
            pass

    def instance(self, alpha, euler=(0, 0, 0), center=(0, 0, 0), translation=(0, 0, 0), scale: float = 1.0) -> np.ndarray:
        a, e, c, t = f64(alpha), f64(euler), f64(center), f64(translation)
        out = np.empty((self.M_local, 3))
        _check(self.ctx.handle, self._lib.gingr_model_instance(self.ctx.handle, self.handle, dptr(a), dptr(e), dptr(c), dptr(t),
                                                               float(scale), dptr(out)), "gingr_model_instance")
        return out

    def coefficients(self, mesh, euler=(0, 0, 0), center=(0, 0, 0), translation=(0, 0, 0)) -> np.ndarray:
        m, e, c, t = f64(mesh), f64(euler), f64(center), f64(translation)
        out = np.empty(self.rank)
        _check(self.ctx.handle, self._lib.gingr_model_coefficients(self.ctx.handle, self.handle, dptr(e), dptr(c), dptr(t),
                                                                   dptr(m), dptr(out)), "gingr_model_coefficients")
        return out

    def posterior_mean(self, obs_points, weights, euler=(0, 0, 0), center=(0, 0, 0), translation=(0, 0, 0),
                       landmarks: Optional["LandmarkCorrespondences"] = None) -> Tuple[np.ndarray, np.ndarray]:
        o, w, e, c, t = f64(obs_points), f64(weights), f64(euler), f64(center), f64(translation)
        mean = np.empty((self.M_local, 3))
        coeffs = np.empty(self.rank)
        n, lp, lx, lc = _landmarks_native(landmarks)
        _check(self.ctx.handle, self._lib.gingr_model_posterior_mean(
            self.ctx.handle, self.handle, dptr(e), dptr(c), dptr(t), dptr(o), dptr(w), n, iptr(lp), dptr(lx), dptr(lc),
            dptr(mean), dptr(coeffs)), "gingr_model_posterior_mean")
        return mean, coeffs

    def posterior(self, obs_points, weights, euler=(0, 0, 0), center=(0, 0, 0), translation=(0, 0, 0),
                  landmarks: Optional["LandmarkCorrespondences"] = None) -> "DeviceModel":
        o, w, e, c, t = f64(obs_points), f64(weights), f64(euler), f64(center), f64(translation)
        n, lp, lx, lc = _landmarks_native(landmarks)
        h = c_void_p()
        _check(self.ctx.handle, self._lib.gingr_model_posterior(
            self.ctx.handle, self.handle, dptr(e), dptr(c), dptr(t), dptr(o), dptr(w), n, iptr(lp), dptr(lx), dptr(lc),
            ctypes.byref(h)), "gingr_model_posterior")
        return PosteriorDevicePointDistributionModel(self.ctx, h, cells=getattr(self.host, "cells", None)).device()

    def _factor(self, factor):
        if factor is None:
            return None
        W = f64(factor)
        if W.shape != (self.rank, self.rank):
            raise ValueError(f"factor must be ({self.rank}, {self.rank}), row-major")
# ... 17 lines not shown
```

include/gingr_hip.h:

```cpp
#ifndef GINGR_HIP_H
#define GINGR_HIP_H

#include <stddef.h>
#include <stdint.h>

#ifdef __cplusplus
extern "C" {
#endif

typedef struct gingr_ctx gingr_ctx;
typedef struct gingr_model gingr_model;
typedef struct gingr_fitter gingr_fitter;

typedef enum gingr_status {
    GINGR_OK = 0,
    GINGR_ERR_BAD_ARGUMENT = 1,
    GINGR_ERR_HIP = 2,
    GINGR_ERR_NONFINITE = 3,
    GINGR_ERR_NOT_SPD = 4,
    GINGR_ERR_NO_DEVICE = 5,
    GINGR_ERR_STATE = 6,
    GINGR_ERR_NOT_CONVERGED = 7
} gingr_status;

typedef enum gingr_global_transform {
    GINGR_NO_TRANSFORMS = 0,
    GINGR_RIGID_TRANSFORMS = 1,
    GINGR_SIMILARITY_TRANSFORMS = 2
} gingr_global_transform;

typedef enum gingr_fitting_status {
    GINGR_FIT_NONE = 0,
    GINGR_FIT_CONVERGED = 1,
    GINGR_FIT_MAX_ITERATION = 2,
    GINGR_FIT_MODEL_FLEXIBILITY_ERROR = 3
} gingr_fitting_status;


int gingr_device_count(void);
int gingr_ctx_create(int device, gingr_ctx **out);
void gingr_ctx_destroy(gingr_ctx *ctx);
const char *gingr_last_error(const gingr_ctx *ctx);
int gingr_ctx_set_stream(gingr_ctx *ctx, void *hip_stream);
void *gingr_ctx_get_stream(gingr_ctx *ctx);
int gingr_ctx_synchronize(gingr_ctx *ctx);
const char *gingr_build_info(void);
typedef enum gingr_ctx_option {
    GINGR_OPT_CULL = 0,
    GINGR_OPT_FINE_CULL = 1,
    GINGR_OPT_NN_GRID = 2,
    GINGR_OPT_TRI_GRID = 3,
    GINGR_OPT_SPLIT_EXCHANGE = 4,
    GINGR_OPT_GRAM_DOWNDATE = 5,
    GINGR_OPT_DECIMATE_BATCH = 6
} gingr_ctx_option;
int gingr_ctx_set_option(gingr_ctx *ctx, int32_t option, int32_t value);
int gingr_ctx_get_option(gingr_ctx *ctx, int32_t option, int32_t *value);


int gingr_cpd_stats(gingr_ctx *ctx, int64_t M, const double *fit, int64_t N, const double *target, double sigma2,
                    double w, double *den, double *P1, double *PX, double *Pt1, double *scalars);

int gingr_cpd_initial_sigma2(gingr_ctx *ctx, int64_t M, const double *ref, int64_t N, const double *target,
                             double *sigma2_out);

int gingr_nn(gingr_ctx *ctx, int64_t M, const double *query, int64_t N, const double *target, int32_t *idx,
             double *d2, double *mean_distance);

int gingr_gauss_block(gingr_ctx *ctx, int64_t na, const double *A, int64_t nb, const double *B, double sigma,
                      double scaling, double *out);

int gingr_model_upload(gingr_ctx *ctx, int64_t M_total, int32_t rank, const double *ref, const double *mean,
                       const double *basis_colmajor, const double *variance, int64_t row_begin, int64_t row_end,
                       gingr_model **out);
void gingr_model_destroy(gingr_model *model);
int gingr_model_gram_exchange(gingr_model *model, void **dev_ptr, int64_t *count);
int gingr_model_finalize(gingr_ctx *ctx, gingr_model *model);
int gingr_gpmm_build_gaussian(gingr_ctx *ctx, int64_t M_total, const double *ref, int32_t n_kernels, const double *sigmas,
                              const double *scalings, double relative_tolerance, int32_t max_rank, int64_t row_begin,
                              int64_t row_end, gingr_model **out);
#define GINGR_KERNEL_GAUSSIAN_MIXTURE 0
#define GINGR_KERNEL_DOT 1
#define GINGR_KERNEL_LOOKUP 2
typedef struct gingr_scalar_kernel {
    int32_t kind;
    int32_t n_kernels;
    const double *sigmas;
    const double *scalings;
    double mirror;
    double scaling;
    const double *lookup;
} gingr_scalar_kernel;
int gingr_gpmm_build_diagonal(gingr_ctx *ctx, int64_t M_total, const double *ref, const gingr_scalar_kernel *kx,
                              const gingr_scalar_kernel *ky, const gingr_scalar_kernel *kz, double relative_tolerance,
                              int32_t max_rank, int64_t row_begin, int64_t row_end, gingr_model **out);
#define GINGR_GPMM_MAX_COLUMNS 1536
typedef struct gingr_gpmm_info {
    int32_t columns;
    int32_t rank;
    int32_t tolerance_reached;
    double residual_fraction;
    double kept_variance_fraction;
} gingr_gpmm_info;
int gingr_gpmm_build_diagonal_ex(gingr_ctx *ctx, int64_t M_total, const double *ref, const gingr_scalar_kernel *kx,
                                 const gingr_scalar_kernel *ky, const gingr_scalar_kernel *kz, double relative_tolerance,
                                 int32_t max_columns, int32_t keep_rank, int64_t row_begin, int64_t row_end, gingr_gpmm_info *info,
                                 gingr_model **out);
int gingr_model_truncate(gingr_ctx *ctx, const gingr_model *src, int32_t k, gingr_model **out);
int gingr_pointset_distance_extrema(gingr_ctx *ctx, const double *xyz, int64_t n, double *max_distance, double *min_distance);
int gingr_model_download(gingr_ctx *ctx, const gingr_model *model, double *ref, double *mean, double *basis_colmajor,
                         double *variance);
int64_t gingr_model_num_points(const gingr_model *model);
int32_t gingr_model_rank(const gingr_model *model);

int gingr_model_instance(gingr_ctx *ctx, const gingr_model *model, const double *alpha, const double euler[3],
                         const double center[3], const double translation[3], double scale, double *out_xyz);

int gingr_model_coefficients(gingr_ctx *ctx, const gingr_model *model, const double euler[3], const double center[3],
                             const double translation[3], const double *mesh_xyz, double *alpha);

int gingr_model_posterior_mean(gingr_ctx *ctx, const gingr_model *model, const double euler[3], const double center[3],
                               const double translation[3], const double *obs_xyz, const double *weight,
                               int32_t n_lm, const int32_t *lm_pid, const double *lm_xyz, const double *lm_cov,
                               double *mean_xyz, double *coeffs);

typedef struct gingr_state_scalars {
    double euler[3];
    double center[3];
    double translation[3];
    double scale;
    double sigma2;
    int32_t iteration;
    int32_t status;
} gingr_state_scalars;

typedef struct gingr_cpd_params {
    double w;
    double lambda;
} gingr_cpd_params;

typedef struct gingr_icp_params {
    double initial_sigma;
    double end_sigma;
    int32_t max_iterations;
} gingr_icp_params;

int gingr_fitter_create(gingr_ctx *ctx, const gingr_model *model, gingr_fitter **out);
void gingr_fitter_destroy(gingr_fitter *f);
int gingr_fitter_set_target(gingr_fitter *f, int64_t N, const double *target_xyz);
int gingr_fitter_set_landmarks(gingr_fitter *f, int32_t n_lm, const int32_t *lm_pid, const double *lm_xyz,
                               const double *lm_cov);
int gingr_fitter_set_options(gingr_fitter *f, int32_t global_transform, double step_length);
int gingr_fitter_set_stop_threshold(gingr_fitter *f, double threshold);
int gingr_fitter_stop_rule_hit(gingr_fitter *f, int32_t *hit);
int gingr_fitter_last_update_error(gingr_fitter *f, int32_t *code);
int gingr_fitter_set_state(gingr_fitter *f, const double *alpha, const gingr_state_scalars *s);
int gingr_fitter_get_state(gingr_fitter *f, double *alpha, gingr_state_scalars *s, double *fit_xyz);
int gingr_fitter_get_cpd_stats(gingr_fitter *f, double *P1, double *PX, double *den, double *scalars6);
int gingr_fitter_get_icp_idx(gingr_fitter *f, int32_t *idx, double *d2);

int gingr_fitter_update_cpd_async(gingr_fitter *f, const gingr_cpd_params *p, int32_t n_iterations);
int gingr_fitter_update_icp_async(gingr_fitter *f, const gingr_icp_params *p, int32_t n_iterations);

int gingr_fitter_set_meshes(gingr_fitter *f, int64_t n_model_triangles, const int32_t *model_triangles,
                            int64_t n_target_triangles, const int32_t *target_triangles);
int gingr_fitter_set_surface_method(gingr_fitter *f, int32_t method);
// ... 259 lines not shown
```

Baseline: 455.7 iterations/s.

## Exploit axis-separable GPMM basis with compact per-axis Gram and block solves

At model finalize, the code detects whether each basis column is nonzero in only one coordinate axis. If so, it builds a compact per-axis basis copy (up to 48 columns per axis). CPD updates on an unsharded model then compute a compact Gram, solve three small Cholesky systems in parallel blocks instead of one rank-100 solve, and use the compact basis when refreshing the fit. This cuts Gram FLOPs and solve cost when the kernel is diagonal per axis, at the price of extra memory and a finalize-time detection pass.

```diff
diff --git a/gingr_amd/_native.py b/gingr_amd/_native.py
--- a/gingr_amd/_native.py
+++ b/gingr_amd/_native.py
@@ -72,6 +72,7 @@
 
 KERNEL_GAUSSIAN_MIXTURE, KERNEL_DOT, KERNEL_LOOKUP = 0, 1, 2
 OPT_CULL, OPT_FINE_CULL, OPT_NN_GRID, OPT_TRI_GRID, OPT_SPLIT_EXCHANGE, OPT_GRAM_DOWNDATE, OPT_DECIMATE_BATCH = 0, 1, 2, 3, 4, 5, 6
+OPT_SEPARABLE = 7
 
 
 class ScalarKernel(ctypes.Structure):
@@ -191,6 +192,7 @@
     "gingr_model_download": (c_int, [c_void_p, c_void_p, _dp, _dp, _dp, _dp]),
     "gingr_model_num_points": (c_int64, [c_void_p]),
     "gingr_model_rank": (c_int32, [c_void_p]),
+    "gingr_model_separable": (c_int, [c_void_p, _ip, _ip, _ip]),
     "gingr_model_instance": (c_int, [c_void_p, c_void_p, _dp, _dp, _dp, _dp, c_double, _dp]),
     "gingr_model_coefficients": (c_int, [c_void_p, c_void_p, _dp, _dp, _dp, _dp, _dp]),
     "gingr_model_posterior_mean": (c_int, [c_void_p, c_void_p, _dp, _dp, _dp, _dp, _dp, c_int32, _ip, _dp, _dp, _dp, _dp]),
diff --git a/gingr_amd/csrc/common.h b/gingr_amd/csrc/common.h
--- a/gingr_amd/csrc/common.h
+++ b/gingr_amd/csrc/common.h
@@ -39,6 +39,7 @@
     int32_t rccl_world = 0, rccl_rank = 0;
     int split_exchange = 0;
     int gram_downdate = -1;
+    int separable = -1;
     int decimate_batch = 16;
     hipStream_t side_stream = nullptr, exchange_stream = nullptr;
     hipEvent_t split_ev[2] = {nullptr, nullptr};
diff --git a/gingr_amd/csrc/context.hip b/gingr_amd/csrc/context.hip
--- a/gingr_amd/csrc/context.hip
+++ b/gingr_amd/csrc/context.hip
@@ -154,6 +154,7 @@
         case GINGR_OPT_SPLIT_EXCHANGE: ctx->split_exchange = value != 0; return GINGR_OK;
         case GINGR_OPT_GRAM_DOWNDATE: ctx->gram_downdate = value < 0 ? -1 : (value != 0); return GINGR_OK;
         case GINGR_OPT_DECIMATE_BATCH: ctx->decimate_batch = value < 1 ? 1 : (value > 60 ? 60 : value); return GINGR_OK;
+        case GINGR_OPT_SEPARABLE: ctx->separable = value < 0 ? -1 : 0; return GINGR_OK;
         default: return gingr_set_error(ctx, GINGR_ERR_BAD_ARGUMENT, "ctx_set_option: unknown option %d", option);
     }
 }
@@ -168,6 +169,7 @@
         case GINGR_OPT_SPLIT_EXCHANGE: *value = ctx->split_exchange; return GINGR_OK;
         case GINGR_OPT_GRAM_DOWNDATE: *value = ctx->gram_downdate; return GINGR_OK;
         case GINGR_OPT_DECIMATE_BATCH: *value = ctx->decimate_batch; return GINGR_OK;
+        case GINGR_OPT_SEPARABLE: *value = ctx->separable; return GINGR_OK;
         default: return gingr_set_error(ctx, GINGR_ERR_BAD_ARGUMENT, "ctx_get_option: unknown option %d", option);
     }
 }
diff --git a/gingr_amd/csrc/fitter.h b/gingr_amd/csrc/fitter.h
--- a/gingr_amd/csrc/fitter.h
+++ b/gingr_amd/csrc/fitter.h
@@ -94,7 +94,8 @@
         std::vector<double> v;
         int flavour = -1;
         double p0 = 0, p1 = 0;
-        bool same(const Key &o) const { return flavour == o.flavour && p0 == o.p0 && p1 == o.p1 && v == o.v; }
+        bool compact = false;
+        bool same(const Key &o) const { return flavour == o.flavour && p0 == o.p0 && p1 == o.p1 && compact == o.compact && v == o.v; }
     };
     Key state_key, post_key;
     bool state_key_valid = false;
@@ -130,6 +131,7 @@
         nf_valid[0] = nf_valid[1] = false;
     }
     double *partial_out = nullptr;
+    bool group_member = false;
     double *fullfit = nullptr, *partial_fullfit = nullptr;
     int32_t *zero_counts = nullptr;
     double *gstage = nullptr;
@@ -180,7 +182,7 @@
 int check_ready(gingr_fitter *f);
 int check_parameters(gingr_fitter *f, const Correspondence &c);
 SweepArgs base_args(const gingr_fitter *f);
-void refresh_fit(gingr_fitter *f);
+void refresh_fit(gingr_fitter *f, bool compact = false);
 void fit_boxes_now(gingr_fitter *f);
 std::vector<double> state_key_values(int32_t r, const double *alpha, const double euler[3], const double center[3], const double t[3],
                                      double scale, double sigma2);
diff --git a/gingr_amd/csrc/fitter.hip b/gingr_amd/csrc/fitter.hip
--- a/gingr_amd/csrc/fitter.hip
+++ b/gingr_amd/csrc/fitter.hip
@@ -63,11 +63,12 @@
     f->fit_boxes_valid = true;
 }
 
-void refresh_fit(gingr_fitter *f) {
+void refresh_fit(gingr_fitter *f, bool compact) {
     SweepArgs a = base_args(f);
     a.coef0 = f->alpha;
     a.shape_out = f->fit;
     if (f->fboxes && f->m->rp <= 512 && f->cpd_seen) {
+        if (compact) a.Qc = f->m->Qc, a.sep_map = f->m->sep_map;
         a.qboxes = f->fboxes + 6 * ceil_div(f->m->M, 256);
         a.box_centre = f->absmax + 2;
         a.absmax_slot = f->absmax + 1;
@@ -300,6 +301,7 @@
     mx(ceil_div(nn_ws_bytes(M, N), 8));
     mx(ceil_div(nn_ws_bytes(N, M), 8));
     mx(gram_ws_doubles(M, rp) + sweep_ws_doubles(M, rp));
+    if (f->m->Qc) mx(gram_compact_ws_doubles(M));
     f->ws_doubles = w;
     GINGR_TRY(dev_alloc(ctx, &f->ws, (size_t)w));
     const int64_t big = M > N ? M : N;
@@ -577,6 +579,7 @@
 }
 
 void fitter_set_partial_output(gingr_fitter *f, double *base) { f->partial_out = base; }
+void fitter_set_group_member(gingr_fitter *f) { f->group_member = true; }
 void fitter_set_partial_fullfit(gingr_fitter *f, double *base) { f->partial_fullfit = base; }
 double *fitter_fullfit(gingr_fitter *f) { return f->fullfit; }
 void fitter_set_partial_revsum(gingr_fitter *f, double *base) { f->partial_revsum = base; }
diff --git a/gingr_amd/csrc/fitter_phases.hip b/gingr_amd/csrc/fitter_phases.hip
--- a/gingr_amd/csrc/fitter_phases.hip
+++ b/gingr_amd/csrc/fitter_phases.hip
@@ -91,6 +91,14 @@
     double *seg0w, *Gw, *rhsw, *sc8w;
 };
 
+bool use_compact(const gingr_fitter *f, const Correspondence &c) {
+    const gingr_model *m = f->m;
+    if (!m->Qc || f->ctx->separable == 0) return false;
+    if (m->M != m->M_total || f->partial_out || f->group_member) return false;
+    if (!(c.kind == Flavour::Cpd || (c.kind == Flavour::Pairs && f->n_pc == 0))) return false;
+    return f->n_lm == 0 && !f->zrand_active && !f->allow_alt;
+}
+
 bool memo_enter(gingr_fitter *f, const Correspondence &c, int phase) {
     const gingr_model *m = f->m;
     if (phase == 0) {
@@ -99,6 +107,7 @@
         k.flavour = memo_flavour_key(c, f->surface_method, f->reversed);
         k.p0 = c.cpd.w;
         k.p1 = c.cpd.lambda;
+        k.compact = use_compact(f, c);
         const bool single = m->M == m->M_total;
         if (single && f->state_key_valid) {
             k.v = f->state_key.v;
@@ -386,6 +395,11 @@
             fa.gate = many;
             out.rhs_gate = few;
         }
+    } else if (use_compact(f, c)) {
+        fa.gram_partial = gram_ws;
+        fa.nslabs = launch_gram_compact(ctx, m->Qc, M, f->weight, f->evec, gram_ws);
+        fa.sep_map = m->sep_map;
+        out.rhs_done = true;
     } else {
         fa.gram_partial = gram_ws;
         fa.nslabs = launch_gram(ctx, m->Q0, M, rp, f->weight, gram_ws, nullptr, f->evec, sweep_ws, &out.rhs_done);
@@ -402,6 +416,8 @@
         launch_posterior_solve_eig(ctx, r, rp, m->eigV, m->eigL, &f->st->sigma2, s.rhs, f->acoef, f->st);
     else if (f->zrand_active && f->allow_alt && f->post_stage == 2 && f->nf_valid[f->live] && m->M == m->M_total && !f->partial_out)
         launch_posterior_sample_cached(ctx, r, rp, f->nfac[f->live], f->fxbuf[f->live] + (int64_t)rp * rp, f->zrand, f->acoef, f->st);
+    else if (use_compact(f, c))
+        launch_posterior_solve_separable(ctx, m, s.G, s.rhs, f->acoef, f->st);
     else
         launch_posterior_solve(ctx, r, rp, s.G, s.rhs, f->zrand_active ? f->zrand : nullptr, f->work, f->acoef, f->st);
     launch_post_matvecs(ctx, m, f->alpha, f->acoef, f->zbuf);
@@ -426,7 +442,7 @@
     a.probabilistic = f->zrand_active ? 1 : 0;
     a.stop_threshold = f->stop_threshold;
     launch_post_solve(ctx, a);
-    refresh_fit(f);
+    refresh_fit(f, use_compact(f, c));
 }
 
 int run_phase(gingr_fitter *f, const Correspondence &c, int phase) {
diff --git a/gingr_amd/csrc/gp.h b/gingr_amd/csrc/gp.h
--- a/gingr_amd/csrc/gp.h
+++ b/gingr_amd/csrc/gp.h
@@ -99,7 +99,24 @@
     double Ps[3] = {0};
     std::vector<double> variance;
     bool finalized = false;
-};
+    bool separable = false;
+    std::vector<int32_t> col_class;
+    std::vector<int32_t> class_cols[3];
+    int32_t rc[3] = {0, 0, 0};
+    double *Qc = nullptr;
+    int32_t *sep_map = nullptr;
+};
+
+constexpr int kCompactCols = 48;
+constexpr int kCompactRowSlack = 48;
+struct SepMap {
+    int32_t rp;
+    __host__ __device__ int cls(int k) const { return k; }
+    __host__ __device__ int pos(int k) const { return rp + k; }
+    __host__ __device__ int col(int d, int p) const { return 2 * rp + d * kCompactCols + p; }
+    __host__ __device__ int total() const { return 2 * rp + 3 * kCompactCols; }
+};
+__host__ __device__ inline int64_t compact_plane_doubles(int64_t M) { return (M + kCompactRowSlack) * kCompactCols; }
 
 void launch_interp_pack(gingr_ctx *ctx, const double *Qs, int32_t rp, const int32_t *inv_src, const int32_t *ids, const double *w,
                         const int32_t *perm_new, int64_t row_begin, int64_t M, double *Q0);
@@ -109,6 +126,7 @@
                       const std::function<int(gingr_model *)> &fill_basis, gingr_model **out, bool finalize = true);
 
 void fitter_set_partial_output(gingr_fitter *f, double *base);
+void fitter_set_group_member(gingr_fitter *f);
 void fitter_set_partial_fullfit(gingr_fitter *f, double *base);
 int check_correspondence(gingr_fitter *f, const Correspondence &c);
 typedef int (*fitter_gather_fn)(void *user, gingr_fitter *f);
@@ -192,6 +210,8 @@
     double *weight_out, *evec_out;
     const DevState *frame;
     ZeroGate gate;
+    const double *Qc;
+    const int32_t *sep_map;
 };
 
 int sweep_num_blocks(int64_t M);
@@ -227,8 +247,11 @@
     int32_t contribute_xpx;
     ZeroGate gate;
     int32_t alt_nslabs;
+    const int32_t *sep_map;
 };
 void launch_phase1_finalize(gingr_ctx *ctx, const Phase1FinalizeArgs &a);
+int64_t gram_compact_ws_doubles(int64_t M);
+int launch_gram_compact(gingr_ctx *ctx, const double *Qc, int64_t M, const double *weight, const double *evec, double *ws);
 int launch_gram_downdate(gingr_ctx *ctx, const double *Q0, int64_t M, int32_t rp, const double *weight, double *ws,
                          const ZeroGate *gate = nullptr);
 
@@ -244,6 +267,7 @@
 
 void launch_posterior_solve(gingr_ctx *ctx, int32_t r, int32_t rp, const double *G, const double *rhs, const double *zrand,
                             double *work, double *a, DevState *st);
+void launch_posterior_solve_separable(gingr_ctx *ctx, const gingr_model *m, const double *G, const double *rhs, double *a, DevState *st);
 int launch_posterior_logpdf(gingr_ctx *ctx, int32_t r, int32_t rp, const double *G, const double *rhs, const double *Stot,
                             const double *qte, double *fx, bool cached, double *work, double *out2, unsigned *sync = nullptr,
                             unsigned epoch = 0, bool keep_factor = true, double *nfac = nullptr);
diff --git a/gingr_amd/csrc/gp.hip b/gingr_amd/csrc/gp.hip
--- a/gingr_amd/csrc/gp.hip
+++ b/gingr_amd/csrc/gp.hip
@@ -10,7 +10,7 @@
 template <bool FAST, typename PtrD>
 __device__ __forceinline__ void posterior_solve_body(PtrD sm, int r, int rp, const double *__restrict__ G, const double *__restrict__ rhs,
                                                      const double *__restrict__ zrand, double *__restrict__ a, DevState *__restrict__ st,
-                                                     int *bad_spd, int *bad) {
+                                                     int *bad_spd, int *bad, const int32_t *__restrict__ cols = nullptr, int ldg = 0) {
     const int n = rp, ld = solve_ld(n);
     constexpr int XR = FAST ? 2 * kNB : kNB;
     auto A = sm;
@@ -22,7 +22,7 @@
         *bad_spd = 0;
         *bad = 0;
     }
-    for (int k = tid; k < kNB * ld; k += kSolveThreads) y[k] = k < r ? rhs[k] : 0.0;
+    for (int k = tid; k < kNB * ld; k += kSolveThreads) y[k] = k < r ? rhs[cols ? cols[k] : k] : 0.0;
     for (int k = tid; k < n; k += kSolveThreads) y2[k] = (zrand && k < r) ? zrand[k] : 0.0;
     if (FAST)
         for (int k = tid; k < kNB * ld; k += kSolveThreads) {
@@ -30,7 +30,10 @@
             y[kNB * ld + k] = (j < n && (j & 15) == c) ? 1.0 : 0.0;
         }
     GINGR_STAGE_CLOCK(7)
-    lds_load_spd<kSolveThreads>(A, ld, r, n, G, 1.0, nullptr, 0.0, 1.0);
+    if (cols)
+        lds_load_spd<kSolveThreads, false, kCompactCols / 16>(A, ld, r, n, G, 1.0, nullptr, 0.0, 1.0, cols, ldg);
+    else
+        lds_load_spd<kSolveThreads>(A, ld, r, n, G, 1.0, nullptr, 0.0, 1.0);
     GINGR_STAGE_CLOCK(0)
     lds_cholesky<kSolveThreads>(A, ld, n, rd, bad_spd, kNB, FAST ? kNB : 0);
     GINGR_STAGE_CLOCK(4)
@@ -51,7 +54,10 @@
     GINGR_STAGE_CLOCK(6)
     for (int k = tid; k < rp; k += kSolveThreads) {
         const double v = k < r ? y[k] + y2[k] : 0.0;
-        a[k] = v;
+        if (!cols)
+            a[k] = v;
+        else if (k < r)
+            a[cols[k]] = v;
         if (!finite_d(v)) *bad = 1;
     }
     __syncthreads();
@@ -63,13 +69,24 @@
     }
 }
 
+struct SepCounts {
+    int32_t rc[3];
+};
 template <int MODE>
 __global__ __launch_bounds__(kSolveThreads) void posterior_solve_lds_kernel(int r, int rp, const double *__restrict__ G,
                                                                   const double *__restrict__ rhs,
                                                                   const double *__restrict__ zrand, double *__restrict__ a,
-                                                                  DevState *__restrict__ st) {
+                                                                  DevState *__restrict__ st, const int32_t *__restrict__ sep_map = nullptr,
+                                                                  SepCounts sc = SepCounts{}) {
     extern __shared__ double lds_sm[];
     __shared__ int bad_spd, bad;
+    if constexpr (MODE == 2) {
+        const int d = blockIdx.x;
+        for (int k = r + (int)threadIdx.x; k < rp; k += kSolveThreads) a[k] = 0.0;
+        if (sc.rc[d] == 0) return;
+        posterior_solve_body<true>(lds_sm, sc.rc[d], kCompactCols, G, rhs, nullptr, a, st, &bad_spd, &bad, sep_map + SepMap{rp}.col(d, 0), rp);
+        return;
+    }
 #ifdef GINGR_SOLVE_TWICE
     for (int pass = 0; pass < 2; ++pass) {
         __syncthreads();
@@ -913,6 +930,13 @@
 }
 }
 
+void launch_posterior_solve_separable(gingr_ctx *ctx, const gingr_model *m, const double *G, const double *rhs, double *a, DevState *st) {
+    TimerScope ts(ctx, 5);
+    const size_t lds = lds_solve_doubles(kCompactCols, 2 * kNB) * sizeof(double);
+    hipLaunchKernelGGL(posterior_solve_lds_kernel<2>, dim3(3), dim3(kSolveThreads), lds, ctx->stream, (int)m->r, (int)m->rp, G, rhs,
+                       (const double *)nullptr, a, st, (const int32_t *)m->sep_map, SepCounts{{m->rc[0], m->rc[1], m->rc[2]}});
+}
+
 void launch_posterior_solve(gingr_ctx *ctx, int32_t r, int32_t rp, const double *G, const double *rhs, const double *zrand,
                             double *work, double *a, DevState *st) {
     TimerScope ts(ctx, 5);
@@ -931,7 +955,8 @@
         auto go = [&](auto kern) {
             if (lds > 48 * 1024)
                 set_dynamic_lds(kern, (size_t)(lds));
-            hipLaunchKernelGGL(kern, dim3(1), dim3(kSolveThreads), lds, ctx->stream, (int)r, (int)rp, G, rhs, zrand, a, st);
+            hipLaunchKernelGGL(kern, dim3(1), dim3(kSolveThreads), lds, ctx->stream, (int)r, (int)rp, G, rhs, zrand, a, st,
+                               (const int32_t *)nullptr, SepCounts{});
         };
         if (fast)
             go(posterior_solve_lds_kernel<0>);
diff --git a/gingr_amd/csrc/gp_gram.hip b/gingr_amd/csrc/gp_gram.hip
--- a/gingr_amd/csrc/gp_gram.hip
+++ b/gingr_amd/csrc/gp_gram.hip
@@ -119,7 +119,7 @@
     return t + q;
 }
 
-template <int NT, int HALF, bool FULL>
+template <int NT, int HALF, bool FULL, int RPP>
 __device__ __forceinline__ void gram_tri_half(const double *__restrict__ Q0, int rp, const double *__restrict__ weight, int64_t r0,
                                               int64_t r1, int kgroup, int kq, int cl, int lane, double *red, double *xchg,
                                               double *__restrict__ out, const double *__restrict__ evec, int64_t npts,
@@ -141,12 +141,12 @@
     const double *pnext = Q0 + first * rp + cl;
     const int64_t pstep = 16 * (int64_t)rp;
     int64_t left_u = r1 - ubase;
-    const int64_t pt_first = first / 3;
-    const int rem_first = (int)(first - 3 * pt_first);
+    const int64_t pt_first = first / RPP;
+    const int rem_first = (int)(first - RPP * pt_first);
     constexpr unsigned kThird = 0x55555556u;
     unsigned third = (unsigned)rem_first * kThird;
-    const double *wclamp = with_w ? weight + r0 / 3 : pclamp;
-    const double *eclamp = with_rhs ? evec + r0 / 3 : pclamp;
+    const double *wclamp = with_w ? weight + r0 / RPP : pclamp;
+    const double *eclamp = with_rhs ? evec + r0 / RPP : pclamp;
     const double *wp = with_w ? weight + pt_first : pclamp;
     const double *ep = with_rhs ? evec + rem_first * npts + pt_first : pclamp;
     const int64_t estep = with_rhs ? 5 + npts : 0, ewrap = with_rhs ? 6 - 2 * npts : 0;
@@ -171,11 +171,16 @@
         }
         left_u -= 16;
         pnext += pstep;
-        const unsigned t2 = third + kThird;
-        const bool wrap = t2 < third;
-        third = t2;
-        wp += wrap ? 6 : 5;
-        ep += wrap ? ewrap : estep;
+        if constexpr (RPP == 1) {
+            wp += 16;
+            ep += 16;
+        } else {
+            const unsigned t2 = third + kThird;
+            const bool wrap = t2 < third;
+            third = t2;
+            wp += wrap ? 6 : 5;
+            ep += wrap ? ewrap : estep;
+        }
     };
     double racc[kO];
 #pragma unroll
@@ -304,7 +309,7 @@
                 for (int reg = 0; reg < 4; ++reg) out[(int64_t)(16 * t + kq + 4 * reg) * rp + 16 * u + cl] = acc[q >> 1][reg];
 }
 
-template <int NT, bool FULL>
+template <int NT, bool FULL, int RPP = 3>
 __global__ __launch_bounds__(512) void gram_tri_kernel(const double *__restrict__ Q0, int64_t rows, int rp,
                                                        const double *__restrict__ weight, int64_t rows_per_slab,
                                                        double *__restrict__ partial, const double *__restrict__ evec, int64_t npts,
@@ -319,10 +324,17 @@
     const int64_t r1 = min(rows, r0 + rows_per_slab);
     double *out = partial + (int64_t)blockIdx.x * rp * rp;
     double *rhs_out = rhs_partial ? rhs_partial + (int64_t)blockIdx.x * rp : nullptr;
+    if constexpr (RPP == 1) {
+        const int d = blockIdx.z;
+        Q0 += (int64_t)d * (rows + kCompactRowSlack) * rp;
+        evec += (int64_t)d * npts;
+        out = partial + ((int64_t)blockIdx.x * 3 + d) * (rp * rp + rp);
+        rhs_out = out + rp * rp;
+    }
     if ((wave >> 2) == 0)
-        gram_tri_half<NT, 0, FULL>(Q0, rp, weight, r0, r1, wave & 3, kq, cl, lane, red, xchg, out, evec, npts, rhs_out, rsh);
+        gram_tri_half<NT, 0, FULL, RPP>(Q0, rp, weight, r0, r1, wave & 3, kq, cl, lane, red, xchg, out, evec, npts, rhs_out, rsh);
     else
-        gram_tri_half<NT, 1, FULL>(Q0, rp, weight, r0, r1, wave & 3, kq, cl, lane, red, xchg, out, evec, npts, rhs_out, rsh);
+        gram_tri_half<NT, 1, FULL, RPP>(Q0, rp, weight, r0, r1, wave & 3, kq, cl, lane, red, xchg, out, evec, npts, rhs_out, rsh);
 }
 
 __global__ __launch_bounds__(256) void gram_reduce_kernel(const double *__restrict__ partial, int nslabs, int rp, int symmetric,
@@ -369,7 +381,16 @@
         const int i = idx / rp, j = idx - i * rp;
         const bool need = idx < rr && !(i > j);
         double s = 0.0;
-        if (need) {
+        if (A.sep_map) {
+            constexpr int64_t kBlock = kCompactCols * kCompactCols + kCompactCols;
+            const SepMap sm{rp};
+            const int ci = need ? A.sep_map[sm.cls(i)] : -1, cj = need ? A.sep_map[sm.cls(j)] : -1;
+            if (ci >= 0 && ci == cj) {
+                const double *p = A.gram_partial + ci * kBlock + A.sep_map[sm.pos(i)] * kCompactCols + A.sep_map[sm.pos(j)];
+#pragma unroll 8
+                for (int q = g; q < A.nslabs; q += 8) s += p[(int64_t)q * 3 * kBlock];
+            }
+        } else if (need) {
             const double *p = A.gram_partial + idx;
 #pragma unroll 8
             for (int q = g; q < A.nslabs; q += 8) s += p[(int64_t)q * rr];
@@ -388,7 +409,17 @@
     if (b < nG + rp) {
         const int k = b - nG;
         double s = 0.0;
-        for (int q = threadIdx.x; q < A.sweep_blocks; q += 256) s += A.sweep_partial[(int64_t)q * rp + k];
+        if (A.sep_map) {
+            constexpr int64_t kBlock = kCompactCols * kCompactCols + kCompactCols;
+            const SepMap sm{rp};
+            const int c = A.sep_map[sm.cls(k)];
+            if (c >= 0) {
+                const double *p = A.gram_partial + c * kBlock + kCompactCols * kCompactCols + A.sep_map[sm.pos(k)];
+                for (int q = threadIdx.x; q < A.nslabs; q += 256) s += p[(int64_t)q * 3 * kBlock];
+            }
+        } else {
+            for (int q = threadIdx.x; q < A.sweep_blocks; q += 256) s += A.sweep_partial[(int64_t)q * rp + k];
+        }
         sv[threadIdx.x] = s;
         __syncthreads();
 #pragma unroll
@@ -597,6 +628,29 @@
     return nslabs;
 }
 
+static void gram_compact_plan(int64_t M, int *nslabs, int64_t *rows_per_slab) {
+    const int64_t want = std::min<int64_t>(170, std::max<int64_t>(1, ceil_div(M, 64)));
+    *rows_per_slab = round_up(ceil_div(M, want), 16);
+    *nslabs = (int)ceil_div(M, *rows_per_slab);
+}
+
+int64_t gram_compact_ws_doubles(int64_t M) {
+    int nslabs;
+    int64_t rps;
+    gram_compact_plan(M, &nslabs, &rps);
+    return (int64_t)nslabs * 3 * (kCompactCols * kCompactCols + kCompactCols);
+}
+
+int launch_gram_compact(gingr_ctx *ctx, const double *Qc, int64_t M, const double *weight, const double *evec, double *ws) {
+    int nslabs;
+    int64_t rps;
+    gram_compact_plan(M, &nslabs, &rps);
+    TimerScope ts(ctx, 2);
+    hipLaunchKernelGGL((gram_tri_kernel<kCompactCols / 16, true, 1>), dim3(nslabs, 1, 3), dim3(512), 0, ctx->stream, Qc, M, (int)kCompactCols,
+                       weight, rps, ws, evec, M, (double *)nullptr, ZeroGate{});
+    return nslabs;
+}
+
 int launch_gram_downdate(gingr_ctx *ctx, const double *Q0, int64_t M, int32_t rp, const double *weight, double *ws, const ZeroGate *gate) {
     int nslabs_tri;
     int64_t rows_per_slab;
diff --git a/gingr_amd/csrc/gp_sweep.hip b/gingr_amd/csrc/gp_sweep.hip
--- a/gingr_amd/csrc/gp_sweep.hip
+++ b/gingr_amd/csrc/gp_sweep.hip
@@ -241,14 +241,17 @@
     if (threadIdx.x == 0) out[k] = sh[0];
 }
 
-template <int KM, int S>
+template <int KM, int S, bool SEP = false>
 __global__ __launch_bounds__(kSweepThreads) void sweep_fit_boxes_kernel(SweepArgs a) {
     constexpr int CH = KM < 8 ? KM : 8;
+    constexpr int ND = SEP ? 3 : 1;
     static_assert(4 % S == 0, "points per group and round");
     extern __shared__ double lds[];
     const int tid = threadIdx.x, lane16 = tid & 15, grp = tid >> 4;
-    const int rp = a.rp, km = rp >> 4;
+    const int rp = a.rp, km = SEP ? KM : rp >> 4;
     const int64_t M = a.M;
+    const int64_t qstride = SEP ? kCompactCols : rp, dstride = SEP ? compact_plane_doubles(M) : rp;
+    const double *basis = SEP ? a.Qc : a.Q0;
     double *coef = lds, *red = lds + rp;
     for (int k = tid; k < rp; k += kSweepThreads) coef[k] = a.coef0[k];
     double R[9], tr[3], cen[3];
@@ -258,10 +261,19 @@
         cen[q] = a.state->center[q];
     }
     const double scale = a.state->scale;
-    double cf[KM];
+    double cf[ND][KM];
     __syncthreads();
 #pragma unroll
-    for (int m = 0; m < KM; ++m) cf[m] = m < km ? coef[m * 16 + lane16] : 0.0;
+    for (int e = 0; e < ND; ++e)
+#pragma unroll
+        for (int m = 0; m < KM; ++m) {
+            if constexpr (SEP) {
+                const int col = a.sep_map[SepMap{rp}.col(e, m * 16 + lane16)];
+                cf[e][m] = col >= 0 ? coef[col] : 0.0;
+            } else {
+                cf[e][m] = m < km ? coef[m * 16 + lane16] : 0.0;
+            }
+        }
     double amax = 0.0;
     for (int64_t qd = blockIdx.x; qd * 64 < M; qd += gridDim.x) {
         double lo[3] = {__builtin_huge_val(), __builtin_huge_val(), __builtin_huge_val()};
@@ -280,11 +292,11 @@
                 for (int s = 0; s < S; ++s) {
                     const int64_t p = qd * 64 + (s0 + s) * kGroups + grp;
                     const int64_t pc = p < M ? p : 0;
-                    const double *q0 = a.Q0 + (3 * pc) * rp + lane16;
+                    const double *q0 = basis + (SEP ? pc : 3 * pc) * qstride + lane16;
 #pragma unroll
                     for (int d = 0; d < 3; ++d) {
 #pragma unroll
-                        for (int m = 0; m < CH; ++m) u[s][d][m] = (mc + m < KM && mc + m < km) ? q0[d * rp + (mc + m) * 16] : 0.0;
+                        for (int m = 0; m < CH; ++m) u[s][d][m] = (mc + m < KM && mc + m < km) ? q0[d * dstride + (mc + m) * 16] : 0.0;
                         if (mc == 0) rm[s][d] = a.ref[d * M + pc] + a.mean[d * M + pc];
                     }
                 }
@@ -294,7 +306,7 @@
                     for (int d = 0; d < 3; ++d)
 #pragma unroll
                         for (int m = 0; m < CH; ++m)
-                            if (mc + m < KM) facc[s][d] = __builtin_fma(u[s][d][m], cf[mc + m], facc[s][d]);
+                            if (mc + m < KM) facc[s][d] = __builtin_fma(u[s][d][m], cf[SEP ? d : 0][mc + m], facc[s][d]);
             }
 #pragma unroll
             for (int s = 0; s < S; ++s) {
@@ -361,7 +373,9 @@
         const int nq = (int)std::min<int64_t>(4096, ceil_div(a.M, 64));
         const size_t l2 = (size_t)(a.rp + kGroups * 8 + 8) * sizeof(double);
         TimerScope ts(ctx, 4);
-        if (a.rp <= 64)
+        if (a.Qc && a.sep_map)
+            hipLaunchKernelGGL((sweep_fit_boxes_kernel<kCompactCols / 16, 4, true>), dim3(nq), dim3(kSweepThreads), l2, ctx->stream, a);
+        else if (a.rp <= 64)
             hipLaunchKernelGGL((sweep_fit_boxes_kernel<4, 4>), dim3(nq), dim3(kSweepThreads), l2, ctx->stream, a);
         else if (a.rp <= 112)
             hipLaunchKernelGGL((sweep_fit_boxes_kernel<7, 4>), dim3(nq), dim3(kSweepThreads), l2, ctx->stream, a);
diff --git a/gingr_amd/csrc/group.hip b/gingr_amd/csrc/group.hip
--- a/gingr_amd/csrc/group.hip
+++ b/gingr_amd/csrc/group.hip
@@ -292,7 +292,11 @@
     }
     g->rank = gingr_model_rank(g->model[0]);
     g->fit.assign((size_t)n, nullptr);
-    return g->run([&](int r) { return gingr_fitter_create(g->ctx[(size_t)r], g->model[(size_t)r], &g->fit[(size_t)r]); });
+    return g->run([&](int r) {
+        const int rc = gingr_fitter_create(g->ctx[(size_t)r], g->model[(size_t)r], &g->fit[(size_t)r]);
+        if (rc == GINGR_OK) fitter_set_group_member(g->fit[(size_t)r]);
+        return rc;
+    });
 }
 
 int exchange_buffers(gingr_group *g, int r, std::vector<hipEvent_t> &ev, const std::vector<double *> &src_base, int64_t src_off, double *dst,
diff --git a/gingr_amd/csrc/model.hip b/gingr_amd/csrc/model.hip
--- a/gingr_amd/csrc/model.hip
+++ b/gingr_amd/csrc/model.hip
@@ -27,7 +27,95 @@
     Q[idx] = q < k ? Qs[row * rps + q] : 0.0;
 }
 
+constexpr int kSepBlocks = 256;
+__global__ __launch_bounds__(256) void sep_flags_kernel(const double *__restrict__ Q0, int64_t rows, int32_t rp, int32_t *__restrict__ partial) {
+    const int64_t per = (rows + gridDim.x - 1) / gridDim.x;
+    const int64_t r0 = (int64_t)blockIdx.x * per, r1 = r0 + per < rows ? r0 + per : rows;
+    for (int k = threadIdx.x; k < rp; k += 256) {
+        int32_t fl[3] = {0, 0, 0};
+        for (int64_t row = r0; row < r1; ++row)
+            if (Q0[row * rp + k] != 0.0) fl[row % 3] = 1;
+        for (int d = 0; d < 3; ++d) partial[(int64_t)blockIdx.x * 3 * rp + d * rp + k] = fl[d];
+    }
+}
+__global__ __launch_bounds__(256) void sep_flags_reduce_kernel(const int32_t *__restrict__ partial, int nblocks, int32_t n, int32_t *__restrict__ flags) {
+    const int q = blockIdx.x * 256 + threadIdx.x;
+    if (q >= n) return;
+    int32_t f = 0;
+    for (int b = 0; b < nblocks; ++b) f |= partial[(int64_t)b * n + q];
+    flags[q] = f;
+}
+__global__ __launch_bounds__(256) void compact_basis_kernel(const double *__restrict__ Q0, int64_t M, int32_t rp, const int32_t *__restrict__ sep_map,
+                                                            double *__restrict__ Qc) {
+    const int64_t idx = (int64_t)blockIdx.x * 256 + threadIdx.x;
+    if (idx >= 3 * M * kCompactCols) return;
+    const int k = (int)(idx % kCompactCols);
+    const int64_t pd = idx / kCompactCols;
+    const int64_t p = pd % M;
+    const int d = (int)(pd / M);
+    const int col = sep_map[SepMap{rp}.col(d, k)];
+    Qc[d * compact_plane_doubles(M) + p * kCompactCols + k] = col >= 0 ? Q0[(3 * p + d) * rp + col] : 0.0;
+}
+
+int model_detect_separable(gingr_ctx *ctx, gingr_model *m) {
+    const int32_t r = m->r, rp = m->rp;
+    const int64_t rows = 3 * m->M;
+    dev_free(m->Qc), dev_free(m->sep_map);
+    m->Qc = nullptr, m->sep_map = nullptr;
+    m->separable = false;
+    const int nb = (int)std::min<int64_t>(kSepBlocks, (rows + 63) / 64);
+    DevBuf part, flags;
+    HIP_TRY(ctx, part.alloc((size_t)nb * 3 * rp * sizeof(int32_t)));
+    HIP_TRY(ctx, flags.alloc((size_t)3 * rp * sizeof(int32_t)));
+    hipLaunchKernelGGL(sep_flags_kernel, dim3(nb), dim3(256), 0, ctx->stream, m->Q0, rows, rp, part.as<int32_t>());
+    hipLaunchKernelGGL(sep_flags_reduce_kernel, dim3((unsigned)ceil_div(3 * rp, 256)), dim3(256), 0, ctx->stream, part.as<int32_t>(), nb, 3 * rp,
+                       flags.as<int32_t>());
+    GINGR_TRY(check_launch(ctx));
+    std::vector<int32_t> hf((size_t)3 * rp);
+    HIP_TRY(ctx, hipMemcpyAsync(hf.data(), flags.p, hf.size() * sizeof(int32_t), hipMemcpyDeviceToHost, ctx->stream));
+    HIP_TRY(ctx, hipStreamSynchronize(ctx->stream));
+    m->col_class.assign((size_t)r, 0);
+    for (int d = 0; d < 3; ++d) m->class_cols[d].clear();
+    bool sep = true;
+    for (int32_t k = 0; k < r; ++k) {
+        const int n = hf[(size_t)k] + hf[(size_t)rp + k] + hf[(size_t)2 * rp + k];
+        if (n > 1) sep = false;
+        const int cls = hf[(size_t)k] ? 0 : hf[(size_t)rp + k] ? 1 : hf[(size_t)2 * rp + k] ? 2 : 0;
+        m->col_class[(size_t)k] = cls;
+        m->class_cols[cls].push_back(k);
+    }
+    for (int d = 0; d < 3; ++d) m->rc[d] = (int32_t)m->class_cols[d].size();
+    if (!sep) {
+        m->col_class.clear();
+        for (int d = 0; d < 3; ++d) m->class_cols[d].clear(), m->rc[d] = 0;
+        return GINGR_OK;
+    }
+    m->separable = true;
+    if (m->M != m->M_total || rp > 112 || std::max(m->rc[0], std::max(m->rc[1], m->rc[2])) > kCompactCols) return GINGR_OK;
+    const SepMap sm{rp};
+    std::vector<int32_t> map((size_t)sm.total(), -1);
+    for (int d = 0; d < 3; ++d)
+        for (int32_t p = 0; p < m->rc[d]; ++p) {
+            const int32_t k = m->class_cols[d][(size_t)p];
+            map[(size_t)sm.cls(k)] = d;
+            map[(size_t)sm.pos(k)] = p;
+            map[(size_t)sm.col(d, p)] = k;
+        }
+    GINGR_TRY(dev_alloc(ctx, &m->sep_map, map.size()));
+    GINGR_TRY(dev_alloc(ctx, &m->Qc, (size_t)3 * compact_plane_doubles(m->M)));
+    HIP_TRY(ctx, hipMemcpyAsync(m->sep_map, map.data(), map.size() * sizeof(int32_t), hipMemcpyHostToDevice, ctx->stream));
+    for (int d = 0; d < 3; ++d)
+        HIP_TRY(ctx, hipMemsetAsync(m->Qc + d * compact_plane_doubles(m->M) + m->M * kCompactCols, 0,
+                                    (size_t)kCompactRowSlack * kCompactCols * sizeof(double), ctx->stream));
+    hipLaunchKernelGGL(compact_basis_kernel, dim3((unsigned)ceil_div(3 * m->M * kCompactCols, 256)), dim3(256), 0, ctx->stream, m->Q0, m->M, rp,
+                       m->sep_map, m->Qc);
+    GINGR_TRY(check_launch(ctx));
+    HIP_TRY(ctx, hipStreamSynchronize(ctx->stream));
+    return GINGR_OK;
+}
+
 int model_finalize_impl(gingr_ctx *ctx, gingr_model *m) {
+    GINGR_TRY(model_detect_separable(ctx, m));
     DevBuf work, flag;
     HIP_TRY(ctx, work.alloc((size_t)binv_work_doubles(m->rp) * sizeof(double)));
     HIP_TRY(ctx, flag.alloc(sizeof(int32_t)));
@@ -224,9 +312,18 @@
 void gingr_model_destroy(gingr_model *m) {
     if (!m) return;
     if (m->ctx) (void)hipSetDevice(m->ctx->device);
-    void *ptrs[] = {m->Q0, m->ref, m->mean, m->mom, m->Binv, m->eigV, m->eigL, m->cmat, m->pvec, m->perm, m->iperm};
+    void *ptrs[] = {m->Q0, m->ref, m->mean, m->mom, m->Binv, m->eigV, m->eigL, m->cmat, m->pvec, m->perm, m->iperm, m->Qc, m->sep_map};
     for (void *p : ptrs) dev_free(p);
     delete m;
+}
+
+int gingr_model_separable(const gingr_model *m, int32_t *separable, int32_t class_counts[3], int32_t *compact) {
+    if (!m || !separable) return GINGR_ERR_BAD_ARGUMENT;
+    *separable = m->separable ? 1 : 0;
+    if (class_counts)
+        for (int d = 0; d < 3; ++d) class_counts[d] = m->rc[d];
+    if (compact) *compact = m->Qc ? 1 : 0;
+    return GINGR_OK;
 }
 
 int64_t gingr_model_num_points(const gingr_model *m) { return m ? m->M : 0; }
diff --git a/gingr_amd/csrc/solve_blocks.h b/gingr_amd/csrc/solve_blocks.h
--- a/gingr_amd/csrc/solve_blocks.h
+++ b/gingr_amd/csrc/solve_blocks.h
@@ -62,26 +62,28 @@
 __host__ __device__ inline int solve_ld(int n) { return n | 1; }
 __host__ __device__ inline size_t lds_solve_doubles(int rp, int xr) { return (size_t)(rp + xr) * solve_ld(rp) + 2 * (size_t)rp; }
 
-template <int NT, bool HAS_S = false>
+template <int NT, bool HAS_S = false, int MAXB = 8>
 __device__ __forceinline__ void lds_load_spd(double *A, int ld, int r, int n, const double *__restrict__ G, double ca,
-                                             const double *__restrict__ S, double cs, double ci) {
+                                             const double *__restrict__ S, double cs, double ci, const int32_t *__restrict__ cols = nullptr,
+                                             int ldg = 0) {
     const int tid = threadIdx.x, tx = tid & 15, ty = tid >> 4;
     constexpr int RB = NT / 16;
-    if (RB == 16 && n <= 128) {
-        double v[36], vs[HAS_S ? 36 : 1];
+    if (RB == 16 && n <= 16 * MAXB) {
+        double v[MAXB * (MAXB + 1) / 2], vs[HAS_S ? MAXB * (MAXB + 1) / 2 : 1];
         int idx = 0;
 #pragma unroll
-        for (int bi = 0; bi < 8; ++bi)
+        for (int bi = 0; bi < MAXB; ++bi)
 #pragma unroll
             for (int bj = 0; bj <= bi; ++bj, ++idx) {
                 const int i = bi * 16 + ty, j = bj * 16 + tx;
-                const int g = min(min(i, r - 1), n - 1) * n + min(j, r - 1);
+                int g = min(min(i, r - 1), n - 1) * n + min(j, r - 1);
+                if (cols) g = cols[min(min(i, r - 1), n - 1)] * ldg + cols[min(j, r - 1)];
                 v[idx] = G[g];
                 if (HAS_S) vs[idx] = S[g];
             }
         idx = 0;
 #pragma unroll
-        for (int bi = 0; bi < 8; ++bi)
+        for (int bi = 0; bi < MAXB; ++bi)
 #pragma unroll
             for (int bj = 0; bj <= bi; ++bj, ++idx) {
                 double t = ca * v[idx];
@@ -90,7 +92,7 @@
             }
         idx = 0;
 #pragma unroll
-        for (int bi = 0; bi < 8; ++bi)
+        for (int bi = 0; bi < MAXB; ++bi)
 #pragma unroll
             for (int bj = 0; bj <= bi; ++bj, ++idx) {
                 const int i = bi * 16 + ty, j = bj * 16 + tx;
diff --git a/gingr_amd/models.py b/gingr_amd/models.py
--- a/gingr_amd/models.py
+++ b/gingr_amd/models.py
@@ -599,6 +599,12 @@
     def finalize(self):
         _check(self.ctx.handle, self._lib.gingr_model_finalize(self.ctx.handle, self.handle), "gingr_model_finalize")
 
+    def separable(self) -> Tuple[bool, Tuple[int, int, int], bool]:
+        sep, compact, counts = ctypes.c_int32(), ctypes.c_int32(), (ctypes.c_int32 * 3)()
+        _check(self.ctx.handle, self._lib.gingr_model_separable(self.handle, ctypes.byref(sep), counts, ctypes.byref(compact)),
+               "gingr_model_separable")
+        return bool(sep.value), tuple(counts), bool(compact.value)
+
     def close(self):
         if getattr(self, "handle", None):
             if self._owner and getattr(self.ctx, "handle", None):
diff --git a/include/gingr_hip.h b/include/gingr_hip.h
--- a/include/gingr_hip.h
+++ b/include/gingr_hip.h
@@ -52,7 +52,8 @@
     GINGR_OPT_TRI_GRID = 3,
     GINGR_OPT_SPLIT_EXCHANGE = 4,
     GINGR_OPT_GRAM_DOWNDATE = 5,
-    GINGR_OPT_DECIMATE_BATCH = 6
+    GINGR_OPT_DECIMATE_BATCH = 6,
+    GINGR_OPT_SEPARABLE = 7
 } gingr_ctx_option;
 int gingr_ctx_set_option(gingr_ctx *ctx, int32_t option, int32_t value);
 int gingr_ctx_get_option(gingr_ctx *ctx, int32_t option, int32_t *value);
@@ -112,6 +113,7 @@
                          double *variance);
 int64_t gingr_model_num_points(const gingr_model *model);
 int32_t gingr_model_rank(const gingr_model *model);
+int gingr_model_separable(const gingr_model *model, int32_t *separable, int32_t class_counts[3], int32_t *compact);
 
 int gingr_model_instance(gingr_ctx *ctx, const gingr_model *model, const double *alpha, const double euler[3],
                          const double center[3], const double translation[3], double scale, double *out_xyz);
```

Measured after the change: 467.4 iterations/s, median of 6. +2.6%, better.
